# crowdbotp/socialways

Measured on AMD Instinct MI355X. Metric: GAN train steps/sec (256 scenes x 8 agents x 8+12 T per GPU step; fp32; social block on), higher is better.
Workload: dtype f32; 1 GPU; m1: 256 scenes x 8 agents x (8 obs + 12 pred) per GPU step = reference --batch-size 2048; use_social=True, n_unrolling_steps=1, info loss on; full=False, global_batch_scenes=256, parallelism=dp1, steps_per_graph_launch=32, settle_steps=992, rehearsal_regions=2, step_alg_bytes=5527040, inputs=z drawn on the host every step

## Files before the change

include/socialways_hip.h:

```cpp
#ifndef SOCIALWAYS_HIP_H
#define SOCIALWAYS_HIP_H
#include <stddef.h>
#include <stdint.h>

#ifdef __cplusplus
extern "C" {
#endif

#define SW_OK 0
#define SW_EARG -1
#define SW_ESHAPE -2
#define SW_EHIP -3

#define SW_H 64
#define SW_Z 32

enum { SW_GRP_ENC = 0, SW_GRP_EMB = 1, SW_GRP_ATT = 2, SW_GRP_DEC = 3, SW_GRP_DISC = 4 };

enum {
  SW_WS_GSAVE = 0,
  SW_WS_GDELTA = 1,
  SW_WS_DSAVE = 2,
  SW_WS_DDELTA = 3,
  SW_WS_WGRAD = 4,
  SW_WS_PAIRS = 5
};

int sw_version(void);
const char* sw_last_error(void);

int sw_param_count(int grp, int Tp);
int sw_param_offset(int grp, int idx, int Tp);
int sw_param_tensors(int grp);
size_t sw_workspace_floats(int ws_id, int B, int To, int Tp, int nb, long long P);

int sw_traj_4d(const float* obsv , const float* pred , int B, int To,
               int Tp, float* obsv4 , float* pred4 , void* stream);

int sw_enc_lstm_fwd(const float* x, int x_mode, const float* enc_w, const float* h0, const float* c0,
                    int B, int T, float* hT, float* cT, float* y , float* act,
                    float* x4s, int t0, void* stream);
int sw_enc_lstm_fwd_aux(const float* x, int x_mode, const float* enc_w, const float* h0, const float* c0, int B, int T,
                        float* hT, float* cT, float* y, float* act, float* x4s, int t0, const float* aux_src,
                        float* aux_dst, long long aux_n, void* stream);
int sw_enc_lstm_fwd_ragged(const float* x, int x_mode, const float* enc_w, const int* obs_len ,
                           int B, int T, float* hT , float* cT , void* stream);
int sw_enc_lstm_bwd(const float* enc_w, const float* act, const float* c0, const float* dhT,
                    const float* dcT, const float* dy, int B, int T, int t0, float* dgates,
                    float* dh0, float* dc0, void* stream);

int sw_social_pool_fwd(const float* obsv , int To, const float* h ,
                       const int* scene_off, int S, int B, int Amax ,
                       const float* emb_w, const float* att_w, float* S_out ,
                       float* attn ,
                       const int* big_blocks , int NB, float* wh_ws, float* ml , void* stream);
int sw_social_pool_fwd_aux(const float* obsv, int To, const float* h, const int* scene_off, int S, int B, int Amax,
                           const float* emb_w, const float* att_w, float* S_out, float* attn, const int* big_blocks,
                           int NB, float* wh_ws, float* ml, const float* aux_src, float* aux_dst, long long aux_n,
                           void* stream);
int sw_social_features(const float* x4_last , int B, float* feat , void* stream);
int sw_embed_features(const float* feat , long long R, const float* emb_w, float* out ,
                      void* stream);
int sw_attention_pool_dense(const float* f , const float* h , const int* scene_off,
                            int S, int B, const float* att_w, float* S_out , void* stream);
int sw_rows_gemm(const float* x, int ldx, const float* w, int w_rs, int w_cs, const float* bias, long long R, int K, int N,
                 float* y, int ldy, int accumulate, void* stream);
int sw_linear_wgrad(const float* delta, int ldd, const float* act, int lda, int R, int N, int K, float* dW, int ldw,
                    float* db, float* wgrad_ws, int accumulate, void* stream);
int sw_embed_features_bwd(const float* feat , long long R, const float* emb_w, const float* dout ,
                          float* rows, float* dfeat, void* stream);
int sw_attention_dense_fwd(const float* f, const float* h, const float* wh, const int* scene_off, int S, int B, float* attn,
                           float* S_out, void* stream);
int sw_attention_dense_bwd(const float* f, const float* h, const float* wh, const float* attn, const float* dS,
                           const int* scene_off, int S, int B, float* dsig, float* df, float* dwh, float* dh, void* stream);
int sw_enc_lstm_wgrad(const float* enc_w, const float* act, const float* x4s, const float* h0, const float* dgates, int B,
                      int T, float* d_enc_w, float* wgrad_ws, float* tmp, void* stream);
int sw_dec_fc_wgrad(const float* dec_w, const float* gsave, const float* gdelta, const float* h, const float* s,
                    const float* z, int B, int To, float* d_dec_w, float* wgrad_ws, float* tmp, void* stream);

int sw_dec_fc_dz(const float* dec_w, const float* gdelta, int B, int To, float* dz, void* stream);

typedef struct sw_wgrad_batch sw_wgrad_batch;
sw_wgrad_batch* sw_wgrad_batch_new(void);
void sw_wgrad_batch_free(sw_wgrad_batch* h);

int sw_social_pool_bwd(const float* obsv, int To, const float* h, const int* scene_off,
                       const long long* pair_off, int S, int B, int Amax, long long P,
                       const float* emb_w, const float* att_w, const float* attn, const float* dS,
                       float* dh, float* d_emb_w, float* d_att_w, float* pair_ws, float* wgrad_ws,
                       const int* big_blocks , int NB, const float* wh_ws, const float* ml,
                       const float* S_pool, float* big_part_ws,
                       sw_wgrad_batch* defer ,
                       void* stream);

int sw_dec_rollout_fwd(const float* obsv , int To, const float* z ,
                       const float* S_pool , const float* hT, const float* cT,
                       const float* enc_w, const float* dec_w, int B, int Tp,
                       float* pred4 , float* h_end, float* c_end ,
                       float* gsave ,
                       const float* gt , float inv_ss, float* ade_part ,
                       void* stream);
int sw_dec_rollout_fwd_aux(const float* obsv, int To, const float* z, const float* S_pool, const float* hT,
                           const float* cT, const float* enc_w, const float* dec_w, int B, int Tp, float* pred4,
                           float* h_end, float* c_end, float* gsave, const float* gt, float inv_ss, float* ade_part,
                           const float* d_w , float* dsave , void* stream);
int sw_dec_sample_fwd(const float* obsv , int To, const float* z ,
                      const float* S_pool , const float* hT, const float* cT ,
                      const float* enc_w, const float* dec_w, int B, int K, int Tp, float* pred4, const float* gt ,
                      float inv_ss, float* err, void* stream);
int sw_sample_reduce(const float* err , int B, int K, float* per_agent , int* best ,
                     void* stream);
int sw_sample_rank(const float* score , const float* err , const int* best ,
                   int B, int K, int M, int* order , float* per_agent , void* stream);
int sw_scene_clearance(const float* pos, int pstride, const float* start , int sstride, const int* scene_off,
                       int S, int B, int K, int Tp, float inv_ss, float* clear , void* stream);
int sw_scene_reduce(const float* err , const float* clear , const int* scene_off, int S, int B,
                    int K, float coll_dist, float* per_scene , int* best , void* stream);
int sw_sample_nms(const float* pos, int pstride, const float* score , const int* scene_off , int S,
                  int B, int K, int Tp, int M, int metric, float inv_ss, float radius, const float* err ,
                  const int* best , int* order , int* count , float* weight ,
                  int* assign , float* per_row , void* stream);
int sw_dec_rollout_bwd(const float* dpred4 , const float* enc_w, const float* dec_w,
                       const float* gsave, int B, int To, int Tp, float* gdelta,
                       float* dhT, float* dcT, float* dS_pool , void* stream);
int sw_dec_rollout_bwd_aux(const float* dpred4, const float* enc_w, const float* dec_w, const float* gsave, int B,
                           int To, int Tp, float* gdelta, float* dhT, float* dcT, float* dS_pool,
                           const float* aux_src, float* aux_dst, const float* aux_mask, long long aux_n, void* stream);
int sw_gen_wgrad(const float* enc_w, const float* dec_w, const float* gsave, const float* gdelta, const float* z,
                 const float* S_pool, int B, int To, int Tp, float* d_enc_w, float* d_dec_w, int part,
                 float* wgrad_ws, float* tmp ,
                 sw_wgrad_batch* pending ,
                 void* stream);
int sw_gen_wgrad_adam(const float* enc_w, const float* dec_w, const float* gsave, const float* gdelta,
                      const float* z, const float* S_pool, int B, int To, int Tp, float* d_enc_w, float* d_dec_w,
                      float* wgrad_ws, float* tmp , sw_wgrad_batch* pending , float* adam_w,
                      float* adam_m, float* adam_v, const float* adam_g, long long adam_n, const float* adam_step,
                      double lr, double beta1, double beta2, double eps, void* stream);

int sw_disc_fwd(const float* obsv, int To, int x_mode, const float* const* pred4 ,
                int nb, const float* d_w, int B, int Tp, float* const* label ,
                float* const* code , float* dsave ,
                int save_lstm ,
                float* w_snapshot ,
                void* stream);
int sw_disc_bwd(const float* d_w, const float* dsave, const float* const* dlabel,
                const float* const* dcode, int nb, int B, int To, int Tp, float* ddelta,
                float* d_d_w, float* const* dpred4, float* wgrad_ws, void* stream);

int sw_disc_bwd_gan(const float* d_w, const float* dsave, const float* const* label,
                    const float* const* code, const float* targets, int t0, int t1, const float* z ,
                    float g_label, float g_code, int nb, int B, int To, int Tp, float* ddelta,
                    float* d_d_w, float* const* dpred4, float* wgrad_ws,
                    float* loss_part ,
                    void* stream);
int sw_disc_bwd_gan_adam(const float* d_w, const float* dsave, const float* const* label, const float* const* code,
                         const float* targets, int t0, int t1, const float* z, float g_label, float g_code, int nb,
                         int B, int To, int Tp, float* ddelta, float* d_d_w, float* const* dpred4, float* wgrad_ws,
                         float* loss_part, float* adam_w, float* adam_m, float* adam_v, const float* adam_step,
                         double lr, double beta1, double beta2, double eps, void* stream);

int sw_disc_update_supported(const float* d_w, int B, int To, int Tp);
int sw_disc_update(const float* obsv , int To, const float* const* pred4 , const float* d_w, int B,
                   int Tp, float* const* label, float* const* code, float* dsave, int obs_pre, float* w_snapshot ,
                   const float* targets, int t0, int t1, const float* z, float g_label, float g_code, float* ddelta,
                   float* d_d_w, float* wgrad_ws, float* loss_part , float* adam_w , float* adam_m,
                   float* adam_v, const float* adam_step, double lr, double beta1, double beta2, double eps, void* stream);

int sw_disc_dpred_supported(int Tp);
int sw_disc_dpred(const float* obsv, int To, int x_mode, const float* pred4 , const float* d_w, int B, int Tp,
                  const float* targets, int t_idx, const float* z , float g_label, float g_code,
                  float* dpred4 , float* label , float* code ,
                  float* loss_part , void* stream);

int sw_disc_score(const float* obsv, int To, int x_mode, const float* pred4 , const float* d_w, int B, int K,
                  int Tp, float* score , float* code , void* stream);

int sw_disc_score_ragged(const float* obsv, int To, int x_mode, const int* obs_len ,
                         const float* pred4 , const float* d_w, int B, int K, int Tp, float* score ,
                         float* code , void* stream);

#define SW_RED_BLOCKS 64
int sw_gan_loss(const float* label_a, const float* targets , int ia,
                const float* code_a, const float* z , const float* label_b, int ib, int B,
                float g_label, float g_code, float* out_sums , float* dlabel_a, float* dcode_a,
                float* dlabel_b, float* dcode_b, float* scratch , void* stream);

int sw_l2_grad(const float* pred4_hat , const float* gt , int B, int Tp, int row0, int row1,
               float scale, float* dpred4 , void* stream);

int sw_variety_grad(const float* pred4_hat_K , const float* gt , int K, int B, int Tp,
                    float scale, float* dpred4_K , int* kmin, float* l2min, void* stream);

int sw_traj_dist(const float* a , const float* b , int Na, int Nb, int nPed, int T,
                 int t0, float* D , void* stream);

#define SW_STAGE_HEADER 8
int sw_stage_step(const float* slot, int B, int To, int Tp, float* obsv_dst , float* pred_dst ,
                  float* pred4_dst , float* targets_dst , float* z_dst ,
                  float* steps_dst , int n_d_updates, void* stream);

int sw_gen_image_floats(void);
int sw_gen_images(const float* enc_w, const float* dec_w, const float* emb_w , const float* att_w ,
                  float* img, void* stream);
int sw_stage_step_img(const float* slot, int B, int To, int Tp, float* obsv_dst, float* pred_dst, float* pred4_dst,
                      float* targets_dst, float* z_dst, float* steps_dst, int n_d_updates, const float* enc_w,
                      const float* dec_w, const float* emb_w , const float* att_w , float* img,
                      const float* d_w , float* d_img , const int* d_tab , void* stream);
int sw_stage_step_zdev(const float* slot, int B, int To, int Tp, float* obsv_dst, float* pred_dst, float* pred4_dst,
                       float* targets_dst, float* z_dst, float* steps_dst, int n_d_updates, const float* enc_w,
                       const float* dec_w, const float* emb_w, const float* att_w, float* img, const float* d_w, float* d_img,
                       const int* d_tab, int z_device, void* stream);

int sw_disc_image_floats(int Tp);
int sw_disc_image_table(int Tp, int* tab_host);
int sw_disc_images(const float* d_w, float* img, const int* tab, int Tp, void* stream);

int sw_lstm_point_fwd(const float* pre, const float* c_prev, int B, int H, float* gates, float* c, float* h, void* stream);
int sw_lstm_point_bwd(const float* gates, const float* c, const float* c_prev, const float* dh, const float* dc, int B,
                      int H, float* dpre, float* dc_prev, void* stream);
int sw_act_fwd(const float* x, long long n, int kind, float* y, void* stream);
int sw_act_bwd(const float* y, const float* dy, long long n, int kind, float* dx, void* stream);
int sw_sqdiff(const float* a, int lda, const float* b, int ldb, const float* target, int target_idx, long long R, int C,
              float gscale, float* out_sum, float* da, int ldda, void* stream);
int sw_pair_features(const float* x4_last, const int* scene_off, const long long* pair_off, int S, float* feat, void* stream);
int sw_attn_pairs_fwd(const float* f, const float* wh, const float* h, const int* scene_off, const long long* pair_off, int S,
                      int B, int F, int H, float* attn, float* S_out, void* stream);
int sw_attn_pairs_bwd(const float* f, const float* wh, const float* h, const float* attn, const float* dS, const int* scene_off,
                      const long long* pair_off, int S, int B, int F, int H, float* dsig, float* df, float* dwh, float* dh,
                      void* stream);

int sw_adam_packed(float* w, const float* g, float* m, float* v, long long n, const float* step, double lr, double beta1,
                   double beta2, double eps, int disc_Tp, void* stream);

int sw_enc_lstm_bwd_aux(const float* enc_w, const float* act, const float* c0, const float* dhT, const float* dcT,
                        const float* dy, int B, int T, int t0, float* dgates, float* dh0, float* dc0, const float* aux_src,
                        float* aux_dst, const float* aux_mask, long long aux_n, void* stream);
int sw_dec_rollout_bwd_dfuse(const float* obsv, const float* pred4, const float* d_w, const float* targets, int t_idx,
                             const float* z, float g_label, float g_code, float* loss_part, float* dpred4, const float* enc_w,
                             const float* dec_w, const float* gsave, int B, int To, int Tp, float* gdelta, float* dhT, float* dcT,
                             float* dS_pool, void* stream);

int sw_wide_gemm(const float* x, long long x_rs, int x_cs, const float* w, long long w_rs, int w_cs, const float* bias,
                 const float* cin, int cin_ld, const float* aux, int aux_ld, long long R, int K, int N, float* y, int y_ld, int epi,
                 void* stream);
int sw_wide_lstm_fwd(const float* x4, int x_ld, const float* h_prev, int hp_ld, const float* c_prev, const float* Wx,
                     const float* b1, const float* b2, const float* Whh, int B, int H, float* gates, float* c_out, float* h_out,
                     int h_ld, float* h_out2, int h2_ld, void* stream);
int sw_wide_lstm_bwd(const float* dh_ext, int dhe_ld, const float* dh_ext2, int dhe2_ld, const float* dg_next, const float* WhhT,
                     const float* gates, const float* c, const float* c_prev, const float* dc_in, int B, int H, float* dgates,
                     float* dc_out, void* stream);
int sw_wide_out_fwd(const float* a3, int D3, const float* W4, const float* b4, float* p, int B, float* pred4_i, int pred_ld,
                    float* x4_tm, void* stream);
int sw_wide_out_bwd(const float* dpred4_i, int pred_ld, const float* dg, const float* WxT, int H4, float* dp_run, int B, float* dv,
                    const float* W4, int D3, float* dz3, void* stream);
int sw_wide_sum_steps(const float* in, long long t_stride, int in_ld, int T, long long R, int C, float* out, int out_ld,
                      void* stream);
int sw_wide_transpose(const float* src, const int* tab, int ntab, int total_tiles, float* dst, void* stream);
int sw_wide_opimage(const float* src, const int* tab, int ntab, long long total_float4, float* dst, void* stream);
int sw_wide_lstm_seq_supported(int H);
int sw_wide_lstm_seq_fwd(const float* x4, const float* Wx, const float* b1, const float* b2, const float* whh_img, int B, int H, int T,
                         float* gates, float* cs, float* hs, float* h_last2, int h2_ld, void* stream);
int sw_wide_lstm_seq_bwd(const float* dh_ext, int dhe_ld, const float* dh_ext2, int dhe2_ld, const float* dg_init, const float* dc_init,
                         const float* whhT_img, const float* gates, const float* cs, int B, int H, int T, float* dgates, void* stream);
int sw_wide_dec_loop_supported(int H);
int sw_wide_dec_loop_fwd(const float* w1h_img, const float* w2_img, const float* w3_img, const float* whh_img, const float* u,
                         const float* b2, const float* b3, const float* W4, const float* b4, const float* Wx, const float* bx1,
                         const float* bx2, const float* p0, int p0_ld, float* a1, float* a2, float* a3, float* pred4, float* x4,
                         float* gates, float* cs, float* hs, float* cat, int B, int H, int To, int Tp, void* stream);
int sw_wide_dec_loop_bwd(const float* whhT_img, const float* w3T_img, const float* w2T_img, const float* w1hT_img,
                         const float* wxT_img, const float* W4, const float* dpred4, const float* a1, const float* a2,
                         const float* gates, const float* cs, float* dgates, float* dv, float* dz3, float* dz2, float* dz1,
                         float* dhcat_out, float* dc_out, int B, int H, int To, int Tp, void* stream);
int sw_wide_disc_heads_supported(int H, int K4, int nl);
int sw_wide_disc_heads_fwd(const long long* p, void* stream);
int sw_wide_disc_heads_bwd(const long long* p, void* stream);
int sw_wide_wgrad(const long long* desc, int n, float* wgrad_ws, void* stream);

long long sw_comm_bytes(int world, long long max_floats);
int sw_comm_alloc(long long bytes, void** ptr);
int sw_comm_free(void* ptr);
int sw_comm_ipc_export(void* ptr, void* handle64 );
int sw_comm_ipc_import(const void* handle64, void** ptr);
int sw_comm_ipc_close(void* ptr);
int sw_comm_status(const void* own_buf, int* status );
int sw_allreduce_direct(void* const* peer_bufs , int rank, int world, long long max_floats, float* grad,
                        long long n, void* stream);
int sw_allreduce_direct_adam(void* const* peer_bufs, int rank, int world, long long max_floats, float* grad, long long n,
                             float* w, float* m, float* v, const float* step, double lr, double beta1, double beta2,
                             double eps, int disc_Tp, void* stream);

int sw_ade_fde(const float* pred4 , const float* gt , int B, int Tp, float inv_ss,
               float* out , float* scratch , void* stream);

int sw_noise_uniform(unsigned long long seed, int domain, unsigned step0, int n_steps, unsigned draw0, int n_draws,
                     unsigned row0, int rows, int cols, int ld, float* out , void* stream);

int sw_kernel_timing(int on);
int sw_kernel_timing_read(char* buf, int cap);
int sw_debug_spin(double us, void* stream);

#ifdef __cplusplus
}
#endif
#endif
```

socialways_amd/_lib.py:

```python
import ctypes
import os

import torch

_HERE = os.path.dirname(os.path.abspath(__file__))
LIB_PATH = os.environ.get("SW_LIB_PATH") or os.path.join(_HERE, "libsocialways_hip.so")

GRP_ENC, GRP_EMB, GRP_ATT, GRP_DEC, GRP_DISC = 0, 1, 2, 3, 4
WS_GSAVE, WS_GDELTA, WS_DSAVE, WS_DDELTA, WS_WGRAD, WS_PAIRS = 0, 1, 2, 3, 4, 5
AMAX = 64
RED_BLOCKS = 64

_vp, _i, _f, _ll = ctypes.c_void_p, ctypes.c_int, ctypes.c_float, ctypes.c_longlong

PROTOTYPES = {
    "sw_version": (_i, []),
    "sw_last_error": (ctypes.c_char_p, []),
    "sw_param_count": (_i, [_i, _i]),
    "sw_param_offset": (_i, [_i, _i, _i]),
    "sw_param_tensors": (_i, [_i]),
    "sw_workspace_floats": (ctypes.c_size_t, [_i, _i, _i, _i, _i, _ll]),
    "sw_traj_4d": (_i, [_vp, _vp, _i, _i, _i, _vp, _vp, _vp]),
    "sw_enc_lstm_fwd": (_i, [_vp, _i, _vp, _vp, _vp, _i, _i, _vp, _vp, _vp, _vp, _vp, _i, _vp]),
    "sw_enc_lstm_fwd_aux": (_i, [_vp, _i, _vp, _vp, _vp, _i, _i, _vp, _vp, _vp, _vp, _vp, _i, _vp, _vp, _ll, _vp]),
    "sw_enc_lstm_fwd_ragged": (_i, [_vp, _i, _vp, _vp, _i, _i, _vp, _vp, _vp]),
    "sw_enc_lstm_bwd": (_i, [_vp, _vp, _vp, _vp, _vp, _vp, _i, _i, _i, _vp, _vp, _vp, _vp]),
    "sw_social_pool_fwd": (_i, [_vp, _i, _vp, _vp, _i, _i, _i, _vp, _vp, _vp, _vp, _vp, _i, _vp, _vp, _vp]),
    "sw_social_pool_fwd_aux": (_i, [_vp, _i, _vp, _vp, _i, _i, _i, _vp, _vp, _vp, _vp, _vp, _i, _vp, _vp, _vp, _vp, _ll, _vp]),
    "sw_social_features": (_i, [_vp, _i, _vp, _vp]),
    "sw_embed_features": (_i, [_vp, _ll, _vp, _vp, _vp]),
    "sw_attention_pool_dense": (_i, [_vp, _vp, _vp, _i, _i, _vp, _vp, _vp]),
    "sw_social_pool_bwd": (_i, [_vp, _i, _vp, _vp, _vp, _i, _i, _i, _ll, _vp, _vp, _vp, _vp, _vp, _vp, _vp,
                                _vp, _vp, _vp, _i, _vp, _vp, _vp, _vp, _vp, _vp]),
    "sw_dec_rollout_fwd": (_i, [_vp, _i, _vp, _vp, _vp, _vp, _vp, _vp, _i, _i, _vp, _vp, _vp, _vp, _vp, _f, _vp, _vp]),
    "sw_dec_rollout_fwd_aux": (_i, [_vp, _i, _vp, _vp, _vp, _vp, _vp, _vp, _i, _i, _vp, _vp, _vp, _vp, _vp, _f, _vp, _vp, _vp, _vp]),
    "sw_dec_sample_fwd": (_i, [_vp, _i, _vp, _vp, _vp, _vp, _vp, _vp, _i, _i, _i, _vp, _vp, _f, _vp, _vp]),
    "sw_sample_reduce": (_i, [_vp, _i, _i, _vp, _vp, _vp]),
    "sw_sample_rank": (_i, [_vp, _vp, _vp, _i, _i, _i, _vp, _vp, _vp]),
    "sw_scene_clearance": (_i, [_vp, _i, _vp, _i, _vp, _i, _i, _i, _i, _f, _vp, _vp]),
    "sw_scene_reduce": (_i, [_vp, _vp, _vp, _i, _i, _i, _f, _vp, _vp, _vp]),
    "sw_sample_nms": (_i, [_vp, _i, _vp, _vp, _i, _i, _i, _i, _i, _i, _f, _f, _vp, _vp, _vp, _vp, _vp, _vp, _vp, _vp]),
    "sw_dec_rollout_bwd": (_i, [_vp, _vp, _vp, _vp, _i, _i, _i, _vp, _vp, _vp, _vp, _vp]),
    "sw_dec_rollout_bwd_aux": (_i, [_vp, _vp, _vp, _vp, _i, _i, _i, _vp, _vp, _vp, _vp, _vp, _vp, _vp, _ll, _vp]),
    "sw_gen_wgrad": (_i, [_vp, _vp, _vp, _vp, _vp, _vp, _i, _i, _i, _vp, _vp, _i, _vp, _vp, _vp, _vp]),
    "sw_gen_wgrad_adam": (_i, [_vp, _vp, _vp, _vp, _vp, _vp, _i, _i, _i, _vp, _vp, _vp, _vp, _vp, _vp, _vp, _vp, _vp,
                               ctypes.c_longlong, _vp, ctypes.c_double, ctypes.c_double, ctypes.c_double, ctypes.c_double, _vp]),
    "sw_enc_lstm_bwd_aux": (_i, [_vp, _vp, _vp, _vp, _vp, _vp, _i, _i, _i, _vp, _vp, _vp, _vp, _vp, _vp, _ll, _vp]),
    "sw_dec_rollout_bwd_dfuse": (_i, [_vp, _vp, _vp, _vp, _i, _vp, _f, _f, _vp, _vp, _vp, _vp, _vp, _i, _i, _i, _vp, _vp, _vp, _vp,
                                      _vp]),
    "sw_rows_gemm": (_i, [_vp, _i, _vp, _i, _i, _vp, ctypes.c_longlong, _i, _i, _vp, _i, _i, _vp]),
    "sw_linear_wgrad": (_i, [_vp, _i, _vp, _i, _i, _i, _i, _vp, _i, _vp, _vp, _i, _vp]),
    "sw_embed_features_bwd": (_i, [_vp, ctypes.c_longlong, _vp, _vp, _vp, _vp, _vp]),
    "sw_attention_dense_fwd": (_i, [_vp, _vp, _vp, _vp, _i, _i, _vp, _vp, _vp]),
    "sw_attention_dense_bwd": (_i, [_vp, _vp, _vp, _vp, _vp, _vp, _i, _i, _vp, _vp, _vp, _vp, _vp]),
    "sw_enc_lstm_wgrad": (_i, [_vp, _vp, _vp, _vp, _vp, _i, _i, _vp, _vp, _vp, _vp]),
    "sw_dec_fc_dz": (_i, [_vp, _vp, _i, _i, _vp, _vp]),
    "sw_dec_fc_wgrad": (_i, [_vp, _vp, _vp, _vp, _vp, _vp, _i, _i, _vp, _vp, _vp, _vp]),
    "sw_wgrad_batch_new": (_vp, []),
    "sw_wgrad_batch_free": (None, [_vp]),
    "sw_disc_fwd": (_i, [_vp, _i, _i, _vp, _i, _vp, _i, _i, _vp, _vp, _vp, _i, _vp, _vp]),
    "sw_disc_bwd": (_i, [_vp, _vp, _vp, _vp, _i, _i, _i, _i, _vp, _vp, _vp, _vp, _vp]),
    "sw_disc_bwd_gan": (_i, [_vp, _vp, _vp, _vp, _vp, _i, _i, _vp, _f, _f, _i, _i, _i, _i, _vp, _vp, _vp, _vp, _vp, _vp]),
    "sw_disc_bwd_gan_adam": (_i, [_vp, _vp, _vp, _vp, _vp, _i, _i, _vp, _f, _f, _i, _i, _i, _i, _vp, _vp, _vp, _vp, _vp,
                                  _vp, _vp, _vp, _vp, ctypes.c_double, ctypes.c_double, ctypes.c_double, ctypes.c_double, _vp]),
    "sw_disc_update_supported": (_i, [_vp, _i, _i, _i]),
    "sw_disc_dpred_supported": (_i, [_i]),
    "sw_disc_update": (_i, [_vp, _i, _vp, _vp, _i, _i, _vp, _vp, _vp, _i, _vp, _vp, _i, _i, _vp, _f, _f, _vp, _vp, _vp, _vp,
                            _vp, _vp, _vp, _vp, ctypes.c_double, ctypes.c_double, ctypes.c_double, ctypes.c_double, _vp]),
    "sw_disc_dpred": (_i, [_vp, _i, _i, _vp, _vp, _i, _i, _vp, _i, _vp, _f, _f, _vp, _vp, _vp, _vp, _vp]),
    "sw_disc_score": (_i, [_vp, _i, _i, _vp, _vp, _i, _i, _i, _vp, _vp, _vp]),
    "sw_disc_score_ragged": (_i, [_vp, _i, _i, _vp, _vp, _vp, _i, _i, _i, _vp, _vp, _vp]),
    "sw_gan_loss": (_i, [_vp, _vp, _i, _vp, _vp, _vp, _i, _i, _f, _f, _vp, _vp, _vp, _vp, _vp, _vp, _vp]),
    "sw_l2_grad": (_i, [_vp, _vp, _i, _i, _i, _i, _f, _vp, _vp]),
    "sw_variety_grad": (_i, [_vp, _vp, _i, _i, _i, _f, _vp, _vp, _vp, _vp]),
    "sw_traj_dist": (_i, [_vp, _vp, _i, _i, _i, _i, _i, _vp, _vp]),
    "sw_stage_step": (_i, [_vp, _i, _i, _i, _vp, _vp, _vp, _vp, _vp, _vp, _i, _vp]),
    "sw_gen_image_floats": (_i, []),
    "sw_gen_images": (_i, [_vp, _vp, _vp, _vp, _vp, _vp]),
    "sw_stage_step_img": (_i, [_vp, _i, _i, _i, _vp, _vp, _vp, _vp, _vp, _vp, _i, _vp, _vp, _vp, _vp, _vp, _vp, _vp, _vp, _vp]),
    "sw_stage_step_zdev": (_i, [_vp, _i, _i, _i, _vp, _vp, _vp, _vp, _vp, _vp, _i, _vp, _vp, _vp, _vp, _vp, _vp, _vp, _vp, _i, _vp]),
    "sw_disc_image_floats": (_i, [_i]),
    "sw_disc_image_table": (_i, [_i, _vp]),
    "sw_disc_images": (_i, [_vp, _vp, _vp, _i, _vp]),
    "sw_ade_fde": (_i, [_vp, _vp, _i, _i, _f, _vp, _vp, _vp]),
    "sw_lstm_point_fwd": (_i, [_vp, _vp, _i, _i, _vp, _vp, _vp, _vp]),
    "sw_lstm_point_bwd": (_i, [_vp, _vp, _vp, _vp, _vp, _i, _i, _vp, _vp, _vp]),
    "sw_act_fwd": (_i, [_vp, _ll, _i, _vp, _vp]),
    "sw_act_bwd": (_i, [_vp, _vp, _ll, _i, _vp, _vp]),
    "sw_sqdiff": (_i, [_vp, _i, _vp, _i, _vp, _i, _ll, _i, _f, _vp, _vp, _i, _vp]),
    "sw_pair_features": (_i, [_vp, _vp, _vp, _i, _vp, _vp]),
    "sw_attn_pairs_fwd": (_i, [_vp, _vp, _vp, _vp, _vp, _i, _i, _i, _i, _vp, _vp, _vp]),
    "sw_attn_pairs_bwd": (_i, [_vp, _vp, _vp, _vp, _vp, _vp, _vp, _i, _i, _i, _i, _vp, _vp, _vp, _vp, _vp]),
    "sw_adam_packed": (_i, [_vp, _vp, _vp, _vp, _ll, _vp, ctypes.c_double, ctypes.c_double, ctypes.c_double,
                            ctypes.c_double, _i, _vp]),
    "sw_wide_gemm": (_i, [_vp, _ll, _i, _vp, _ll, _i, _vp, _vp, _i, _vp, _i, _ll, _i, _i, _vp, _i, _i, _vp]),
    "sw_wide_lstm_fwd": (_i, [_vp, _i, _vp, _i, _vp, _vp, _vp, _vp, _vp, _i, _i, _vp, _vp, _vp, _i, _vp, _i, _vp]),
    "sw_wide_lstm_bwd": (_i, [_vp, _i, _vp, _i, _vp, _vp, _vp, _vp, _vp, _vp, _i, _i, _vp, _vp, _vp]),
    "sw_wide_out_fwd": (_i, [_vp, _i, _vp, _vp, _vp, _i, _vp, _i, _vp, _vp]),
    "sw_wide_out_bwd": (_i, [_vp, _i, _vp, _vp, _i, _vp, _i, _vp, _vp, _i, _vp, _vp]),
    "sw_wide_sum_steps": (_i, [_vp, _ll, _i, _i, _ll, _i, _vp, _i, _vp]),
    "sw_wide_wgrad": (_i, [_vp, _i, _vp, _vp]),
    "sw_wide_transpose": (_i, [_vp, _vp, _i, _i, _vp, _vp]),
    "sw_wide_dec_loop_supported": (_i, [_i]),
    "sw_wide_dec_loop_fwd": (_i, [_vp] * 13 + [_i] + [_vp] * 9 + [_i, _i, _i, _i, _vp]),
    "sw_wide_dec_loop_bwd": (_i, [_vp] * 18 + [_i, _i, _i, _i, _vp]),
    "sw_wide_disc_heads_supported": (_i, [_i, _i, _i]),
    "sw_wide_disc_heads_fwd": (_i, [_vp, _vp]),
    "sw_wide_disc_heads_bwd": (_i, [_vp, _vp]),
    "sw_wide_opimage": (_i, [_vp, _vp, _i, _ll, _vp, _vp]),
    "sw_wide_lstm_seq_supported": (_i, [_i]),
    "sw_wide_lstm_seq_fwd": (_i, [_vp, _vp, _vp, _vp, _vp, _i, _i, _i, _vp, _vp, _vp, _vp, _i, _vp]),
    "sw_wide_lstm_seq_bwd": (_i, [_vp, _i, _vp, _i, _vp, _vp, _vp, _vp, _vp, _i, _i, _i, _vp, _vp]),
    "sw_comm_bytes": (_ll, [_i, _ll]),
    "sw_comm_alloc": (_i, [_ll, _vp]),
    "sw_comm_free": (_i, [_vp]),
    "sw_comm_ipc_export": (_i, [_vp, _vp]),
    "sw_comm_ipc_import": (_i, [_vp, _vp]),
    "sw_comm_ipc_close": (_i, [_vp]),
    "sw_comm_status": (_i, [_vp, _vp]),
    "sw_allreduce_direct": (_i, [_vp, _i, _i, _ll, _vp, _ll, _vp]),
    "sw_allreduce_direct_adam": (_i, [_vp, _i, _i, _ll, _vp, _ll, _vp, _vp, _vp, _vp, ctypes.c_double, ctypes.c_double,
                                      ctypes.c_double, ctypes.c_double, _i, _vp]),
    "sw_noise_uniform": (_i, [ctypes.c_ulonglong, _i, ctypes.c_uint, _i, ctypes.c_uint, _i, ctypes.c_uint, _i, _i, _i, _vp, _vp]),
}

DEBUG_PROTOTYPES = {
    "sw_kernel_timing": (_i, [_i]),
    "sw_kernel_timing_read": (_i, [ctypes.c_char_p, _i]),
    "sw_debug_spin": (_i, [ctypes.c_double, _vp]),
}
_lib = None


class SocialWaysHipError(RuntimeError):
    pass


def load():
    global _lib
    if _lib is not None:
        return _lib
    if not os.path.exists(LIB_PATH):
        raise SocialWaysHipError(
            "%s not found - build it with `python -c 'import __graft_entry__ as g; g.build()'` or "
            "`make -C socialways_amd/csrc`; socialways_amd has no CPU fallback" % LIB_PATH)
    lib = ctypes.CDLL(LIB_PATH)
    for name, (res, args) in list(PROTOTYPES.items()) + list(DEBUG_PROTOTYPES.items()):
        fn = getattr(lib, name)
        fn.restype = res
        fn.argtypes = args
    _lib = lib
    return lib


def ptr(t):
    if t is None:
        return None
    assert t.is_contiguous(), "socialways_amd kernels need contiguous tensors"
    return t.data_ptr()


def ptr_strided(t):
    return None if t is None else t.data_ptr()


def stream():
    return torch.cuda.current_stream().cuda_stream


TIMING = None


def call(name, *args):
    lib = load()
    t = TIMING
    if t is not None and name in t["names"]:
        e0, e1 = torch.cuda.Event(enable_timing=True), torch.cuda.Event(enable_timing=True)
        e0.record()
        rc = getattr(lib, name)(*args)
        e1.record()
        t["events"].append((name, e0, e1))
    else:
        rc = getattr(lib, name)(*args)
    if rc != 0:
        msg = {-1: "bad argument", -2: "unsupported shape", -3: "HIP error: " + lib.sw_last_error().decode()}.get(rc, "?")
        raise SocialWaysHipError("%s failed (%d): %s" % (name, rc, msg))


def ptr_array(tensors):
    arr = (ctypes.c_void_p * len(tensors))(*[ptr(t) for t in tensors])
    return ctypes.cast(arr, ctypes.c_void_p), arr


def workspace_floats(ws_id, B, To, Tp, nb=1, P=0):
    return int(load().sw_workspace_floats(ws_id, B, To, Tp, nb, P))


def require_gpu(t):
    if not t.is_cuda:
        raise SocialWaysHipError("socialways_amd runs on MI355X only: got a %s tensor (no CPU fallback)" % t.device)


def indexed_device(device):
    d = torch.device(device)
    if d.type == "cuda" and d.index is None and torch.cuda.is_available():
        d = torch.device("cuda", torch.cuda.current_device())
    return d
```

socialways_amd/csrc/sw_misc.hip:

```cpp
#include "../../include/socialways_hip.h"
#include "sw_common.h"
#include "sw_lstm_dev.h"
#include <stdlib.h>
#include "sw_wgrad.h"
#include <stdio.h>
#include <string.h>

static thread_local char g_err[256] = "";
void sw_set_error(const char* what, hipError_t e) {
  snprintf(g_err, sizeof(g_err), "%s: %s", what, hipGetErrorString(e));
}
extern "C" const char* sw_last_error(void) { return g_err; }

int sw_set_lds(const void* fn, int bytes, int& have) {
  if (have >= bytes) return SW_OK;
  hipError_t e = hipFuncSetAttribute(fn, hipFuncAttributeMaxDynamicSharedMemorySize, bytes);
  if (e != hipSuccess) {
    sw_set_error("hipFuncSetAttribute(MaxDynamicSharedMemorySize)", e);
    return SW_EHIP;
  }
  have = bytes;
  return SW_OK;
}

#include <string>
#include <vector>
#include <map>
bool g_sw_ktime_on = false;
#include <mutex>
namespace {
struct KtRec { const char* name; hipEvent_t e0, e1; bool ended; };
std::vector<KtRec> g_kt;
std::mutex g_kt_mu;
thread_local long t_kt_open = -1;
}
void sw_ktime_begin(const char* name, hipStream_t st) {
  t_kt_open = -1;
  hipStreamCaptureStatus cs = hipStreamCaptureStatusNone;
  if (hipStreamIsCapturing(st, &cs) != hipSuccess || cs != hipStreamCaptureStatusNone) { (void)hipGetLastError(); return; }
  KtRec r{name, nullptr, nullptr, false};
  if (hipEventCreate(&r.e0) != hipSuccess) { (void)hipGetLastError(); return; }
  if (hipEventCreate(&r.e1) != hipSuccess) { (void)hipGetLastError(); (void)hipEventDestroy(r.e0); return; }
  (void)hipEventRecord(r.e0, st);
  std::lock_guard<std::mutex> lk(g_kt_mu);
  g_kt.push_back(r);
  t_kt_open = (long)g_kt.size() - 1;
}
void sw_ktime_end(hipStream_t st) {
  const long i = t_kt_open;
  t_kt_open = -1;
  if (i < 0) return;
  std::lock_guard<std::mutex> lk(g_kt_mu);
  if (i >= (long)g_kt.size() || g_kt[i].ended) return;
  (void)hipEventRecord(g_kt[i].e1, st);
  g_kt[i].ended = true;
}
extern "C" int sw_kernel_timing(int on) {
  std::lock_guard<std::mutex> lk(g_kt_mu);
  for (auto& r : g_kt) { (void)hipEventDestroy(r.e0); (void)hipEventDestroy(r.e1); }
  g_kt.clear();
  g_sw_ktime_on = on != 0;
  return SW_OK;
}
extern "C" int sw_kernel_timing_read(char* buf, int cap) {
  if (hipDeviceSynchronize() != hipSuccess) return SW_EHIP;
  std::map<std::string, std::pair<long, double>> agg;
  std::lock_guard<std::mutex> lk(g_kt_mu);
  for (auto& r : g_kt) {
    if (!r.ended) continue;
    float ms = 0.f;
    if (hipEventElapsedTime(&ms, r.e0, r.e1) != hipSuccess) { (void)hipGetLastError(); continue; }
    std::string n(r.name);
    size_t a = n.find_first_not_of("( ");
    n = n.substr(a == std::string::npos ? 0 : a);
    n = n.substr(0, n.find_first_of("<)"));
    auto& e = agg[n];
    e.first += 1;
    e.second += 1e3 * ms;
  }
  std::string out;
  char line[256];
  for (auto& kv : agg) {
    snprintf(line, sizeof(line), "%s %ld %.3f\n", kv.first.c_str(), kv.second.first, kv.second.second);
    out += line;
  }
  if (buf && cap > 0) {
    const size_t k = out.size() < (size_t)cap - 1 ? out.size() : (size_t)cap - 1;
    memcpy(buf, out.data(), k);
    buf[k] = 0;
  }
  return (int)out.size() + 1;
}
__global__ void spin_kernel(long long cycles) {
  const long long t0 = wall_clock64();
  while (wall_clock64() - t0 < cycles) __builtin_amdgcn_s_sleep(32);
}
__global__ void nop_kernel() {}
extern "C" int sw_debug_spin(double us, void* stream) {
  if (us < 0 || us > 2e6) return SW_EARG;
  if (us == 0.0) {
    SW_LAUNCH(nop_kernel, dim3(1), dim3(64), 0, (hipStream_t)stream);
    SW_CHECK_LAUNCH("nop_kernel");
    return SW_OK;
  }
  SW_LAUNCH(spin_kernel, dim3(1), dim3(64), 0, (hipStream_t)stream, (long long)(us * 100.0));
  SW_CHECK_LAUNCH("spin_kernel");
  return SW_OK;
}

__global__ __launch_bounds__(256) void adam_packed_kernel(WgAdam ad, long long n) {
  __shared__ float bc[2];
  if (threadIdx.x == 0) wg_adam_bc_compute(ad.step, ad.beta1, ad.beta2, bc[0], bc[1]);
  __syncthreads();
  const float bc1 = bc[0], bc2s = bc[1];
  for (long long i = (long long)blockIdx.x * 256 + threadIdx.x; i < n; i += (long long)gridDim.x * 256) {
    const float g = ad.g0[i];
    wg_adam_fin(ad, wg_adam_pre(ad, ad.g0 + i), bc1, bc2s, g);
  }
}
extern "C" int sw_adam_packed(float* w, const float* g, float* m, float* v, long long n, const float* step, double lr,
                              double beta1, double beta2, double eps, int disc_Tp, void* stream) {
  if (!w || !g || !m || !v || !step || n < 1) return SW_EARG;
  WgAdam ad;
  ad.w = w; ad.m = m; ad.v = v; ad.g0 = g; ad.step = step; ad.n = (size_t)n;
  ad.lr = lr; ad.beta1 = beta1; ad.beta2 = beta2; ad.eps = eps;
  if (disc_Tp > 0) {
    const DiscImages di = sw_disc_images_for(w, disc_Tp);
    ad.img = const_cast<float*>(di.img);
    ad.tab = di.tab;
  }
  int blocks = (int)((n + 255) / 256);
  if (blocks > 512) blocks = 512;
  SW_LAUNCH(adam_packed_kernel, dim3(blocks), dim3(256), 0, (hipStream_t)stream, ad, n);
  SW_CHECK_LAUNCH("adam_packed_kernel");
  return SW_OK;
}
extern "C" int sw_version(void) { return 3; }

size_t sw_dsave_floats(int B, int To, int Tp, int nb);
size_t sw_ddelta_floats(int B, int To, int Tp, int nb);

static int group_offsets(int grp, int Tp, int* off, int* count) {
  using namespace swp;
  switch (grp) {
    case SW_GRP_ENC: {
      const int o[] = {ENC_EMB_W, ENC_EMB_B, ENC_WIH, ENC_WHH, ENC_BIH, ENC_BHH};
      memcpy(off, o, sizeof(o));
      *count = ENC_N;
      return 6;
    }
    case SW_GRP_EMB: {
      const int o[] = {EMB_W0, EMB_B0, EMB_W1, EMB_B1, EMB_W2, EMB_B2};
      memcpy(off, o, sizeof(o));
      *count = EMB_N;
      return 6;
    }
    case SW_GRP_ATT: {
      const int o[] = {ATT_W, ATT_B};
      memcpy(off, o, sizeof(o));
      *count = ATT_N;
      return 2;
    }
    case SW_GRP_DEC: {
      const int o[] = {DEC_W1, DEC_B1, DEC_W2, DEC_B2, DEC_W3, DEC_B3, DEC_W4, DEC_B4};
      memcpy(off, o, sizeof(o));
      *count = DEC_N;
      return 8;
    }
    case SW_GRP_DISC: {
      if (Tp < 1) return -1;
      Disc d = disc(Tp);
      const int o[] = {d.wih,  d.whh,  d.bih,  d.bhh,  d.of0w, d.of0b, d.of1w, d.of1b, d.pe0w, d.pe0b,
                       d.pe1w, d.pe1b, d.cl0w, d.cl0b, d.cl1w, d.cl1b, d.la0w, d.la0b, d.la1w, d.la1b};
      memcpy(off, o, sizeof(o));
      *count = d.n;
      return 20;
    }
  }
  return -1;
}
extern "C" int sw_param_tensors(int grp) {
  int off[32], n;
  return group_offsets(grp, 1, off, &n);
}
extern "C" int sw_param_count(int grp, int Tp) {
  int off[32], n = -1;
  if (group_offsets(grp, Tp, off, &n) < 0) return SW_EARG;
  return n;
}
extern "C" int sw_param_offset(int grp, int idx, int Tp) {
  int off[32], n;
  int k = group_offsets(grp, Tp, off, &n);
  if (k < 0 || idx < 0 || idx >= k) return SW_EARG;
  return off[idx];
}

extern "C" size_t sw_workspace_floats(int ws_id, int B, int To, int Tp, int nb, long long P) {
  if (B < 0 || To < 1 || Tp < 1) return 0;
  switch (ws_id) {
    case SW_WS_GSAVE: return gsave_layout(B, To, Tp).total;
    case SW_WS_GDELTA: return gdelta_layout(B, To, Tp).total;
    case SW_WS_DSAVE: return sw_dsave_floats(B, To, Tp, nb < 1 ? 1 : nb);
    case SW_WS_DDELTA: return sw_ddelta_floats(B, To, Tp, nb < 1 ? 1 : nb);
    case SW_WS_WGRAD: return SW_WG_WS_FLOATS;
    case SW_WS_PAIRS: return (size_t)B * 200 + (size_t)(P < 0 ? 0 : P) * 196;
  }
  return 0;
}

#define SW_DEC_COMPOSE_BLOCKS 13
__device__ __forceinline__ void compose_bwd_block(const int blk, const float* __restrict__ enc_w,
                                                  const float* __restrict__ dWx, const float* __restrict__ dbx,
                                                  float* __restrict__ d_enc_w, const float* __restrict__ dec_w,
                                                  const float* __restrict__ Ms, float* __restrict__ d_dec_w,
                                                  const WgAdam& ad, const float* __restrict__ snap) {
  using namespace swp;
  float bc1 = 1.f, bc2s = 1.f;
  if (ad.w) wg_adam_bc(ad, bc1, bc2s);
  auto put = [&](float* dst, float g) {
    *dst = g;
    if (ad.w) wg_adam1(ad, bc1, bc2s, dst, g);
  };
  if (blk >= 128) {
    const int o = (blk - 128) * 256 + threadIdx.x;
    const float* M = Ms;
    const float* sv = Ms + 160;
    const float* W3 = snap ? snap + swimg::RAW_W3 : dec_w + DEC_W3;
    const float* W4 = snap ? snap + swimg::RAW_W4 : dec_w + DEC_W4;
    const float* b3 = snap ? snap + swimg::RAW_B3 : dec_w + DEC_B3;
    if (o < 3200) {
      const int m = o / 80, k = o - m * 80;
      put(d_dec_w + DEC_W3 + o, fmaf(W4[m], M[k], W4[40 + m] * M[80 + k]));
    } else if (o < 3240) {
      const int m = o - 3200;
      put(d_dec_w + DEC_B3 + m, fmaf(W4[m], sv[0], W4[40 + m] * sv[1]));
    } else if (o < 3320) {
      const int c = (o - 3240) / 40, m = (o - 3240) - c * 40;
      float v = sv[c] * b3[m];
      for (int k = 0; k < 80; ++k) v = fmaf(M[c * 80 + k], W3[m * 80 + k], v);
      put(d_dec_w + DEC_W4 + c * 40 + m, v);
    } else if (o < 3322) {
      put(d_dec_w + DEC_B4 + (o - 3320), sv[o - 3320]);
    }
    return;
  }
  const float* We = snap ? snap + swimg::RAW_WE : enc_w + ENC_EMB_W;
  const float* be = snap ? snap + swimg::RAW_BE : enc_w + ENC_EMB_B;
  const float* Wih = snap ? snap + swimg::RAW_WIH : enc_w + ENC_WIH;
  const int t = threadIdx.x;
  if (blk < 64) {
    int i = blk * 256 + t;
    int row = i >> 6, e = i & 63;
    f32x4 g = ld4(dWx + row * 4), w = ld4(We + e * 4);
    float v = dbx[row] * be[e];
    v = fmaf(g[0], w[0], v); v = fmaf(g[1], w[1], v); v = fmaf(g[2], w[2], v); v = fmaf(g[3], w[3], v);
    put(d_enc_w + ENC_WIH + i, v);
    if (blk == 0) {
      put(d_enc_w + ENC_BIH + t, dbx[t]);
      put(d_enc_w + ENC_BHH + t, dbx[t]);
    }
    return;
  }
  __shared__ float red[5][256];
  const int e = blk - 64;
  float w = Wih[t * 64 + e];
  f32x4 g = ld4(dWx + t * 4);
  red[0][t] = w * g[0]; red[1][t] = w * g[1]; red[2][t] = w * g[2]; red[3][t] = w * g[3]; red[4][t] = w * dbx[t];
  __syncthreads();
  for (int o = 128; o > 0; o >>= 1) {
    if (t < o) {
#pragma unroll
      for (int c = 0; c < 5; ++c) red[c][t] += red[c][t + o];
    }
    __syncthreads();
  }
  if (t < 4) put(d_enc_w + ENC_EMB_W + e * 4 + t, red[t][0]);
  if (t == 4) put(d_enc_w + ENC_EMB_B + e, red[4][0]);
}

__global__ __launch_bounds__(256) void enc_compose_bwd_kernel(const float* __restrict__ enc_w,
                                                              const float* __restrict__ dWx,
                                                              const float* __restrict__ dbx,
                                                              float* __restrict__ d_enc_w,
                                                              const float* __restrict__ dec_w,
                                                              const float* __restrict__ Ms,
                                                              float* __restrict__ d_dec_w, WgAdam ad,
                                                              const float* __restrict__ snap) {
  compose_bwd_block((int)blockIdx.x, enc_w, dWx, dbx, d_enc_w, dec_w, Ms, d_dec_w, ad, snap);
}
__global__ __launch_bounds__(256) void compose_bwd_part_kernel(const float* __restrict__ enc_w, const float* __restrict__ dWx,
                                                               const float* __restrict__ dbx, float* __restrict__ d_enc_w,
                                                               const float* __restrict__ dec_w, const float* __restrict__ Ms,
                                                               float* __restrict__ d_dec_w, int block0) {
  compose_bwd_block((int)blockIdx.x + block0, enc_w, dWx, dbx, d_enc_w, dec_w, Ms, d_dec_w, WgAdam(), nullptr);
}

static int gen_wgrad_impl(const float* enc_w, const float* dec_w, const float* gsave, const float* gdelta, const float* z,
                          const float* S_pool, int B, int To, int Tp, float* d_enc_w, float* d_dec_w, int part,
                          float* wgrad_ws, float* tmp, sw_wgrad_batch* pending, void* stream, WgAdam ad,
                          const float* snap) {
  if (!enc_w || !dec_w || !gsave || !gdelta || !z || !S_pool || !d_enc_w || !d_dec_w || !wgrad_ws || !tmp || B < 1 || To < 2 ||
      Tp < 1 || part < 0 || part > 2)
    return SW_EARG;
  using namespace swp;
  const GSave gs = gsave_layout(B, To, Tp);
  const GDelta gd = gdelta_layout(B, To, Tp);
  const int Ta = To + Tp - 1;
  float* dWx = tmp;
  float* dbx = tmp + 1024;
  float* dM = tmp + 1280;
  hipStream_t st = (hipStream_t)stream;
  WgBatch wb;
  if (pending) {
    wb = *wg_pending(pending);
    *wg_pending(pending) = WgBatch();
  }
  int rc_add = 0;
  const int t_lo = part == 1 ? To : 0, t_hi = part == 2 ? To : Ta;
  const int acc = part == 2 ? 1 : 0;
  if (t_hi > t_lo)
    rc_add |= wg_add_tail(wb, gdelta + gd.dgates + (size_t)t_lo * B * 256, 256,
                          gsave + gs.act + ((ptrdiff_t)t_lo - 1) * B * 384 + 320, 384, (t_hi - t_lo) * B, 256, 64,
                          d_enc_w + ENC_WHH, 64, gsave + gs.x4s + (size_t)t_lo * B * 4, 4, 4, dWx, 4,
                          t_lo < 1 ? B : 0 , dbx, nullptr, acc);
  if (part != 2) {
    rc_add |= wg_add(wb, gdelta + gd.dz1, 160, gsave + gs.act + (size_t)(To - 1) * B * 384 + 320, 384, Tp * B, 160, 64,
                     d_dec_w + DEC_W1, 160, nullptr, nullptr, 0);
    rc_add |= wg_add(wb, gdelta + gd.du, 160, S_pool, 64, B, 160, 64, d_dec_w + DEC_W1 + 64, 160, nullptr, nullptr, 0);
    rc_add |= wg_add(wb, gdelta + gd.du, 160, z, 32, B, 160, 32, d_dec_w + DEC_W1 + 128, 160, d_dec_w + DEC_B1, nullptr, 0);
    rc_add |= wg_add(wb, gdelta + gd.dz2, 80, gsave + gs.a1, 160, Tp * B, 80, 160, d_dec_w + DEC_W2, 160, d_dec_w + DEC_B2,
                     nullptr, 0);
    rc_add |= wg_add(wb, gdelta + gd.dv, 4, gsave + gs.a2, 80, Tp * B, 2, 80, dM, 80, dM + 160, nullptr, 0);
  }
  if (rc_add) return SW_ESHAPE;
  if (int rc = ad.w ? wg_launch_adam(wb, wgrad_ws, ad, st) : wg_launch(wb, wgrad_ws, st)) return rc;
  if (part != 1) {
    SW_LAUNCH(enc_compose_bwd_kernel, dim3(128 + SW_DEC_COMPOSE_BLOCKS), dim3(256), 0, st, enc_w, dWx, dbx, d_enc_w,
                       dec_w, dM, d_dec_w, ad, snap);
    SW_CHECK_LAUNCH("enc_compose_bwd_kernel");
  }
  return SW_OK;
}
extern "C" int sw_gen_wgrad(const float* enc_w, const float* dec_w, const float* gsave, const float* gdelta, const float* z,
                            const float* S_pool, int B, int To, int Tp, float* d_enc_w, float* d_dec_w, int part,
                            float* wgrad_ws, float* tmp, sw_wgrad_batch* pending, void* stream) {
  return gen_wgrad_impl(enc_w, dec_w, gsave, gdelta, z, S_pool, B, To, Tp, d_enc_w, d_dec_w, part, wgrad_ws, tmp, pending,
                        stream, WgAdam(), nullptr);
}
extern "C" int sw_gen_wgrad_adam(const float* enc_w, const float* dec_w, const float* gsave, const float* gdelta,
                                 const float* z, const float* S_pool, int B, int To, int Tp, float* d_enc_w, float* d_dec_w,
                                 float* wgrad_ws, float* tmp, sw_wgrad_batch* pending, float* adam_w, float* adam_m,
                                 float* adam_v, const float* adam_g, long long adam_n, const float* adam_step, double lr,
                                 double beta1, double beta2, double eps, void* stream) {
  if (!adam_w || !adam_m || !adam_v || !adam_g || !adam_step || adam_n < 1 || !enc_w || !dec_w || !d_enc_w || !d_dec_w)
    return SW_EARG;
  if (enc_w - adam_w != d_enc_w - adam_g || dec_w - adam_w != d_dec_w - adam_g || enc_w < adam_w ||
      dec_w + swp::DEC_N > adam_w + adam_n || enc_w + swp::ENC_N > adam_w + adam_n || dec_w < adam_w)
    return SW_EARG;
  const float* img = sw_gen_images_for(enc_w, dec_w);
  if (!img) return SW_EARG;
  WgAdam ad;
  ad.w = adam_w; ad.m = adam_m; ad.v = adam_v; ad.g0 = adam_g; ad.step = adam_step; ad.n = (size_t)adam_n;
  ad.lr = lr; ad.beta1 = beta1; ad.beta2 = beta2; ad.eps = eps;
  return gen_wgrad_impl(enc_w, dec_w, gsave, gdelta, z, S_pool, B, To, Tp, d_enc_w, d_dec_w, 0, wgrad_ws, tmp, pending, stream,
                        ad, img);
}

extern "C" int sw_enc_lstm_wgrad(const float* enc_w, const float* act, const float* x4s, const float* h0, const float* dgates,
                                 int B, int T, float* d_enc_w, float* wgrad_ws, float* tmp, void* stream) {
  if (!enc_w || !act || !x4s || !dgates || !d_enc_w || !wgrad_ws || !tmp || B < 1 || T < 1) return SW_EARG;
  using namespace swp;
  hipStream_t st = (hipStream_t)stream;
  float* dWx = tmp;
  float* dbx = tmp + 1024;
  WgBatch wb;
  if (wg_add_tail(wb, dgates, 256, act - (ptrdiff_t)B * 384 + 320, 384, T * B, 256, 64, d_enc_w + ENC_WHH, 64, x4s, 4, 4, dWx, 4,
                  B, dbx, nullptr, 0))
    return SW_ESHAPE;
  if (int rc = wg_launch(wb, wgrad_ws, st)) return rc;
  if (h0) {
    WgBatch w0;
    if (wg_add(w0, dgates, 256, h0, 64, B, 256, 64, d_enc_w + ENC_WHH, 64, nullptr, nullptr, 1)) return SW_ESHAPE;
    if (int rc = wg_launch(w0, wgrad_ws, st)) return rc;
  }
  SW_LAUNCH(compose_bwd_part_kernel, dim3(128), dim3(256), 0, st, enc_w, dWx, dbx, d_enc_w, nullptr, nullptr, nullptr, 0);
  SW_CHECK_LAUNCH("compose_bwd_part_kernel");
  return SW_OK;
}
extern "C" int sw_dec_fc_wgrad(const float* dec_w, const float* gsave, const float* gdelta, const float* h, const float* s,
                               const float* z, int B, int To, float* d_dec_w, float* wgrad_ws, float* tmp, void* stream) {
  if (!dec_w || !gsave || !gdelta || !h || !z || !d_dec_w || !wgrad_ws || !tmp || B < 1 || To < 2) return SW_EARG;
  using namespace swp;
  hipStream_t st = (hipStream_t)stream;
  const GSave gs = gsave_layout(B, To, 1);
  const GDelta gd = gdelta_layout(B, To, 1);
  float* dM = tmp + 1280;
  WgBatch wb;
  int rc = 0;
  rc |= wg_add(wb, gdelta + gd.dz1, 160, h, 64, B, 160, 64, d_dec_w + DEC_W1, 160, nullptr, nullptr, 0);
  if (s) rc |= wg_add(wb, gdelta + gd.dz1, 160, s, 64, B, 160, 64, d_dec_w + DEC_W1 + 64, 160, nullptr, nullptr, 0);
  rc |= wg_add(wb, gdelta + gd.dz1, 160, z, 32, B, 160, 32, d_dec_w + DEC_W1 + 128, 160, d_dec_w + DEC_B1, nullptr, 0);
  rc |= wg_add(wb, gdelta + gd.dz2, 80, gsave + gs.a1, 160, B, 80, 160, d_dec_w + DEC_W2, 160, d_dec_w + DEC_B2, nullptr, 0);
  rc |= wg_add(wb, gdelta + gd.dv, 4, gsave + gs.a2, 80, B, 2, 80, dM, 80, dM + 160, nullptr, 0);
  if (rc) return SW_ESHAPE;
  if (int r2 = wg_launch(wb, wgrad_ws, st)) return r2;
  if (!s) {
    if (hipMemset2DAsync(d_dec_w + DEC_W1 + 64, 160 * sizeof(float), 0, 64 * sizeof(float), 160, st) != hipSuccess) return SW_EHIP;
  }
  SW_LAUNCH(compose_bwd_part_kernel, dim3(SW_DEC_COMPOSE_BLOCKS), dim3(256), 0, st, nullptr, nullptr, nullptr, nullptr,
                     dec_w, dM, d_dec_w, 128);
  SW_CHECK_LAUNCH("compose_bwd_part_kernel");
  return SW_OK;
}

__device__ __forceinline__ void block_sum3(float& a, float& b, float& c, float (*red)[16]) {
#pragma unroll
  for (int o = 32; o > 0; o >>= 1) {
    a += __shfl_xor(a, o);
    b += __shfl_xor(b, o);
    c += __shfl_xor(c, o);
  }
  int w = threadIdx.x >> 6, l = threadIdx.x & 63;
  if (l == 0) { red[0][w] = a; red[1][w] = b; red[2][w] = c; }
  __syncthreads();
  if (w == 0) {
    a = l < 16 ? red[0][l] : 0.f;
    b = l < 16 ? red[1][l] : 0.f;
    c = l < 16 ? red[2][l] : 0.f;
#pragma unroll
    for (int o = 8; o > 0; o >>= 1) {
      a += __shfl_xor(a, o);
      b += __shfl_xor(b, o);
      c += __shfl_xor(c, o);
    }
  }
}

__global__ __launch_bounds__(1024) void gan_loss_kernel(
    const float* __restrict__ label_a, const float* __restrict__ targets, int ia, const float* __restrict__ code_a,
    const float* __restrict__ z, const float* __restrict__ label_b, int ib, int B, float g_label, float g_code,
    float* __restrict__ out, float* __restrict__ dlabel_a, float* __restrict__ dcode_a, float* __restrict__ dlabel_b,
    float* __restrict__ dcode_b) {
  __shared__ float red[3][16];
  const float t_a = targets[ia], t_b = targets[ib];
  float s0 = 0.f, s1 = 0.f, s2 = 0.f;
  for (int b = blockIdx.x * blockDim.x + threadIdx.x; b < B; b += gridDim.x * blockDim.x) {
    float e = label_a[b] - t_a;
    s0 = fmaf(e, e, s0);
    if (dlabel_a) dlabel_a[b] = 2.0f * e * g_label;
    float c0 = code_a[(size_t)b * 2] - z[(size_t)b * SW_Z], c1 = code_a[(size_t)b * 2 + 1] - z[(size_t)b * SW_Z + 1];
    s1 += c0 * c0 + c1 * c1;
    if (dcode_a) {
      dcode_a[(size_t)b * 2] = 2.0f * c0 * g_code;
      dcode_a[(size_t)b * 2 + 1] = 2.0f * c1 * g_code;
    }
    if (label_b) {
      float f = label_b[b] - t_b;
      s2 = fmaf(f, f, s2);
      if (dlabel_b) dlabel_b[b] = 2.0f * f * g_label;
    }
    if (dcode_b) {
      dcode_b[(size_t)b * 2] = 0.f;
      dcode_b[(size_t)b * 2 + 1] = 0.f;
    }
  }
  block_sum3(s0, s1, s2, red);
  if (threadIdx.x == 0) { out[3 * blockIdx.x] = s0; out[3 * blockIdx.x + 1] = s1; out[3 * blockIdx.x + 2] = s2; }
}

__global__ __launch_bounds__(64) void sum3_kernel(const float* __restrict__ part, int G, float s_a, float* __restrict__ out) {
  float a = 0.f, b = 0.f, c = 0.f;
  for (int g = threadIdx.x; g < G; g += 64) { a += part[3 * g]; b += part[3 * g + 1]; c += part[3 * g + 2]; }
#pragma unroll
  for (int o = 32; o > 0; o >>= 1) {
    a += __shfl_xor(a, o);
    b += __shfl_xor(b, o);
    c += __shfl_xor(c, o);
  }
  if (threadIdx.x == 0) { out[0] = a * s_a; out[1] = b; out[2] = c; }
}
#define SW_RED_SINGLE 32768
static inline int red_blocks(long long n, const float* scratch) {
  if (!scratch || n <= SW_RED_SINGLE) return 1;
  long long g = (n + 8191) / 8192;
  return (int)(g > SW_RED_BLOCKS ? SW_RED_BLOCKS : g);
}

extern "C" int sw_gan_loss(const float* label_a, const float* targets, int ia, const float* code_a, const float* z,
                           const float* label_b, int ib, int B, float g_label, float g_code, float* out_sums,
                           float* dlabel_a, float* dcode_a, float* dlabel_b, float* dcode_b, float* scratch,
                           void* stream) {
  if (!label_a || !targets || !code_a || !z || !out_sums || B < 1 || ia < 0 || ib < 0) return SW_EARG;
  const int G = red_blocks((long long)B * 4, scratch);
  SW_LAUNCH(gan_loss_kernel, dim3(G), dim3(1024), 0, (hipStream_t)stream, label_a, targets, ia, code_a, z,
                     label_b, ib, B, g_label, g_code, G > 1 ? scratch : out_sums, dlabel_a, dcode_a, dlabel_b, dcode_b);
  SW_CHECK_LAUNCH("gan_loss_kernel");
  if (G > 1) {
    SW_LAUNCH(sum3_kernel, dim3(1), dim3(64), 0, (hipStream_t)stream, scratch, G, 1.0f, out_sums);
    SW_CHECK_LAUNCH("sum3_kernel");
  }
  return SW_OK;
}

__global__ __launch_bounds__(1024) void ade_fde_kernel(const float* __restrict__ pred4, const float* __restrict__ gt,
                                                       int B, int Tp, float inv_ss, float* __restrict__ out,
                                                       int single) {
  __shared__ float red[3][16];
  float sa = 0.f, sf = 0.f, sl = 0.f;
  const int n = B * Tp;
  for (int base = blockIdx.x * 1024 * 8; base < n; base += gridDim.x * 1024 * 8) {
    f32x4 p[8];
    float2 g[8];
#pragma unroll
    for (int u = 0; u < 8; ++u) {
      int i = base + threadIdx.x + 1024 * u;
      bool ok = i < n;
      p[u] = ok ? ld4(pred4 + (size_t)i * 4) : f32x4{0.f, 0.f, 0.f, 0.f};
      g[u] = ok ? *reinterpret_cast<const float2*>(gt + (size_t)i * 2) : float2{0.f, 0.f};
    }
#pragma unroll
    for (int u = 0; u < 8; ++u) {
      int i = base + threadIdx.x + 1024 * u;
      float dx = (p[u][0] - g[u].x) * inv_ss, dy = (p[u][1] - g[u].y) * inv_ss;
      float q = dx * dx + dy * dy;
      float e = sqrtf(q);
      sa += e;
      sl += q;
      if (i < n && i % Tp == Tp - 1) sf += e;
    }
  }
  block_sum3(sa, sf, sl, red);
  if (threadIdx.x == 0) {
    out[3 * blockIdx.x] = single ? sa / (float)Tp : sa;
    out[3 * blockIdx.x + 1] = sf;
    out[3 * blockIdx.x + 2] = sl;
  }
}

extern "C" int sw_ade_fde(const float* pred4, const float* gt, int B, int Tp, float inv_ss, float* out, float* scratch,
                          void* stream) {
  if (!pred4 || !gt || !out || B < 1 || Tp < 1) return SW_EARG;
  const int G = red_blocks((long long)B * Tp, scratch);
  SW_LAUNCH(ade_fde_kernel, dim3(G), dim3(1024), 0, (hipStream_t)stream, pred4, gt, B, Tp, inv_ss,
                     G > 1 ? scratch : out, G == 1 ? 1 : 0);
  SW_CHECK_LAUNCH("ade_fde_kernel");
  if (G > 1) {
    SW_LAUNCH(sum3_kernel, dim3(1), dim3(64), 0, (hipStream_t)stream, scratch, G, 1.0f / (float)Tp, out);
    SW_CHECK_LAUNCH("sum3_kernel");
  }
  return SW_OK;
}

__global__ __launch_bounds__(256) void l2_grad_kernel(const float* __restrict__ pred4, const float* __restrict__ gt,
                                                       int Tp, int row0, int row1, float scale,
                                                       float* __restrict__ dpred4) {
  const long long n = (long long)(row1 - row0) * Tp;
  for (long long i = (long long)blockIdx.x * 256 + threadIdx.x; i < n; i += (long long)gridDim.x * 256) {
    const size_t e = (size_t)row0 * Tp + i;
    f32x4 p = ld4(pred4 + e * 4), d = ld4(dpred4 + e * 4);
    float2 g = *reinterpret_cast<const float2*>(gt + e * 2);
    d[0] = fmaf(scale, p[0] - g.x, d[0]);
    d[1] = fmaf(scale, p[1] - g.y, d[1]);
    st4(dpred4 + e * 4, d);
  }
}
extern "C" int sw_l2_grad(const float* pred4, const float* gt, int B, int Tp, int row0, int row1, float scale,
                          float* dpred4, void* stream) {
  if (!pred4 || !gt || !dpred4 || B < 1 || Tp < 1 || row0 < 0 || row1 > B || row0 > row1) return SW_EARG;
  if (row0 == row1) return SW_OK;
  long long n = (long long)(row1 - row0) * Tp;
  int blocks = (int)((n + 255) / 256);
  if (blocks > 1024) blocks = 1024;
  SW_LAUNCH(l2_grad_kernel, dim3(blocks), dim3(256), 0, (hipStream_t)stream, pred4, gt, Tp, row0, row1, scale,
                     dpred4);
  SW_CHECK_LAUNCH("l2_grad_kernel");
  return SW_OK;
}

__global__ __launch_bounds__(256) void variety_grad_kernel(const float* __restrict__ predK, const float* __restrict__ gt,
                                                            int K, int B, int Tp, float scale, float* __restrict__ dpredK,
                                                            int* __restrict__ kmin_out, float* __restrict__ l2min_out) {
  const int lane = sw_lane(), b = blockIdx.x * 4 + sw_wave();
  if (b >= B) return;
  float l2 = 3.0e38f;
  if (lane < K) {
    float s = 0.f;
    const float* ph = predK + ((size_t)lane * B + b) * Tp * 4;
    for (int t = 0; t < Tp; ++t) {
      const f32x4 p = ld4(ph + t * 4);
      const float2 g = *reinterpret_cast<const float2*>(gt + ((size_t)b * Tp + t) * 2);
      const float dx = p[0] - g.x, dy = p[1] - g.y;
      s = fmaf(dx, dx, fmaf(dy, dy, s));
    }
    l2 = s / (float)(2 * Tp);
  }
  int km = lane;
#pragma unroll
  for (int o = 32; o > 0; o >>= 1) {
    const float ol = __shfl_xor(l2, o);
    const int ok = __shfl_xor(km, o);
    if (ol < l2 || (ol == l2 && ok < km)) {
      l2 = ol;
      km = ok;
    }
  }
  if (lane == 0) {
    if (kmin_out) kmin_out[b] = km;
    if (l2min_out) l2min_out[b] = l2;
  }
  for (int t = lane; t < Tp; t += 64) {
    const size_t e = ((size_t)km * B + b) * Tp + t;
    f32x4 p = ld4(predK + e * 4), d = ld4(dpredK + e * 4);
    const float2 g = *reinterpret_cast<const float2*>(gt + ((size_t)b * Tp + t) * 2);
    d[0] = fmaf(scale, p[0] - g.x, d[0]);
    d[1] = fmaf(scale, p[1] - g.y, d[1]);
    st4(dpredK + e * 4, d);
  }
}
extern "C" int sw_variety_grad(const float* predK, const float* gt, int K, int B, int Tp, float scale, float* dpredK,
                               int* kmin, float* l2min, void* stream) {
  if (!predK || !gt || !dpredK || B < 1 || Tp < 1 || K < 1) return SW_EARG;
  if (K > 64) return SW_ESHAPE;
  SW_LAUNCH(variety_grad_kernel, dim3((B + 3) / 4), dim3(256), 0, (hipStream_t)stream, predK, gt, K, B, Tp, scale,
                     dpredK, kmin, l2min);
  SW_CHECK_LAUNCH("variety_grad_kernel");
  return SW_OK;
}

__global__ __launch_bounds__(256) void sample_reduce_kernel(const float* __restrict__ err, int B, int K,
                                                             float* __restrict__ per_agent, int* __restrict__ best) {
  const int a = blockIdx.x * 256 + threadIdx.x;
  if (a >= B) return;
  const float2* e = reinterpret_cast<const float2*>(err) + a;
  float2 v = e[0];
  float sa = v.x, sf = v.y, ma = v.x, mf = v.y;
  int kb = 0;
#pragma unroll 8
  for (int k = 1; k < K; ++k) {
    v = e[(size_t)k * B];
    sa += v.x;
    sf += v.y;
    if (v.x < ma) {
      ma = v.x;
      kb = k;
    }
    mf = v.y < mf ? v.y : mf;
  }
  st4(per_agent + (size_t)a * 4, f32x4{sa / (float)K, sf / (float)K, ma, mf});
  if (best) best[a] = kb;
}
extern "C" int sw_sample_reduce(const float* err, int B, int K, float* per_agent, int* best, void* stream) {
  if (!err || !per_agent || B < 0 || K < 1) return SW_EARG;
  if (B == 0) return SW_OK;
  SW_LAUNCH(sample_reduce_kernel, dim3((B + 255) / 256), dim3(256), 0, (hipStream_t)stream, err, B, K, per_agent, best);
  SW_CHECK_LAUNCH("sample_reduce_kernel");
  return SW_OK;
}

#define SW_RANK_MAXK 4096
__global__ __launch_bounds__(256) void sample_rank_kernel(const float* __restrict__ score, const float* __restrict__ err,
                                                           const int* __restrict__ best, int B, int K, int M,
                                                           int* __restrict__ order, float* __restrict__ per_agent) {
  extern __shared__ __attribute__((aligned(16))) float rank_s[];
  const int wave = threadIdx.x >> 6, lane = threadIdx.x & 63;
  const int a = min((int)blockIdx.x * 4 + wave, B - 1);
  const bool live = (int)blockIdx.x * 4 + wave < B;
  float* s = rank_s + wave * K;
  for (int k = lane; k < K; k += 64) s[k] = score[(size_t)k * B + a];
  __syncthreads();
  const float2* e = reinterpret_cast<const float2*>(err);
  const float inf = __builtin_inff();
  float ma = inf, mf = inf;
  int k0 = -1, rb = 0;
  const int kb = best ? best[a] : -1;
  for (int k = lane; k < K; k += 64) {
    const float v = s[k];
    int r = 0;
    for (int j = 0; j < K; ++j) {
      const float u = s[j];
      r += (u > v || (u == v && j < k)) ? 1 : 0;
    }
    if (r < M) {
      if (live) order[(size_t)a * M + r] = k;
      if (per_agent) {
        const float2 ek = e[(size_t)k * B + a];
        ma = fminf(ma, ek.x);
        mf = fminf(mf, ek.y);
      }
    }
    if (r == 0) k0 = k;
    if (k == kb) rb = r;
  }
  if (!per_agent) return;
#pragma unroll
  for (int o = 32; o > 0; o >>= 1) {
    ma = fminf(ma, __shfl_xor(ma, o));
    mf = fminf(mf, __shfl_xor(mf, o));
    k0 = max(k0, __shfl_xor(k0, o));
    rb = max(rb, __shfl_xor(rb, o));
  }
  if (lane == 0 && live) {
    const float2 e0 = e[(size_t)max(k0, 0) * B + a];
    float* p = per_agent + (size_t)a * 5;
    p[0] = e0.x; p[1] = e0.y; p[2] = ma; p[3] = mf; p[4] = (float)rb;
  }
}
extern "C" int sw_sample_rank(const float* score, const float* err, const int* best, int B, int K, int M, int* order,
                              float* per_agent, void* stream) {
  if (!score || !order || B < 0 || K < 1 || M < 1 || M > K || (per_agent && !err)) return SW_EARG;
  if (K > SW_RANK_MAXK) return SW_ESHAPE;
  if (B == 0) return SW_OK;
  SW_LAUNCH(sample_rank_kernel, dim3((B + 3) / 4), dim3(256), 4 * K * sizeof(float), (hipStream_t)stream, score, err, best, B, K,
            M, order, per_agent);
  SW_CHECK_LAUNCH("sample_rank_kernel");
  return SW_OK;
}

__global__ __launch_bounds__(256) void traj_dist_kernel(const float* __restrict__ a, const float* __restrict__ b, int Na,
                                                         int Nb, int nPed, int T, int t0, float* __restrict__ D) {
  const long long n = (long long)nPed * Na * Nb;
  for (long long e = (long long)blockIdx.x * 256 + threadIdx.x; e < n; e += (long long)gridDim.x * 256) {
    const int j = (int)(e % Nb), i = (int)((e / Nb) % Na), k = (int)(e / ((long long)Nb * Na));
    const float2* pa = reinterpret_cast<const float2*>(a) + ((size_t)i * nPed + k) * T;
    const float2* pb = reinterpret_cast<const float2*>(b) + ((size_t)j * nPed + k) * T;
    float s = 0.f;
    for (int t = t0; t < T; ++t) {
      float2 x = pa[t], y = pb[t];
      float dx = x.x - y.x, dy = x.y - y.y;
      s += sqrtf(dx * dx + dy * dy);
    }
    D[e] = s / (float)(T - t0);
  }
}
extern "C" int sw_traj_dist(const float* a, const float* b, int Na, int Nb, int nPed, int T, int t0, float* D,
                            void* stream) {
  if (!a || !b || !D || Na < 1 || Nb < 1 || nPed < 1 || T < 1 || t0 < 0 || t0 >= T) return SW_EARG;
  long long n = (long long)nPed * Na * Nb;
  int blocks = (int)((n + 255) / 256);
  if (blocks > 2048) blocks = 2048;
  SW_LAUNCH(traj_dist_kernel, dim3(blocks), dim3(256), 0, (hipStream_t)stream, a, b, Na, Nb, nPed, T, t0, D);
  SW_CHECK_LAUNCH("traj_dist_kernel");
  return SW_OK;
}

#define SW_IMG_BLOCKS 64
__device__ __forceinline__ void gen_images_block(const float* __restrict__ enc_w, const float* __restrict__ dec_w,
                                                 const float* __restrict__ emb_w, const float* __restrict__ att_w,
                                                 float* __restrict__ img, int blk) {
  using namespace swp;
  if (blk == 0) {
    lstm_prep_rows(enc_w + ENC_EMB_W, enc_w + ENC_EMB_B, enc_w + ENC_WIH, enc_w + ENC_BIH, enc_w + ENC_BHH, true,
                   img + swimg::WX, img + swimg::BX);
    return;
  }
  if (blk == 1) {
    const int t = threadIdx.x;
    if (t < 160) {
      const int c = t / 80, k = t - c * 80;
      const float* w4 = dec_w + DEC_W4 + c * 40;
      float v0 = 0.f, v1 = 0.f, v2 = 0.f, v3 = 0.f;
#pragma unroll
      for (int m = 0; m < 40; m += 4) {
        v0 = fmaf(w4[m], dec_w[DEC_W3 + m * 80 + k], v0);
        v1 = fmaf(w4[m + 1], dec_w[DEC_W3 + (m + 1) * 80 + k], v1);
        v2 = fmaf(w4[m + 2], dec_w[DEC_W3 + (m + 2) * 80 + k], v2);
        v3 = fmaf(w4[m + 3], dec_w[DEC_W3 + (m + 3) * 80 + k], v3);
      }
      img[swimg::W43 + c * 80 + k] = (v0 + v1) + (v2 + v3);
    } else if (t < 162) {
      const int c = t - 160;
      float v = dec_w[DEC_B4 + c];
#pragma unroll
      for (int m = 0; m < 40; m += 4) {
        const f32x4 w = ld4(dec_w + DEC_W4 + c * 40 + m), bb = ld4(dec_w + DEC_B3 + m);
        v = fmaf(w[0], bb[0], fmaf(w[1], bb[1], fmaf(w[2], bb[2], fmaf(w[3], bb[3], v))));
      }
      img[swimg::W43 + 160 + c] = v;
    }
    return;
  }
  const int nth = (SW_IMG_BLOCKS - 2) * 256, tid = (blk - 2) * 256 + threadIdx.x;
  for (int i = tid; i < (swimg::RAW_END - swimg::RAW_WIH) / 4; i += nth) {
    const int o = swimg::RAW_WIH + 4 * i;
    const float* src = o < swimg::RAW_WE   ? enc_w + ENC_WIH + (o - swimg::RAW_WIH)
                       : o < swimg::RAW_BE ? enc_w + ENC_EMB_W + (o - swimg::RAW_WE)
                       : o < swimg::RAW_W3 ? enc_w + ENC_EMB_B + (o - swimg::RAW_BE)
                       : o < swimg::RAW_B3 ? dec_w + DEC_W3 + (o - swimg::RAW_W3)
                       : o < swimg::RAW_W4 ? dec_w + DEC_B3 + (o - swimg::RAW_B3)
                                           : dec_w + DEC_W4 + (o - swimg::RAW_W4);
    st4(img + o, ld4(src));
  }
  auto op_image = [&](int dst0, const float* W, int ldw, int c0, int KJ, int ntile) {
    for (int f = tid; f < ntile * KJ * 64; f += nth) {
      const int t = f / (KJ * 64), rem = f - t * (KJ * 64), j = rem >> 6, l = rem & 63;
      st4(img + dst0 + 4 * (size_t)f, ld4(W + (size_t)(16 * t + (l & 15)) * ldw + c0 + 16 * j + 4 * (l >> 4)));
    }
  };
  auto op_image_T = [&](int dst0, const float* W, int ldw, int KJ, int ntile) {
    for (int f = tid; f < ntile * KJ * 64; f += nth) {
      const int t = f / (KJ * 64), rem = f - t * (KJ * 64), j = rem >> 6, l = rem & 63;
      const float* col = W + (size_t)(16 * j + 4 * (l >> 4)) * ldw + 16 * t + (l & 15);
      st4(img + dst0 + 4 * (size_t)f, f32x4{col[0], col[ldw], col[2 * ldw], col[3 * ldw]});
    }
  };
  op_image(swimg::OP_WHH, enc_w + ENC_WHH, 64, 0, 4, 16);
  op_image(swimg::OP_W1H, dec_w + DEC_W1, 160, 0, 4, 10);
  op_image(swimg::OP_W1SZ, dec_w + DEC_W1, 160, 64, 6, 10);
  op_image(swimg::OP_W2, dec_w + DEC_W2, 160, 0, 10, 5);
  op_image_T(swimg::OP_WHHT, enc_w + ENC_WHH, 64, 16, 4);
  op_image_T(swimg::OP_W2T, dec_w + DEC_W2, 160, 5, 10);
  op_image_T(swimg::OP_W1HT, dec_w + DEC_W1, 160, 10, 4);
  for (int f = tid; f < 8 * 2 * 4 * 64; f += nth) {
    const int l = f & 63, j = (f >> 6) & 3, tile = (f >> 8) & 1, w = f >> 9, m = l & 15;
    const int row = (2 * tile + ((m & 3) >> 1)) * 64 + 8 * w + 2 * (m >> 2) + (m & 1);
    st4(img + swimg::OP_WHH8 + 4 * (size_t)f, ld4(enc_w + ENC_WHH + (size_t)row * 64 + 16 * j + 4 * (l >> 4)));
  }
  if (emb_w) {
    op_image(swimg::OP_E1, emb_w + EMB_W1, 32, 0, 2, 4);
    op_image(swimg::OP_E2, emb_w + EMB_W2, 64, 0, 4, 4);
    op_image_T(swimg::OP_E1T, emb_w + EMB_W1, 32, 4, 2);
    op_image_T(swimg::OP_E2T, emb_w + EMB_W2, 64, 4, 4);
    op_image_T(swimg::OP_ATT_T, att_w + ATT_W, 64, 4, 4);
  }
}
__global__ __launch_bounds__(256) void gen_images_kernel(const float* __restrict__ enc_w, const float* __restrict__ dec_w,
                                                          const float* __restrict__ emb_w, const float* __restrict__ att_w,
                                                          float* __restrict__ img) {
  gen_images_block(enc_w, dec_w, emb_w, att_w, img, blockIdx.x);
}
static thread_local const float *g_img_enc = nullptr, *g_img_dec = nullptr, *g_img_emb = nullptr, *g_img_att = nullptr,
                                *g_img = nullptr;
const float* sw_soc_images_for(const float* emb_w, const float* att_w) {
  return (g_img && emb_w && emb_w == g_img_emb && att_w == g_img_att) ? g_img : nullptr;
}
const float* sw_gen_images_for(const float* enc_w, const float* dec_w) {
  return (g_img && enc_w == g_img_enc && (!dec_w || dec_w == g_img_dec)) ? g_img : nullptr;
}
extern "C" int sw_gen_image_floats(void) { return swimg::N; }
static void gen_images_register(const float* enc_w, const float* dec_w, const float* emb_w, const float* att_w,
                                const float* img) {
  g_img_enc = enc_w; g_img_dec = dec_w; g_img_emb = emb_w; g_img_att = att_w; g_img = img;
}
extern "C" int sw_gen_images(const float* enc_w, const float* dec_w, const float* emb_w, const float* att_w, float* img,
                             void* stream) {
  if (!img) {
    gen_images_register(nullptr, nullptr, nullptr, nullptr, nullptr);
    return SW_OK;
  }
  if (!enc_w || !dec_w || ((emb_w != nullptr) != (att_w != nullptr))) return SW_EARG;
  SW_LAUNCH(gen_images_kernel, dim3(SW_IMG_BLOCKS), dim3(256), 0, (hipStream_t)stream, enc_w, dec_w, emb_w, att_w, img);
  SW_CHECK_LAUNCH("gen_images_kernel");
  gen_images_register(enc_w, dec_w, emb_w, att_w, img);
  return SW_OK;
}

__global__ __launch_bounds__(256) void stage_step_kernel(const float* __restrict__ slot, int B, int To, int Tp,
                                                          float* __restrict__ obsv_dst, float* __restrict__ pred_dst,
                                                          float* __restrict__ pred4_dst, float* __restrict__ targets_dst,
                                                          float* __restrict__ z_dst, float* __restrict__ steps_dst,
                                                          int n_d_updates, const float* __restrict__ enc_w,
                                                          const float* __restrict__ dec_w, const float* __restrict__ emb_w,
                                                          const float* __restrict__ att_w, float* __restrict__ img,
                                                          int img_blocks, const float* __restrict__ d_w,
                                                          float* __restrict__ d_img, const int* __restrict__ d_tab, int d_n,
                                                          int dimg_blocks, int z_device) {
  if ((int)blockIdx.x >= (int)gridDim.x - img_blocks) {
    gen_images_block(enc_w, dec_w, emb_w, att_w, img, (int)blockIdx.x - ((int)gridDim.x - img_blocks));
    return;
  }
  if ((int)blockIdx.x >= (int)gridDim.x - img_blocks - dimg_blocks) {
    disc_images_scatter(d_w, d_img, d_tab, d_n, (int)blockIdx.x - ((int)gridDim.x - img_blocks - dimg_blocks), dimg_blocks);
    return;
  }
  const unsigned long long* ptrs = reinterpret_cast<const unsigned long long*>(slot);
  const float* obsv = reinterpret_cast<const float*>(ptrs[0]);
  const float* pred = reinterpret_cast<const float*>(ptrs[1]);
  const int gid = blockIdx.x * 256 + threadIdx.x, gsz = ((int)gridDim.x - img_blocks - dimg_blocks) * 256;
  if (z_dst) {
    const float* zs = z_device ? reinterpret_cast<const float*>(ptrs[4]) : slot + 8;
    for (int i = gid; i < B * SW_Z / 4; i += gsz) st4(z_dst + 4 * (size_t)i, ld4(zs + 4 * (size_t)i));
  }
  if (gid < 2) targets_dst[gid] = slot[4 + gid];
  if (steps_dst && gid <= n_d_updates) steps_dst[gid] = gid < n_d_updates ? slot[6] + 1.0f + (float)gid : slot[7] + 1.0f;
  for (int i = gid; i < B * To; i += gsz)
    *reinterpret_cast<float2*>(obsv_dst + 2 * (size_t)i) = *reinterpret_cast<const float2*>(obsv + 2 * (size_t)i);
  for (int k = gid; k < B * Tp; k += gsz) {
    const int b = k / Tp, t = k - b * Tp;
    const float2 p = *reinterpret_cast<const float2*>(pred + 2 * (size_t)k);
    const float2 q = *reinterpret_cast<const float2*>(t == 0 ? obsv + ((size_t)b * To + To - 1) * 2 : pred + 2 * (size_t)k - 2);
    *reinterpret_cast<float2*>(pred_dst + 2 * (size_t)k) = p;
    st4(pred4_dst + 4 * (size_t)k, f32x4{p.x, p.y, p.x - q.x, p.y - q.y});
  }
}
#define SW_DIMG_BLOCKS 16
extern "C" int sw_stage_step_zdev(const float* slot, int B, int To, int Tp, float* obsv_dst, float* pred_dst,
                                  float* pred4_dst, float* targets_dst, float* z_dst, float* steps_dst, int n_d_updates,
                                  const float* enc_w, const float* dec_w, const float* emb_w, const float* att_w, float* img,
                                  const float* d_w, float* d_img, const int* d_tab, int z_device, void* stream) {
  if (z_device && !z_dst) return SW_EARG;
  if (!slot || !obsv_dst || !pred_dst || !pred4_dst || !targets_dst || B < 1 || To < 2 || Tp < 1 ||
      n_d_updates < 0 || n_d_updates > 254)
    return SW_EARG;
  if (img && (!enc_w || !dec_w || ((emb_w != nullptr) != (att_w != nullptr)))) return SW_EARG;
  if (d_img && (!d_w || !d_tab || Tp > 64)) return SW_EARG;
  int n = z_dst ? B * SW_Z / 4 : B * (To > Tp ? To : Tp);
  int blocks = (n + 255) / 256;
  if (blocks > 1024) blocks = 1024;
  const int ib = img ? SW_IMG_BLOCKS : 0, db = d_img ? SW_DIMG_BLOCKS : 0;
  SW_LAUNCH(stage_step_kernel, dim3(blocks + ib + db), dim3(256), 0, (hipStream_t)stream, slot, B, To, Tp, obsv_dst,
                     pred_dst, pred4_dst, targets_dst, z_dst, steps_dst, n_d_updates, enc_w, dec_w, emb_w, att_w, img, ib,
                     d_w, d_img, d_tab, d_img ? swp::disc(Tp).n : 0, db, z_device ? 1 : 0);
  SW_CHECK_LAUNCH("stage_step_kernel");
  if (img) gen_images_register(enc_w, dec_w, emb_w, att_w, img);
  if (d_img) sw_disc_images_register(d_w, d_img, d_tab, Tp);
  return SW_OK;
}
extern "C" int sw_stage_step_img(const float* slot, int B, int To, int Tp, float* obsv_dst, float* pred_dst,
                                 float* pred4_dst, float* targets_dst, float* z_dst, float* steps_dst, int n_d_updates,
                                 const float* enc_w, const float* dec_w, const float* emb_w, const float* att_w, float* img,
                                 const float* d_w, float* d_img, const int* d_tab, void* stream) {
  return sw_stage_step_zdev(slot, B, To, Tp, obsv_dst, pred_dst, pred4_dst, targets_dst, z_dst, steps_dst, n_d_updates, enc_w,
                            dec_w, emb_w, att_w, img, d_w, d_img, d_tab, 0, stream);
}
extern "C" int sw_stage_step(const float* slot, int B, int To, int Tp, float* obsv_dst, float* pred_dst,
                             float* pred4_dst, float* targets_dst, float* z_dst, float* steps_dst, int n_d_updates,
                             void* stream) {
  return sw_stage_step_img(slot, B, To, Tp, obsv_dst, pred_dst, pred4_dst, targets_dst, z_dst, steps_dst, n_d_updates, nullptr,
                           nullptr, nullptr, nullptr, nullptr, nullptr, nullptr, nullptr, stream);
}
```

socialways_amd/csrc/sw_wgrad.h:

```cpp
#pragma once
#include <hip/hip_runtime.h>
#include <stddef.h>

#define SW_WG_MAXP 24
#define SW_WG_MAXSPLIT 256
#define SW_WG_WS_FLOATS ((size_t)SW_WG_MAXSPLIT * 65536)

struct WgProblem {
  const float* delta;
  const float* act;
  float* dW;
  float* db;
  float* db2;
  size_t ws_off;
  int ldd, lda, ldw, R, N, K, ones, accumulate;
  int nbn, nbk, nsplit, job0, out0;
  int pre;
  const float* act2;
  float* dW2;
  int lda2, ldw2, K2, row0;
};
struct WgBatch {
  int job0s[SW_WG_MAXP], out0s[SW_WG_MAXP];
  WgProblem p[SW_WG_MAXP];
  int np = 0, total_jobs = 0, total_out = 0;
  size_t top_reserved = 0;
};

struct WgAdam {
  float* w = nullptr;
  float* m = nullptr;
  float* v = nullptr;
  const float* g0 = nullptr;
  const float* step = nullptr;
  double lr = 0, beta1 = 0, beta2 = 0, eps = 0;
  size_t n = ~(size_t)0;
  const float* bc = nullptr;
  float* img = nullptr;
  const int* tab = nullptr;
};
__device__ __forceinline__ void wg_adam_bc_compute(const float* step, double beta1, double beta2, float& bc1, float& bc2s) {
  const float st = *step;
  bc1 = (float)(1 - pow(beta1, (double)st));
  bc2s = (float)sqrt(1 - pow(beta2, (double)st));
}
__device__ __forceinline__ void wg_adam_bc(const WgAdam& A, float& bc1, float& bc2s) {
  if (A.bc) {
    bc1 = A.bc[0];
    bc2s = A.bc[1];
    return;
  }
  wg_adam_bc_compute(A.step, A.beta1, A.beta2, bc1, bc2s);
}
struct WgAdamPre {
  size_t i;
  float m, v, w;
  int2 t;
};
__device__ __forceinline__ WgAdamPre wg_adam_pre(const WgAdam& A, const float* gptr) {
  WgAdamPre s;
  s.i = (size_t)(gptr - A.g0);
  s.t = int2{-1, -1};
  if (s.i >= A.n) {
    s.i = ~(size_t)0;
    s.m = s.v = s.w = 0.f;
    return s;
  }
  s.m = A.m[s.i];
  s.v = A.v[s.i];
  s.w = A.w[s.i];
  if (A.img) s.t = reinterpret_cast<const int2*>(A.tab)[s.i];
  return s;
}
__device__ __forceinline__ void wg_adam_fin(const WgAdam& A, const WgAdamPre& s, float bc1, float bc2s, float grad) {
  if (s.i == ~(size_t)0) return;
  const float m = (float)((double)s.m + (1 - A.beta1) * ((double)grad - (double)s.m));
  const float v = (float)(A.beta2 * s.v + (1 - A.beta2) * grad * grad);
  const float step_size = (float)(A.lr / bc1);
  const float denom = (float)((sqrtf(v) / bc2s) + A.eps);
  A.m[s.i] = m;
  A.v[s.i] = v;
  const float wn = s.w - step_size * m / denom;
  A.w[s.i] = wn;
  if (A.img) {
    if (s.t.x >= 0) A.img[s.t.x] = wn;
    if (s.t.y >= 0) A.img[s.t.y] = wn;
  }
}
__device__ __forceinline__ void wg_adam1(const WgAdam& A, float bc1, float bc2s, const float* gptr, float grad) {
  wg_adam_fin(A, wg_adam_pre(A, gptr), bc1, bc2s, grad);
}
int wg_reduce_launch_adam(WgBatch& b, float* ws, const WgAdam& ad, hipStream_t stream);
int wg_reduce_launch(WgBatch& b, float* ws, hipStream_t stream);
int wg_launch_adam(WgBatch& b, float* ws, WgAdam& ad, hipStream_t stream);

bool wg_shape_ok(int N, int K);
int wg_add(WgBatch& b, const float* delta, int ldd, const float* act, int lda, int R, int N, int K, float* dW,
           int ldw, float* db, float* db2, int accumulate);
int wg_add_tail(WgBatch& b, const float* delta, int ldd, const float* act, int lda, int R, int N, int K, float* dW,
                int ldw, const float* act2, int lda2, int K2, float* dW2, int ldw2, int row0, float* db, float* db2,
                int accumulate);
double wg_total_work(const WgBatch& b);
size_t wg_finalize(WgBatch& b);
int wg_launch(WgBatch& b, float* ws, hipStream_t stream);
int wg_add_pre(WgBatch& b, int N, int K, float* dW, int ldw, float* db, int nslices);
int wg_launch_finalized(WgBatch& b, float* ws, hipStream_t stream);
struct sw_wgrad_batch;
WgBatch* wg_pending(sw_wgrad_batch* h);
```

socialways_amd/csrc/sw_wgrad.hip:

```cpp
#include "../../include/socialways_hip.h"
#include "sw_common.h"
#include "sw_wgrad.h"
#include "sw_wgrad_dev.h"
#include <stdlib.h>

__host__ __device__ inline int wg_grid_jobs(int total_jobs) { return (total_jobs + 31) & ~31; }
#ifdef SW_WG_STAMP
__device__ unsigned long long g_wg_stamps[4 * 4096];
extern "C" int sw_debug_wg_stamps(unsigned long long* host, int n) {
  return hipMemcpyFromSymbol(host, HIP_SYMBOL(g_wg_stamps), sizeof(unsigned long long) * (size_t)n) == hipSuccess ? 0 : -1;
}
#endif
__global__ __launch_bounds__(SW_THREADS, 2) void wgrad_partial_kernel(WgBatch batch, float* __restrict__ ws,
                                                                      const float* __restrict__ adam_step, double beta1,
                                                                      double beta2, float* __restrict__ bc_out) {
  __shared__ __attribute__((aligned(16))) float red[SW_WG_RED_FLOATS];
  if ((int)blockIdx.x >= wg_grid_jobs(batch.total_jobs)) {
    if (threadIdx.x == 0) {
      float bc1, bc2s;
      wg_adam_bc_compute(adam_step, beta1, beta2, bc1, bc2s);
      bc_out[0] = bc1;
      bc_out[1] = bc2s;
    }
    return;
  }
  const int v = blockIdx.x, l = v >> 3;
  const int job = ((((l >> 2) << 3) + (v & 7)) << 2) + (l & 3);
  if (job >= batch.total_jobs) return;
#ifdef SW_WG_STAMP
  const unsigned long long t0 = wall_clock64();
#endif
  wg_job(batch, ws, job, red);
#ifdef SW_WG_STAMP
  if (threadIdx.x == 0 && blockIdx.x < 2048) {
    int p = 0;
    while (p + 1 < batch.np && job >= batch.job0s[p + 1]) ++p;
    unsigned long long* o = g_wg_stamps + (batch.total_jobs < 400 ? 4 * 2048 : 0) + 4 * blockIdx.x;
    o[0] = t0;
    o[1] = wall_clock64();
    o[2] = p;
    o[3] = batch.total_jobs;
  }
#endif
}
__device__ float g_wg_bc[2 * 64];
static float* wg_bc_slot() {
  static float* base[32] = {};
  static unsigned next = 0;
  int dev = -1;
  if (hipGetDevice(&dev) != hipSuccess || dev < 0 || dev >= 32) return nullptr;
  if (!base[dev]) {
    void* p = nullptr;
    if (hipGetSymbolAddress(&p, HIP_SYMBOL(g_wg_bc)) != hipSuccess) {
      (void)hipGetLastError();
      return nullptr;
    }
    base[dev] = (float*)p;
  }
  return base[dev] + 2 * (next++ % 64);
}

#ifndef SW_WG_RSUB
#define SW_WG_RSUB 4
#endif
#define SW_WG_REL (64 / SW_WG_RSUB)
__global__ __launch_bounds__(256) void wgrad_reduce_kernel(WgBatch batch, const float* __restrict__ ws, WgAdam ad) {
  const int gid = blockIdx.x * 256 + threadIdx.x;
  const int lane = gid & 63, el = lane % SW_WG_REL, sub = lane / SW_WG_REL;
  const int i = (gid >> 6) * SW_WG_REL + el;
  bool live = i < batch.total_out;
  int ii = live ? i : batch.total_out - 1;
  int p = 0;
#pragma unroll 1
  while (p + 1 < batch.np && ii >= batch.out0s[p + 1]) ++p;
  const WgProblem& P = batch.p[p];
  const int e = ii - P.out0;
  const int Kc = P.K + P.K2 + P.ones;
  const size_t stride = (size_t)P.N * Kc;
  const float* src = ws + P.ws_off + e;
  const int n = e / Kc, k = e - n * Kc;
  float* dst = k < P.K ? P.dW + (size_t)n * P.ldw + k : k < P.K + P.K2 ? P.dW2 + (size_t)n * P.ldw2 + (k - P.K) : P.db + n;
  float* dst2 = (k >= P.K + P.K2 && P.db2) ? P.db2 + n : nullptr;
  WgAdamPre a1 = {}, a2 = {};
  float old1 = 0.f, old2 = 0.f;
  if (ad.w) {
    a1 = wg_adam_pre(ad, dst);
    if (dst2) a2 = wg_adam_pre(ad, dst2);
  }
  if (P.accumulate) {
    old1 = *dst;
    if (dst2) old2 = *dst2;
  }
  float s = 0.f;
  float s1 = 0.f, s2 = 0.f, s3 = 0.f;
  int q = sub;
  for (; q + 3 * SW_WG_RSUB < P.nsplit; q += 4 * SW_WG_RSUB) {
    s += src[(size_t)q * stride];
    s1 += src[(size_t)(q + SW_WG_RSUB) * stride];
    s2 += src[(size_t)(q + 2 * SW_WG_RSUB) * stride];
    s3 += src[(size_t)(q + 3 * SW_WG_RSUB) * stride];
  }
  for (; q < P.nsplit; q += SW_WG_RSUB) s += src[(size_t)q * stride];
  s = (s + s1) + (s2 + s3);
#pragma unroll
  for (int o = SW_WG_REL; o < 64; o <<= 1) s += __shfl_xor(s, o);
  float bc1 = 1.f, bc2s = 1.f;
  if (ad.w) wg_adam_bc(ad, bc1, bc2s);
  if (!live || sub != 0) return;
  const float g = P.accumulate ? old1 + s : s;
  *dst = g;
  if (ad.w) wg_adam_fin(ad, a1, bc1, bc2s, g);
  if (dst2) {
    const float g2 = P.accumulate ? old2 + s : s;
    *dst2 = g2;
    if (ad.w) wg_adam_fin(ad, a2, bc1, bc2s, g2);
  }
}

bool wg_shape_ok(int N, int K) {
  for (int n0 = 0; n0 < N; n0 += 64)
    if (!wg_tiles(N - n0 < 64 ? N - n0 : 64, false)) return false;
  return K == 0 || wg_tiles(K, true) != 0;
}

static bool wg_span_ok(int R, int ld, int row0) {
  const long long rows = (long long)R / 4 + 4 + 8 * 4 * SW_WG_DEPTH + row0;
  return rows * ld * 4 < (1LL << 31);
}

int wg_add(WgBatch& b, const float* delta, int ldd, const float* act, int lda, int R, int N, int K, float* dW,
           int ldw, float* db, float* db2, int accumulate) {
  if (N > 256 || (ldd & 3) || (lda & 3)) return SW_ESHAPE;
  if (!wg_span_ok(R, ldd, 0) || !wg_span_ok(R, lda, 0)) return SW_ESHAPE;
  if (K < 1) return SW_ESHAPE;
  const int Nfull = N > 64 && (N & 63) && (N & 63) <= 32 && b.np + 2 * ((K + 63) / 64) <= SW_WG_MAXP ? (N & ~63) : N;
  for (int n0 = 0; n0 < N; n0 = (n0 == 0 ? Nfull : N)) {
    const int Nseg = n0 == 0 ? Nfull : N - Nfull;
    for (int c0 = 0; c0 < K; c0 += 64) {
      if (b.np >= SW_WG_MAXP) return SW_ESHAPE;
      const int c1 = c0 + 64 < K ? c0 + 64 : K;
      const bool has_ones = db && c1 == K;
      WgProblem& P = b.p[b.np++];
      P.delta = delta + n0; P.ldd = ldd; P.act = act + c0; P.lda = lda;
      P.R = R; P.N = Nseg; P.K = c1 - c0; P.ones = has_ones ? 1 : 0;
      P.dW = dW + (size_t)n0 * ldw + c0; P.ldw = ldw; P.db = has_ones ? db + n0 : nullptr;
      P.db2 = has_ones && db2 ? db2 + n0 : nullptr;
      P.accumulate = accumulate;
      P.pre = 0;
      P.act2 = nullptr; P.dW2 = nullptr; P.lda2 = P.ldw2 = P.K2 = P.row0 = 0;
      if (!wg_shape_ok(Nseg, P.K)) return SW_ESHAPE;
      P.nbn = (Nseg + 15) / 16;
      P.nbk = P.K > 0 ? wg_tiles(P.K, true) : 1;
    }
  }
  return SW_OK;
}

int wg_add_tail(WgBatch& b, const float* delta, int ldd, const float* act, int lda, int R, int N, int K, float* dW,
                int ldw, const float* act2, int lda2, int K2, float* dW2, int ldw2, int row0, float* db, float* db2,
                int accumulate) {
  if (N > 256 || (ldd & 3) || (lda & 3) || (lda2 & 3) || K != 64 || K2 != 4 || b.np >= SW_WG_MAXP)
    return SW_ESHAPE;
  if (row0 < 0 || !wg_span_ok(R, ldd, 0) || !wg_span_ok(R, lda, row0) || !wg_span_ok(R, lda2, 0)) return SW_ESHAPE;
  WgProblem& P = b.p[b.np++];
  P.delta = delta; P.ldd = ldd; P.act = act; P.lda = lda; P.R = R; P.N = N; P.K = K; P.ones = db ? 1 : 0;
  P.dW = dW; P.ldw = ldw; P.db = db; P.db2 = db ? db2 : nullptr; P.accumulate = accumulate; P.pre = 0;
  P.act2 = act2; P.lda2 = lda2; P.K2 = K2; P.dW2 = dW2; P.ldw2 = ldw2; P.row0 = row0;
  if (!wg_shape_ok(N, K)) return SW_ESHAPE;
  P.nbn = (N + 15) / 16;
  P.nbk = 4;
  return SW_OK;
}

int wg_add_pre(WgBatch& b, int N, int K, float* dW, int ldw, float* db, int nslices) {
  if (b.np >= SW_WG_MAXP || N < 1 || K < 1 || !db || nslices < 1) return SW_ESHAPE;
  WgProblem& P = b.p[b.np++];
  P.delta = nullptr; P.act = nullptr; P.ldd = P.lda = 0; P.R = 0;
  P.N = N; P.K = K; P.ones = 1; P.dW = dW; P.ldw = ldw; P.db = db; P.db2 = nullptr; P.accumulate = 0;
  P.nbn = (N + 15) / 16; P.nbk = (K + 1 + 15) / 16;
  P.act2 = nullptr; P.dW2 = nullptr; P.lda2 = P.ldw2 = P.K2 = P.row0 = 0;
  P.pre = nslices;
  b.top_reserved += (size_t)nslices * N * (K + 1);
  if (b.top_reserved > SW_WG_WS_FLOATS) return SW_ESHAPE;
  P.ws_off = SW_WG_WS_FLOATS - b.top_reserved;
  return SW_OK;
}

#ifndef SW_WG_GROUP_C0
#define SW_WG_GROUP_C0 256.0
#endif
#ifndef SW_WG_ROUND_UP
#define SW_WG_ROUND_UP 0.75
#endif
static double wg_cost(const WgProblem& P) {
  double c = 0;
  for (int n0 = 0; n0 < P.N; n0 += 64) {
    int ni = (P.N - n0 + 15) / 16;
    if (ni > 4) ni = 4;
    double per_group = ni * P.nbk * 32.0 + ni * (P.K2 + P.ones) * 4.0 + SW_WG_GROUP_C0;
    if (per_group < 192.0) per_group = 192.0;
    c += per_group;
  }
  return c * (P.R / 4.0 + 8.0);
}
double wg_total_work(const WgBatch& b) {
  double w = 0;
  for (int i = 0; i < b.np; ++i)
    if (!b.p[i].pre) w += wg_cost(b.p[i]);
  return w;
}

size_t wg_finalize(WgBatch& b) {
  {
    auto key = [](const WgProblem& P) { return P.pre ? 0 : (P.N + 63) / 64; };
    for (int i = 1; i < b.np; ++i) {
      const WgProblem t = b.p[i];
      int j = i;
      for (; j > 0 && key(b.p[j - 1]) < key(t); --j) b.p[j] = b.p[j - 1];
      b.p[j] = t;
    }
  }
  const double total = wg_total_work(b) + 1.0;
  static const double grain = 8192.0 * (1.0 + SW_WG_GROUP_C0 / 512.0);
  double target = total / grain / 4.0;
  if (target < 64.0) target = 64.0;
  const double maxwg = target >= 4096.0 ? 1024.0 : 512.0;
  if (target > maxwg) target = maxwg;
  const double small_env = 256.0;
  const bool one_per_cu = target > 256.0 && target < 448.0;
  if (one_per_cu) target = small_env;
  auto assign = [&](double tgt) {
    size_t ws = 0;
    int job = 0, out = 0;
    for (int i = 0; i < b.np; ++i) {
      WgProblem& P = b.p[i];
      const int NB = (P.N + 63) / 64;
      int ns;
      if (P.pre) {
        ns = P.pre;
      } else {
        const double share = tgt * wg_cost(P) / total / NB;
        ns = (int)(share + (share < 4.0 && maxwg <= 512.0 ? SW_WG_ROUND_UP : 0.5));
        int cap = (P.R + 127) / 128;
        if (ns > cap) ns = cap;
        if (ns > SW_WG_MAXSPLIT) ns = SW_WG_MAXSPLIT;
        if (ns < 1) ns = 1;
      }
      P.nsplit = ns;
      P.job0 = job;
      b.job0s[i] = job;
      b.out0s[i] = out;
      if (!P.pre) job += ns * NB;
      P.out0 = out;
      const int Kc = P.K + P.K2 + P.ones;
      out += P.N * Kc;
      if (!P.pre) {
        P.ws_off = ws;
        ws += (size_t)ns * P.N * Kc;
      }
    }
    b.total_jobs = job;
    b.total_out = out;
    return ws;
  };
  size_t ws = assign(target);
  const int limit = one_per_cu ? (int)small_env : (target >= maxwg ? (int)maxwg : 1 << 30);
  for (double tgt = target - 4.0; b.total_jobs > limit && tgt > 64.0; tgt -= 4.0) ws = assign(tgt);
  return ws + b.top_reserved;
}

struct sw_wgrad_batch {
  WgBatch b;
};
extern "C" sw_wgrad_batch* sw_wgrad_batch_new(void) { return new sw_wgrad_batch(); }
extern "C" void sw_wgrad_batch_free(sw_wgrad_batch* h) { delete h; }
WgBatch* wg_pending(sw_wgrad_batch* h) { return h ? &h->b : nullptr; }

int wg_launch(WgBatch& b, float* ws, hipStream_t stream) {
  if (b.np == 0) return SW_OK;
  size_t need = wg_finalize(b);
  if (need > SW_WG_WS_FLOATS) return SW_ESHAPE;
  return wg_launch_finalized(b, ws, stream);
}

int wg_reduce_launch_adam(WgBatch& b, float* ws, const WgAdam& ad, hipStream_t stream) {
  if (b.total_out == 0) return SW_OK;
  SW_LAUNCH(wgrad_reduce_kernel, dim3((b.total_out * SW_WG_RSUB + 255) / 256), dim3(256), 0, stream, b, ws, ad);
  SW_CHECK_LAUNCH("wgrad_reduce_kernel");
  return SW_OK;
}
int wg_reduce_launch(WgBatch& b, float* ws, hipStream_t stream) { return wg_reduce_launch_adam(b, ws, WgAdam(), stream); }
int wg_launch_adam(WgBatch& b, float* ws, WgAdam& ad, hipStream_t stream) {
  if (b.np == 0) return SW_OK;
  size_t need = wg_finalize(b);
  if (need > SW_WG_WS_FLOATS) return SW_ESHAPE;
  if (b.total_out == 0) return SW_OK;
  ad.bc = nullptr;
  if (b.total_jobs > 0) {
    float* bc = ad.w ? wg_bc_slot() : nullptr;
    SW_LAUNCH(wgrad_partial_kernel, dim3(wg_grid_jobs(b.total_jobs) + (bc ? 1 : 0)), dim3(SW_THREADS), 0, stream, b, ws, ad.step,
                       ad.beta1, ad.beta2, bc);
    SW_CHECK_LAUNCH("wgrad_partial_kernel");
    ad.bc = bc;
  }
  return wg_reduce_launch_adam(b, ws, ad, stream);
}

int wg_launch_finalized(WgBatch& b, float* ws, hipStream_t stream) {
  if (b.total_out == 0) return SW_OK;
  if (b.total_jobs > 0) {
    SW_LAUNCH(wgrad_partial_kernel, dim3(wg_grid_jobs(b.total_jobs)), dim3(SW_THREADS), 0, stream, b, ws, (const float*)nullptr,
                       0.0, 0.0, (float*)nullptr);
    SW_CHECK_LAUNCH("wgrad_partial_kernel");
  }
  return wg_reduce_launch(b, ws, stream);
}
```

socialways_amd/csrc/sw_wgrad_dev.h:

```cpp
#pragma once
#include <type_traits>
#include "sw_common.h"
#include "sw_wgrad.h"
#ifndef SW_WG_DEPTH
#define SW_WG_DEPTH 4
#endif
#ifndef SW_WG_DEPTH5
#define SW_WG_DEPTH5 2
#endif
#ifndef SW_WG_DEPTH_TAIL
#define SW_WG_DEPTH_TAIL SW_WG_DEPTH
#endif

#define SW_WG_RLD 69

typedef __amdgpu_buffer_rsrc_t wg_rsrc;
__device__ __forceinline__ wg_rsrc wg_make_rsrc(const float* base, unsigned bytes) {
  return __builtin_amdgcn_make_buffer_rsrc(const_cast<float*>(base), 0, (int)bytes, 0x00020000);
}
template <int NV>
__device__ __forceinline__ void wg_ldv(float (&v)[NV], wg_rsrc rs, unsigned off) {
  unsigned u[NV];
  if constexpr (NV == 4) {
    const auto q = __builtin_amdgcn_raw_buffer_load_b128(rs, (int)off, 0, 0);
    u[0] = q[0]; u[1] = q[1]; u[2] = q[2]; u[3] = q[3];
  } else if constexpr (NV == 3) {
    const auto q = __builtin_amdgcn_raw_buffer_load_b96(rs, (int)off, 0, 0);
    u[0] = q[0]; u[1] = q[1]; u[2] = q[2];
  } else if constexpr (NV == 2) {
    const auto q = __builtin_amdgcn_raw_buffer_load_b64(rs, (int)off, 0, 0);
    u[0] = q[0]; u[1] = q[1];
  } else {
    u[0] = __builtin_amdgcn_raw_buffer_load_b32(rs, (int)off, 0, 0);
  }
#pragma unroll
  for (int i = 0; i < NV; ++i) v[i] = __uint_as_float(u[i]);
}

__host__ __device__ inline int wg_tiles(int n, bool allow3) {
  if (n <= 16) return 1;
  for (int t = (n + 15) >> 4; t <= 4; ++t)
    if ((t != 3 || allow3) && n % t == 0) return t;
  return 0;
}

template <int NA, int KR, int K2, int ONES, int DSCALE = 1>
__device__ __forceinline__ void wg_run(const float* __restrict__ dbase, const float* __restrict__ abase, int ldd, int lda,
                                       int rbeg, int rend, int acol, int bcol, int lg, int ln,
                                       float* __restrict__ mine,
                                       const float* __restrict__ abase2, int lda2, int row0, int xoff) {
  constexpr int KT = KR, XC = K2 + ONES;
  f32x4 acc[NA][KT];
#pragma unroll
  for (int i = 0; i < NA; ++i) {
#pragma unroll
    for (int kt = 0; kt < KT; ++kt) acc[i][kt] = f32x4{0.f, 0.f, 0.f, 0.f};
  }
  float xacc[NA][XC > 0 ? XC : 1];
#pragma unroll
  for (int i = 0; i < NA; ++i) {
#pragma unroll
    for (int c = 0; c < (XC > 0 ? XC : 1); ++c) xacc[i][c] = 0.f;
  }
  constexpr int DEPTH = (K2 > 0 ? SW_WG_DEPTH_TAIL : SW_WG_DEPTH) * DSCALE;
  float a[DEPTH][NA], b[DEPTH][KT];
  f32x4 xq[DEPTH];
  const int abeg = K2 > 0 ? max(rbeg, row0) : rbeg, aend = max(abeg, rend);
  const wg_rsrc drs = wg_make_rsrc(dbase + (size_t)rbeg * ldd, (unsigned)(rend - rbeg) * (unsigned)ldd * 4u);
  const wg_rsrc ars = wg_make_rsrc(abase + (size_t)abeg * lda, (unsigned)(aend - abeg) * (unsigned)lda * 4u);
  const wg_rsrc xrs = wg_make_rsrc(abase2 + (size_t)rbeg * lda2, (unsigned)(rend - rbeg) * (unsigned)lda2 * 4u);
  unsigned doff = (unsigned)(lg * ldd + acol) * 4u, aoff = (unsigned)((rbeg - abeg + lg) * lda + bcol) * 4u;
  unsigned xoff2 = (unsigned)(lg * lda2) * 4u;
  const unsigned dstep = 16u * (unsigned)ldd, astep = 16u * (unsigned)lda, xstep = 16u * (unsigned)lda2;
  auto load = [&](float (&av)[NA], float (&bv)[KT], f32x4& xv) {
    wg_ldv<NA>(av, drs, doff);
    doff += dstep;
    wg_ldv<KR>(bv, ars, aoff);
    aoff += astep;
    if constexpr (K2 > 0) {
      float x4[4];
      wg_ldv<4>(x4, xrs, xoff2);
      xv = f32x4{x4[0], x4[1], x4[2], x4[3]};
      xoff2 += xstep;
    }
  };
#pragma unroll
  for (int q = 0; q < DEPTH - 1; ++q) load(a[q], b[q], xq[q]);
  for (int r = rbeg; r < rend; r += 4 * DEPTH) {
#pragma unroll
    for (int q = 0; q < DEPTH; ++q) {
      load(a[(q + DEPTH - 1) % DEPTH], b[(q + DEPTH - 1) % DEPTH], xq[(q + DEPTH - 1) % DEPTH]);
      asm volatile("" ::: "memory");
#pragma unroll
      for (int i = 0; i < NA; ++i) asm volatile("" : "+v"(a[q][i]));
#pragma unroll
      for (int kt = 0; kt < KT; ++kt) asm volatile("" : "+v"(b[q][kt]));
      if constexpr (K2 > 0) asm volatile("" : "+v"(xq[q]));
#pragma unroll
      for (int i = 0; i < NA; ++i) {
#pragma unroll
        for (int kt = 0; kt < KT; ++kt) {
          acc[i][kt] = SW_MFMA(a[q][i], b[q][kt], acc[i][kt]);
        }
      }
#pragma unroll
      for (int i = 0; i < NA; ++i) {
        if constexpr (K2 > 0) {
#pragma unroll
          for (int c = 0; c < K2; ++c) xacc[i][c] = fmaf(a[q][i], xq[q][c], xacc[i][c]);
        }
        if constexpr (ONES) xacc[i][K2] += a[q][i];
      }
    }
  }
#pragma unroll
  for (int i = 0; i < NA; ++i) {
#pragma unroll
    for (int kt = 0; kt < KT; ++kt) {
#pragma unroll
      for (int r = 0; r < 4; ++r) {
        const int orow = NA * (4 * lg + r) + i;
        if (KR * ln + kt < xoff) mine[orow * SW_WG_RLD + KR * ln + kt] = acc[i][kt][r];
      }
    }
  }
  if constexpr (XC > 0) {
#pragma unroll
    for (int i = 0; i < NA; ++i) {
#pragma unroll
      for (int c = 0; c < XC; ++c) {
        float v = xacc[i][c];
        v += __shfl_xor(v, 16);
        v += __shfl_xor(v, 32);
        if (lg == 0) mine[(NA * ln + i) * SW_WG_RLD + xoff + c] = v;
      }
    }
  }
}

#define SW_WG_RED_FLOATS (4 * 64 * SW_WG_RLD)
template <int DSCALE = 1>
__device__ __forceinline__ void wg_job(const WgBatch& batch, float* __restrict__ ws, int job, float* red) {
  const int lane = sw_lane(), wave = sw_wave(), ln = lane & 15, lg = lane >> 4;
  int p = 0;
#pragma unroll 1
  while (p + 1 < batch.np && job >= batch.job0s[p + 1]) ++p;
  const WgProblem& P = batch.p[p];
  const int j = job - P.job0;
  const int NB = (P.N + 63) >> 6;
  const int sg = j / NB, nb = j - sg * NB;
  const int s = sg * 4 + wave;
  const int N = P.N, K = P.K, Kc = P.K + P.K2 + P.ones;
  const int n0 = nb * 64;
  const int Nb = min(64, N - n0);
  const int NA = wg_tiles(Nb, false);
  const int KR = K > 0 ? wg_tiles(K, true) : 1;
  const int nsub = P.nsplit * 4;
  const int rows_per = (((P.R + nsub - 1) / nsub) + 3) & ~3;
  const int rbeg = __builtin_amdgcn_readfirstlane(min(P.R, s * rows_per));
  const int rend = __builtin_amdgcn_readfirstlane(min(P.R, rbeg + rows_per));
  const int acol = n0 + max(0, min(NA * ln, Nb - NA));
  const int bcol = max(0, min(KR * ln, K - KR));
  float* mine = red + wave * 64 * SW_WG_RLD;
#define WG_CASE(na, kr, k2, on)                                                                                     \
  case ((na * 8 + kr) * 2 + (k2 ? 1 : 0)) * 2 + on:                                                                 \
    wg_run<na, kr, k2, on, DSCALE>(P.delta, P.act, P.ldd, P.lda, rbeg, rend, acol, bcol, lg, ln,                      \
                                   mine, P.act2 ? P.act2 : P.delta, P.act2 ? P.lda2 : P.ldd, P.row0, K);            \
    break;
#define WG_CASES(na)                                                                                                \
  WG_CASE(na, 1, 0, 0) WG_CASE(na, 2, 0, 0) WG_CASE(na, 3, 0, 0) WG_CASE(na, 4, 0, 0)                               \
  WG_CASE(na, 1, 0, 1) WG_CASE(na, 2, 0, 1) WG_CASE(na, 3, 0, 1) WG_CASE(na, 4, 0, 1)                               \
  WG_CASE(na, 4, 4, 0) WG_CASE(na, 4, 4, 1)
  switch (((NA * 8 + KR) * 2 + (P.K2 ? 1 : 0)) * 2 + (P.ones ? 1 : 0)) {
    WG_CASES(1) WG_CASES(2) WG_CASES(4)
  }
#undef WG_CASES
#undef WG_CASE
  sw_barrier();
  float* out = ws + P.ws_off + (size_t)sg * N * Kc;
  const int rows = min(64, N - n0), cols = min(SW_WG_RLD, Kc);
  const int dq = SW_THREADS / cols, dr = SW_THREADS - dq * cols;
  int rr = threadIdx.x / cols, cc = threadIdx.x - rr * cols;
  const float* r0 = red, *r1 = red + 64 * SW_WG_RLD, *r2 = red + 2 * 64 * SW_WG_RLD, *r3 = red + 3 * 64 * SW_WG_RLD;
  for (int e = threadIdx.x; e < rows * cols; e += SW_THREADS) {
    const int o = rr * SW_WG_RLD + cc;
    const float v = (r0[o] + r1[o]) + (r2[o] + r3[o]);
    out[(size_t)(n0 + rr) * Kc + cc] = v;
    cc += dr;
    rr += dq;
    if (cc >= cols) {
      cc -= cols;
      ++rr;
    }
  }
}
```

socialways_amd/ops.py:

```python
import os

import numpy as np
import torch

from . import _lib as L
from .data import check_obs_len


class SceneIndex:

    def __init__(self, sub_batches, B, device):
        sb = np.asarray(sub_batches, dtype=np.int64).reshape(-1, 2)
        if len(sb) == 0:
            sb = np.array([[0, B]], dtype=np.int64)
        if sb[0, 0] != 0 or sb[-1, 1] != B or (sb[1:, 0] != sb[:-1, 1]).any():
            raise ValueError("sub_batches must tile [0, B) contiguously")
        n = sb[:, 1] - sb[:, 0]
        if (n <= 0).any():
            raise ValueError("empty scene in sub_batches")
        self.S = len(sb)
        self.B = int(B)
        small = n <= L.AMAX
        self.amax = int(n[small].max()) if small.any() else 0
        pairs = np.where((n > 1) & small, n * n, 0)
        recs, row = [], 0
        for sc in np.nonzero(~small)[0]:
            ns = int(n[sc])
            nblk = (ns + 15) // 16
            for k in range(nblk):
                recs.append((sc, 16 * k, row + k * ns, row, nblk, k, 0, 0))
            row += nblk * ns
        self.NB, self.big_rows = len(recs), row
        self.big_blocks = torch.tensor(recs, dtype=torch.int32).reshape(-1, 8).to(device) if recs else None
        poff = np.concatenate([[0], np.cumsum(pairs)]).astype(np.int64)
        self.P = int(poff[-1])
        off = np.concatenate([sb[:, 0], [B]]).astype(np.int32)
        self.scene_off = torch.from_numpy(off).to(device)
        self.pair_off = torch.from_numpy(poff).to(device)
        self.sizes = n

    _cache = {}

    @classmethod
    def get(cls, sub_batches, B, device):
        sb = np.ascontiguousarray(np.asarray(sub_batches, dtype=np.int64))
        key = (sb.tobytes(), int(B), str(device))
        hit = cls._cache.get(key)
        if hit is None:
            if len(cls._cache) > 4096:
                cls._cache.clear()
            hit = cls._cache[key] = cls(sb, B, device)
            hit.key = key
        return hit


class Workspaces:

    def __init__(self, device):
        self.device = device
        self.buf = {}
        self._wgb = None
        self.retired = []
        self.version = 0

    @property
    def wgrad_batch(self):
        if self._wgb is None:
            lib = L.load()
            self._wgb, self._free = lib.sw_wgrad_batch_new(), lib.sw_wgrad_batch_free
        return self._wgb

    def __del__(self):
        if getattr(self, "_wgb", None):
            self._free(self._wgb)
            self._wgb = None

    def get(self, name, nfloats):
        t = self.buf.get(name)
        if t is None or t.numel() < nfloats:
            if t is not None:
                self.retired.append(t)
                self.version += 1
            n = max(int(nfloats), 1) if t is None else max(int(nfloats), int(1.25 * t.numel()))
            t = torch.empty(n, dtype=torch.float32, device=self.device)
            self.buf[name] = t
        return t

    def release_retired(self):
        self.retired.clear()


_default_ws = {}


def default_ws(device):
    key = str(device)
    if key not in _default_ws:
        _default_ws[key] = Workspaces(device)
    return _default_ws[key]


class GenCtx:
    __slots__ = ("obsv", "noise", "scenes", "hT", "cT", "S", "attn", "gsave", "B", "To", "Tp", "use_social", "wh", "ml")


def gen_forward(enc_w, emb_w, att_w, dec_w, obsv, noise, scenes, n_next, use_social, save, ws=None, tag="g", ade=None,
                noise_src=None, d_obs=None):
    L.require_gpu(obsv)
    obsv = obsv.contiguous()
    noise = noise.contiguous()
    B, To = obsv.shape[0], obsv.shape[1]
    if noise.shape != (B, 32):
        raise ValueError("noise must be (B, 32)")
    dev = obsv.device
    st = L.stream()
    hT = torch.empty(B, 64, device=dev)
    cT = torch.empty(B, 64, device=dev)
    pred4 = torch.empty(B, n_next, 4, device=dev)
    gsave = None
    if save:
        nfl = L.workspace_floats(L.WS_GSAVE, B, To, n_next)
        gsave = ws.get(tag + ".gsave", nfl) if ws is not None else torch.empty(nfl, device=dev)
    x4s_off = (To + n_next - 1) * B * 384
    z_in_enc, z_in_soc, n_enc = noise_src, None, noise.numel() if noise_src else 0
    L.call("sw_enc_lstm_fwd_aux", L.ptr(obsv), 0, L.ptr(enc_w), None, None, B, To, L.ptr(hT), L.ptr(cT), None,
           L.ptr(gsave), (gsave.data_ptr() + 4 * x4s_off) if save else None, 0,
           z_in_enc, L.ptr(noise) if z_in_enc else None, n_enc, st)
    attn = wh = ml = None
    if use_social:
        S = torch.empty(B, 64, device=dev)
        attn = torch.empty(B, L.AMAX, device=dev) if save else None
        if scenes.NB:
            wh = torch.empty(B * 132, device=dev)
            ml = torch.empty(B, 2, device=dev) if save else None
        L.call("sw_social_pool_fwd_aux", L.ptr(obsv), To, L.ptr(hT), L.ptr(scenes.scene_off), scenes.S, B, scenes.amax,
               L.ptr(emb_w), L.ptr(att_w), L.ptr(S), L.ptr(attn), L.ptr(scenes.big_blocks), scenes.NB, L.ptr(wh), L.ptr(ml),
               z_in_soc, (noise.data_ptr() + 4 * n_enc) if z_in_soc else None, (noise.numel() - n_enc) if z_in_soc else 0, st)
    else:
        S = torch.zeros(B, 64, device=dev)
    L.call("sw_dec_rollout_fwd_aux", L.ptr(obsv), To, L.ptr(noise), L.ptr(S), L.ptr(hT), L.ptr(cT), L.ptr(enc_w),
           L.ptr(dec_w), B, n_next, L.ptr(pred4), None, None, L.ptr(gsave),
           L.ptr(ade[0]) if ade else None, float(ade[1]) if ade else 0.0, L.ptr(ade[2]) if ade else None,
           L.ptr(d_obs[0]) if d_obs else None, L.ptr(d_obs[1]) if d_obs else None, st)
    if not save:
        return pred4, None
    ctx = GenCtx()
    ctx.obsv, ctx.noise, ctx.scenes, ctx.hT, ctx.cT, ctx.S, ctx.attn = obsv, noise, scenes, hT, cT, S, attn
    ctx.gsave, ctx.B, ctx.To, ctx.Tp, ctx.use_social = gsave, B, To, n_next, use_social
    ctx.wh, ctx.ml = wh, ml
    return pred4, ctx


DFUSE = True


def gen_backward(enc_w, emb_w, att_w, dec_w, ctx, dpred4, d_enc, d_emb, d_att, d_dec, ws=None, tag="g", aux=None, adam=None,
                 dfuse=None):
    dev = ctx.obsv.device
    ws = ws or default_ws(dev)
    B, To, Tp = ctx.B, ctx.To, ctx.Tp
    gdelta = ws.get(tag + ".gdelta", L.workspace_floats(L.WS_GDELTA, B, To, Tp))
    wgrad = ws.get("wgrad", L.workspace_floats(L.WS_WGRAD, B, To, Tp))
    tmp = ws.get(tag + ".dwx", 2048)
    dhT = torch.empty(B, 64, device=dev)
    dcT = torch.empty(B, 64, device=dev)
    dS = torch.empty(B, 64, device=dev)
    aux_late = None
    if dfuse is not None:
        d_w, pred_hat, targets, t_idx, z, g_label, g_code, loss_part = dfuse
        dscr = ws.get(tag + ".dpred", B * Tp * 4)
        L.call("sw_dec_rollout_bwd_dfuse", L.ptr(ctx.obsv), L.ptr(pred_hat), L.ptr(d_w), L.ptr(targets), int(t_idx), L.ptr(z),
               g_label, g_code, L.ptr(loss_part), L.ptr(dscr), L.ptr(enc_w), L.ptr(dec_w), L.ptr(ctx.gsave), B, To, Tp,
               L.ptr(gdelta), L.ptr(dhT), L.ptr(dcT), L.ptr(dS), L.stream())
        aux_late = aux
    else:
        dpred4 = dpred4.contiguous()
        L.call("sw_dec_rollout_bwd_aux", L.ptr(dpred4), L.ptr(enc_w), L.ptr(dec_w), L.ptr(ctx.gsave), B, To, Tp,
               L.ptr(gdelta), L.ptr(dhT), L.ptr(dcT), L.ptr(dS), L.ptr(aux[0]) if aux else None, L.ptr(aux[1]) if aux else None,
               L.ptr(aux[2]) if aux else None, aux[1].numel() if aux else 0, L.stream())
    pending = None
    if ctx.use_social and (ctx.scenes.P > 0 or ctx.scenes.NB > 0):
        sc = ctx.scenes
        pending = ws.wgrad_batch
        pws = ws.get("pairs", L.workspace_floats(L.WS_PAIRS, B, To, Tp, 1, sc.P))
        bigp = ws.get("bigpart", sc.big_rows * 132) if sc.NB else None
        L.call("sw_social_pool_bwd", L.ptr(ctx.obsv), To, L.ptr(ctx.hT), L.ptr(sc.scene_off), L.ptr(sc.pair_off), sc.S,
               B, sc.amax, sc.P, L.ptr(emb_w), L.ptr(att_w), L.ptr(ctx.attn), L.ptr(dS), L.ptr(dhT), L.ptr(d_emb),
               L.ptr(d_att), L.ptr(pws), L.ptr(wgrad), L.ptr(sc.big_blocks), sc.NB, L.ptr(ctx.wh), L.ptr(ctx.ml),
               L.ptr(ctx.S), L.ptr(bigp), pending, L.stream())
    else:
        d_emb.zero_()
        d_att.zero_()
    L.call("sw_enc_lstm_bwd_aux", L.ptr(enc_w), L.ptr(ctx.gsave), None, L.ptr(dhT), L.ptr(dcT), None, B, To, 0,
           L.ptr(gdelta), None, None, L.ptr(aux_late[0]) if aux_late else None, L.ptr(aux_late[1]) if aux_late else None,
           L.ptr(aux_late[2]) if aux_late else None, aux_late[1].numel() if aux_late else 0, L.stream())
    if adam is not None:
        w_all, g_all, m, v, step, lr, b1, b2, eps = adam
        L.call("sw_gen_wgrad_adam", L.ptr(enc_w), L.ptr(dec_w), L.ptr(ctx.gsave), L.ptr(gdelta), L.ptr(ctx.noise), L.ptr(ctx.S),
               B, To, Tp, L.ptr(d_enc), L.ptr(d_dec), L.ptr(wgrad), L.ptr(tmp), pending, L.ptr(w_all), L.ptr(m), L.ptr(v),
               L.ptr(g_all), w_all.numel(), L.ptr(step), lr, b1, b2, eps, L.stream())
        return
    L.call("sw_gen_wgrad", L.ptr(enc_w), L.ptr(dec_w), L.ptr(ctx.gsave), L.ptr(gdelta), L.ptr(ctx.noise), L.ptr(ctx.S), B, To, Tp,
           L.ptr(d_enc), L.ptr(d_dec), 0, L.ptr(wgrad), L.ptr(tmp), pending, L.stream())


class GenCtxK:
    __slots__ = ("one", "K", "obsv_k", "noise_k", "S_k", "gsave_k")


def gen_forward_k(enc_w, emb_w, att_w, dec_w, obsv, noise_k, scenes, n_next, use_social, K, ws, tag="gv"):
    L.require_gpu(obsv)
    obsv = obsv.contiguous()
    noise_k = noise_k.contiguous()
    B, To = obsv.shape[0], obsv.shape[1]
    KB = K * B
    if noise_k.shape != (KB, 32):
        raise ValueError("noise must be (K * B, 32)")
    dev = obsv.device
    st = L.stream()
    hT, cT = torch.empty(B, 64, device=dev), torch.empty(B, 64, device=dev)
    gsave_1 = ws.get(tag + ".gsave1", L.workspace_floats(L.WS_GSAVE, B, To, n_next))
    gsave_k = ws.get(tag + ".gsave", L.workspace_floats(L.WS_GSAVE, KB, To, n_next))
    Ta = To + n_next - 1
    L.call("sw_enc_lstm_fwd_aux", L.ptr(obsv), 0, L.ptr(enc_w), None, None, B, To, L.ptr(hT), L.ptr(cT), None,
           L.ptr(gsave_1), gsave_1.data_ptr() + 4 * Ta * B * 384, 0, None, None, 0, st)
    attn = wh = ml = None
    if use_social:
        S = torch.empty(B, 64, device=dev)
        attn = torch.empty(B, L.AMAX, device=dev)
        if scenes.NB:
            wh, ml = torch.empty(B * 132, device=dev), torch.empty(B, 2, device=dev)
        L.call("sw_social_pool_fwd_aux", L.ptr(obsv), To, L.ptr(hT), L.ptr(scenes.scene_off), scenes.S, B, scenes.amax,
               L.ptr(emb_w), L.ptr(att_w), L.ptr(S), L.ptr(attn), L.ptr(scenes.big_blocks), scenes.NB, L.ptr(wh), L.ptr(ml),
               None, None, 0, st)
    else:
        S = torch.zeros(B, 64, device=dev)
    obsv_k, hT_k, cT_k, S_k = obsv.repeat(K, 1, 1), hT.repeat(K, 1), cT.repeat(K, 1), S.repeat(K, 1)
    row = gsave_1[(To - 1) * B * 384: To * B * 384].view(1, B, 384)
    gsave_k[(To - 1) * KB * 384: To * KB * 384].view(K, B, 384).copy_(row.expand(K, B, 384))
    pred4 = torch.empty(KB, n_next, 4, device=dev)
    L.call("sw_dec_rollout_fwd_aux", L.ptr(obsv_k), To, L.ptr(noise_k), L.ptr(S_k), L.ptr(hT_k), L.ptr(cT_k), L.ptr(enc_w),
           L.ptr(dec_w), KB, n_next, L.ptr(pred4), None, None, L.ptr(gsave_k), None, 0.0, None, None, None, st)
    one = GenCtx()
    one.obsv, one.noise, one.scenes, one.hT, one.cT, one.S, one.attn = obsv, noise_k[:B], scenes, hT, cT, S, attn
    one.gsave, one.B, one.To, one.Tp, one.use_social, one.wh, one.ml = gsave_1, B, To, n_next, use_social, wh, ml
    ctx = GenCtxK()
    ctx.one, ctx.K, ctx.obsv_k, ctx.noise_k, ctx.S_k, ctx.gsave_k = one, K, obsv_k, noise_k, S_k, gsave_k
    return pred4, ctx


def gen_backward_k(enc_w, emb_w, att_w, dec_w, ctx, dpred4_k, d_enc, d_emb, d_att, d_dec, ws, tag="gv", aux=None):
    one, K = ctx.one, ctx.K
    dev = dpred4_k.device
    B, To, Tp = one.B, one.To, one.Tp
    KB = K * B
    dpred4_k = dpred4_k.contiguous()
    gdelta_k = ws.get(tag + ".gdelta", L.workspace_floats(L.WS_GDELTA, KB, To, Tp))
    gdelta_1 = ws.get(tag + ".gdelta1", L.workspace_floats(L.WS_GDELTA, B, To, Tp))
    wgrad = ws.get("wgrad", L.workspace_floats(L.WS_WGRAD, B, To, Tp))
    tmp = ws.get(tag + ".dwx", 2048)
    dh_k, dc_k, dS_k = (torch.empty(KB, 64, device=dev) for _ in range(3))
    L.call("sw_dec_rollout_bwd_aux", L.ptr(dpred4_k), L.ptr(enc_w), L.ptr(dec_w), L.ptr(ctx.gsave_k), KB, To, Tp,
           L.ptr(gdelta_k), L.ptr(dh_k), L.ptr(dc_k), L.ptr(dS_k), L.ptr(aux[0]) if aux else None,
           L.ptr(aux[1]) if aux else None, L.ptr(aux[2]) if aux else None, aux[1].numel() if aux else 0, L.stream())
    dhT, dcT, dS = (t.view(K, B, 64).sum(0) for t in (dh_k, dc_k, dS_k))
    L.call("sw_gen_wgrad", L.ptr(enc_w), L.ptr(dec_w), L.ptr(ctx.gsave_k), L.ptr(gdelta_k), L.ptr(ctx.noise_k), L.ptr(ctx.S_k),
           KB, To, Tp, L.ptr(d_enc), L.ptr(d_dec), 1, L.ptr(wgrad), L.ptr(tmp), None, L.stream())
    pending = None
    if one.use_social and (one.scenes.P > 0 or one.scenes.NB > 0):
        sc = one.scenes
        pending = ws.wgrad_batch
        pws = ws.get("pairs", L.workspace_floats(L.WS_PAIRS, B, To, Tp, 1, sc.P))
        bigp = ws.get("bigpart", sc.big_rows * 132) if sc.NB else None
        L.call("sw_social_pool_bwd", L.ptr(one.obsv), To, L.ptr(one.hT), L.ptr(sc.scene_off), L.ptr(sc.pair_off), sc.S,
               B, sc.amax, sc.P, L.ptr(emb_w), L.ptr(att_w), L.ptr(one.attn), L.ptr(dS), L.ptr(dhT), L.ptr(d_emb),
               L.ptr(d_att), L.ptr(pws), L.ptr(wgrad), L.ptr(sc.big_blocks), sc.NB, L.ptr(one.wh), L.ptr(one.ml),
               L.ptr(one.S), L.ptr(bigp), pending, L.stream())
    else:
        d_emb.zero_()
        d_att.zero_()
    L.call("sw_enc_lstm_bwd", L.ptr(enc_w), L.ptr(one.gsave), None, L.ptr(dhT), L.ptr(dcT), None, B, To, 0,
           L.ptr(gdelta_1), None, None, L.stream())
    L.call("sw_gen_wgrad", L.ptr(enc_w), L.ptr(dec_w), L.ptr(one.gsave), L.ptr(gdelta_1), L.ptr(one.noise), L.ptr(one.S), B, To, Tp,
           L.ptr(d_enc), L.ptr(d_dec), 2, L.ptr(wgrad), L.ptr(tmp), pending, L.stream())


def obs_len_arg(obs_len, B, To, lo, device):
    if obs_len is None:
        return None
    if isinstance(obs_len, torch.Tensor) and obs_len.device.type != "cpu":
        if obs_len.dtype not in (torch.int32, torch.int64, torch.int16, torch.int8, torch.uint8):
            raise ValueError("obs_len must hold integers, got dtype %s" % obs_len.dtype)
        if tuple(obs_len.shape) != (B,):
            raise ValueError("obs_len must be (B,) = (%d,), got %s" % (B, tuple(obs_len.shape)))
        return obs_len.to(device=device, dtype=torch.int32).contiguous()
    host = obs_len.numpy() if isinstance(obs_len, torch.Tensor) else obs_len
    return torch.from_numpy(check_obs_len(host, B, To, lo)).to(device)


def _check_obs_len_tensor(obs_len, B, device):
    if not isinstance(obs_len, torch.Tensor) or obs_len.dtype != torch.int32 or tuple(obs_len.shape) != (B,) \
            or obs_len.device != device:
        raise ValueError("obs_len must be an int32 tensor (B,) = (%d,) on %s" % (B, device))
    return obs_len.contiguous()


_sample_img = {}


def gen_sample(enc_w, emb_w, att_w, dec_w, obsv, noise_k, scenes, n_next, use_social, K, gt=None, inv_ss=1.0,
               want_pred=True, keep_pred=False, obs_len=None):
    L.require_gpu(obsv)
    obsv = obsv.contiguous()
    noise_k = noise_k.contiguous()
    B, To = obsv.shape[0], obsv.shape[1]
    if K < 1:
        raise ValueError("K must be at least 1")
    if noise_k.shape != (K * B, 32):
        raise ValueError("noise must be (K * B, 32)")
    want_pred = want_pred or keep_pred
    if gt is None and not want_pred:
        raise ValueError("nothing asked for: neither trajectories nor errors")
    if gt is not None:
        gt = gt.contiguous()
        if gt.shape != (B, n_next, 2):
            raise ValueError("gt must be (B, n_next, 2)")
    dev = obsv.device
    if obs_len is not None:
        obs_len = _check_obs_len_tensor(obs_len, B, dev)
    st = L.stream()
    pred4 = torch.empty(K * B, n_next, 4, device=dev) if want_pred else None
    if B == 0:
        return pred4, None
    img = _sample_img.get(str(dev))
    if img is None:
        img = _sample_img[str(dev)] = torch.empty(L.load().sw_gen_image_floats(), device=dev)
    hT, cT = torch.empty(B, 64, device=dev), torch.empty(B, 64, device=dev)
    err = torch.empty(K, B, 2, device=dev) if gt is not None else None
    L.call("sw_gen_images", L.ptr(enc_w), L.ptr(dec_w), L.ptr(emb_w), L.ptr(att_w), L.ptr(img), st)
    try:
        if obs_len is None:
            L.call("sw_enc_lstm_fwd_aux", L.ptr(obsv), 0, L.ptr(enc_w), None, None, B, To, L.ptr(hT), L.ptr(cT), None,
                   None, None, 0, None, None, 0, st)
        else:
            L.call("sw_enc_lstm_fwd_ragged", L.ptr(obsv), 0, L.ptr(enc_w), L.ptr(obs_len), B, To, L.ptr(hT), L.ptr(cT), st)
        S = None
        if use_social:
            S = torch.empty(B, 64, device=dev)
            wh = torch.empty(B * 132, device=dev) if scenes.NB else None
            L.call("sw_social_pool_fwd_aux", L.ptr(obsv), To, L.ptr(hT), L.ptr(scenes.scene_off), scenes.S, B, scenes.amax,
                   L.ptr(emb_w), L.ptr(att_w), L.ptr(S), None, L.ptr(scenes.big_blocks), scenes.NB, L.ptr(wh), None,
                   None, None, 0, st)
        L.call("sw_dec_sample_fwd", L.ptr(obsv), To, L.ptr(noise_k), L.ptr(S), L.ptr(hT), L.ptr(cT), L.ptr(enc_w),
               L.ptr(dec_w), B, K, n_next, L.ptr(pred4), L.ptr(gt), float(inv_ss), L.ptr(err), st)
    finally:
        L.call("sw_gen_images", None, None, None, None, None, None)
    if err is None:
        return pred4, None
    per_agent = torch.empty(B, 4, device=dev)
    best = torch.empty(B, dtype=torch.int32, device=dev)
    L.call("sw_sample_reduce", L.ptr(err), B, K, L.ptr(per_agent), L.ptr(best), st)
    return pred4, (per_agent, best, err)


def scene_clearance(pos, start, scenes, K, inv_ss=1.0):
    L.require_gpu(pos)
    pos = pos.contiguous()
    Tp, pstride, B = pos.shape[-2], pos.shape[-1], scenes.B
    if pstride not in (2, 4) or pos.numel() != K * B * Tp * pstride:
        raise ValueError("pos must be (K * B, Tp, 2 or 4) with K = %d, B = %d, got %s" % (K, B, tuple(pos.shape)))
    sstride = 0
    if start is not None:
        if start.dim() != 2 or start.shape[0] != B or start.shape[1] < 2 or start.device != pos.device:
            raise ValueError("start must be (B, >= 2) on the device of pos, got %s" % (tuple(start.shape),))
        if start.dtype != torch.float32 or start.stride(1) != 1 or start.stride(0) < 2:
            start = start[:, :2].float().contiguous()
        sstride = start.stride(0)
    clear = torch.empty(K, B, device=pos.device)
    L.call("sw_scene_clearance", L.ptr(pos), pstride, L.ptr_strided(start), sstride, L.ptr(scenes.scene_off), scenes.S, B, K,
           Tp, float(inv_ss), L.ptr(clear), L.stream())
    return clear


def scene_reduce(err, clear, scenes, K, coll_dist):
    L.require_gpu(err)
    err = err.contiguous()
    B = scenes.B
    if err.numel() != K * B * 2 or (clear is not None and tuple(clear.shape) != (K, B)):
        raise ValueError("err must be (K, B, 2) and clear (K, B)")
    per_scene = torch.empty(scenes.S, 6, device=err.device)
    kbest = torch.empty(scenes.S, dtype=torch.int32, device=err.device)
    L.call("sw_scene_reduce", L.ptr(err), L.ptr(clear), L.ptr(scenes.scene_off), scenes.S, B, K, float(coll_dist),
           L.ptr(per_scene), L.ptr(kbest), L.stream())
    return per_scene, kbest


def scene_metrics(err, pred4, obsv, scenes, K, n_next, inv_ss, coll_dist):
    if pred4.shape[-2] != n_next:
        raise ValueError("pred4 must hold n_next = %d steps" % n_next)
    clear = scene_clearance(pred4, obsv[:, -1], scenes, K, inv_ss)
    per_scene, kbest = scene_reduce(err, clear, scenes, K, coll_dist)
    return per_scene, kbest, clear


class DiscCtx:
    __slots__ = ("dsave", "B", "To", "Tp", "nb")


D_OBS_MAX_TILES = 128


def d_obs_buffer(ws, B, To, Tp, nb=2, tag="d"):
    if (B + 15) // 16 > D_OBS_MAX_TILES:
        return None
    return ws.get(tag + ".dsave", L.workspace_floats(L.WS_DSAVE, B, To, Tp, nb))


def disc_forward(d_w, obsv, preds, save, ws=None, tag="d", save_lstm=True, w_snapshot=None):
    L.require_gpu(obsv)
    obsv = obsv.contiguous()
    preds = [p.contiguous() for p in preds]
    B, To = obsv.shape[0], obsv.shape[1]
    x_mode = {2: 0, 4: 1}[obsv.shape[2]]
    Tp = preds[0].shape[1]
    nb = len(preds)
    dev = obsv.device
    labels = [torch.empty(B, 1, device=dev) for _ in preds]
    codes = [torch.empty(B, 2, device=dev) for _ in preds]
    dsave = None
    if save:
        nfl = L.workspace_floats(L.WS_DSAVE, B, To, Tp, nb)
        dsave = ws.get(tag + ".dsave", nfl) if ws is not None else torch.empty(nfl, device=dev)
    pp, _k1 = L.ptr_array(preds)
    lp, _k2 = L.ptr_array(labels)
    cp, _k3 = L.ptr_array(codes)
    L.call("sw_disc_fwd", L.ptr(obsv), To, x_mode, pp, nb, L.ptr(d_w), B, Tp, lp, cp, L.ptr(dsave), int(save_lstm),
           L.ptr(w_snapshot), L.stream())
    if not save:
        return labels, codes, None
    ctx = DiscCtx()
    ctx.dsave, ctx.B, ctx.To, ctx.Tp, ctx.nb = dsave, B, To, Tp, nb
    return labels, codes, ctx


def disc_score(d_w, obsv, pred4, K, want_code=True, obs_len=None):
    if K < 1:
        raise ValueError("K must be at least 1")
    if obsv.dim() != 3 or obsv.shape[2] not in (2, 4) or (obsv.shape[2] == 2 and obsv.shape[1] < 2) or obsv.shape[1] < 1:
        raise ValueError("obsv must be (B, To >= 2, 2) or (B, To >= 1, 4), got %s" % (tuple(obsv.shape),))
    B, To = obsv.shape[0], obsv.shape[1]
    if pred4.dim() not in (3, 4) or pred4.shape[-1] != 4 or pred4.shape[-2] < 1 or pred4.numel() != K * B * pred4.shape[-2] * 4 \
            or (pred4.dim() == 4 and tuple(pred4.shape[:2]) != (K, B)):
        raise ValueError("pred4 must be (K * B, Tp, 4) or (K, B, Tp, 4) with K = %d, B = %d, got %s" % (K, B, tuple(pred4.shape)))
    if pred4.device != obsv.device:
        raise ValueError("pred4 must be on the device of obsv")
    L.require_gpu(obsv)
    if obs_len is not None:
        obs_len = _check_obs_len_tensor(obs_len, B, obsv.device)
    obsv, pred4 = obsv.float().contiguous(), pred4.float().contiguous()
    Tp = pred4.shape[-2]
    score = torch.empty(K, B, device=obsv.device)
    code = torch.empty(K, B, 2, device=obsv.device) if want_code else None
    if B == 0:
        return score, code
    x_mode = {2: 0, 4: 1}[obsv.shape[2]]
    if obs_len is None:
        L.call("sw_disc_score", L.ptr(obsv), To, x_mode, L.ptr(pred4), L.ptr(d_w), B, K, Tp, L.ptr(score), L.ptr(code), L.stream())
    else:
        L.call("sw_disc_score_ragged", L.ptr(obsv), To, x_mode, L.ptr(obs_len), L.ptr(pred4), L.ptr(d_w), B, K, Tp, L.ptr(score),
               L.ptr(code), L.stream())
    return score, code


RANK_MAX_K = 4096


def _check_picks(score, K, M, err, best):
    if score.dim() != 2 or score.shape[0] != K or K < 1:
        raise ValueError("score must be (K, B) with K = %d >= 1, got %s" % (K, tuple(score.shape)))
    B = score.shape[1]
    if not 1 <= M <= K:
        raise ValueError("M must lie in 1 .. K = %d, got %d" % (K, M))
    if K > RANK_MAX_K:
        raise ValueError("K must be at most %d, got %d" % (RANK_MAX_K, K))
    if err is not None and (tuple(err.shape) != (K, B, 2) or err.device != score.device):
        raise ValueError("err must be (K, B, 2) = (%d, %d, 2) on the device of score, got %s" % (K, B, tuple(err.shape)))
    if best is not None:
        if err is None:
            raise ValueError("best is only used with err")
        if tuple(best.shape) != (B,) or best.dtype != torch.int32 or best.device != score.device:
            raise ValueError("best must be (B,) = (%d,) int32 on the device of score, got %s %s" % (B, tuple(best.shape), best.dtype))
        best = best.contiguous()
    return B, best


def sample_rank(score, K, M, err=None, best=None):
    B, best = _check_picks(score, K, M, err, best)
    L.require_gpu(score)
    score = score.float().contiguous()
    order = torch.empty(B, M, dtype=torch.int32, device=score.device)
    per_agent = None
    if err is not None:
        err = err.float().contiguous()
        per_agent = torch.empty(B, 5, device=score.device)
    if B == 0:
        return order, per_agent
    L.call("sw_sample_rank", L.ptr(score), L.ptr(err), L.ptr(best), B, K, M, L.ptr(order), L.ptr(per_agent), L.stream())
    return order, per_agent


NMS_METRICS = {"fde": 0, "ade": 1}


def sample_nms(pos, score, K, M, radius, metric="fde", scenes=None, inv_ss=1.0, err=None, best=None):
    B, best = _check_picks(score, K, M, err, best)
    if metric not in NMS_METRICS:
        raise ValueError("metric must be one of %s, got %r" % (sorted(NMS_METRICS), metric))
    if not float(radius) >= 0.0:
        raise ValueError("radius must be >= 0, got %r" % (radius,))
    if not float(inv_ss) > 0.0:
        raise ValueError("inv_ss must be > 0, got %r" % (inv_ss,))
    if pos.dim() not in (3, 4) or pos.shape[-1] not in (2, 4) or pos.shape[-2] < 1 \
            or pos.numel() != K * B * pos.shape[-2] * pos.shape[-1] or (pos.dim() == 4 and tuple(pos.shape[:2]) != (K, B)):
        raise ValueError("pos must be (K * B, Tp, 2 or 4) or (K, B, Tp, 2 or 4) with K = %d, B = %d, got %s" % (K, B, tuple(pos.shape)))
    if pos.device != score.device:
        raise ValueError("pos must be on the device of score")
    if scenes is not None and scenes.B != B:
        raise ValueError("scenes index %d rows, score has B = %d" % (scenes.B, B))
    L.require_gpu(score)
    score, pos = score.float().contiguous(), pos.float().contiguous()
    dev = score.device
    G = scenes.S if scenes is not None else B
    order = torch.empty(G, M, dtype=torch.int32, device=dev)
    count = torch.empty(G, dtype=torch.int32, device=dev)
    weight = torch.empty(G, M, device=dev)
    assign = torch.empty(G, K, dtype=torch.int32, device=dev)
    per_row = None
    if err is not None:
        err = err.float().contiguous()
        per_row = torch.empty(B, 6, device=dev)
    if B == 0:
        return order, count, weight, assign, per_row
    L.call("sw_sample_nms", L.ptr(pos), pos.shape[-1], L.ptr(score), L.ptr(scenes.scene_off) if scenes is not None else None,
           G if scenes is not None else 0, B, K, pos.shape[-2], M, NMS_METRICS[metric], float(inv_ss), float(radius), L.ptr(err),
           L.ptr(best), L.ptr(order), L.ptr(count), L.ptr(weight), L.ptr(assign), L.ptr(per_row), L.stream())
    return order, count, weight, assign, per_row


def disc_backward(d_w, ctx, dlabels, dcodes, d_d_w=None, want_dpred=(), ws=None, tag="d"):
    dev = dlabels[0].device
    ws = ws or default_ws(dev)
    B, To, Tp, nb = ctx.B, ctx.To, ctx.Tp, ctx.nb
    dlabels = [t.contiguous() for t in dlabels]
    dcodes = [t.contiguous() for t in dcodes]
    want = list(want_dpred) + [False] * (nb - len(want_dpred))
    dpreds = [torch.empty(B, Tp, 4, device=dev) if w else None for w in want]
    ddelta = wgrad = None
    if d_d_w is not None:
        ddelta = ws.get(tag + ".ddelta", L.workspace_floats(L.WS_DDELTA, B, To, Tp, nb))
        wgrad = ws.get("wgrad", L.workspace_floats(L.WS_WGRAD, B, To, Tp))
    lp, _k1 = L.ptr_array(dlabels)
    cp, _k2 = L.ptr_array(dcodes)
    dp, _k3 = L.ptr_array(dpreds)
    L.call("sw_disc_bwd", L.ptr(d_w), L.ptr(ctx.dsave), lp, cp, nb, B, To, Tp, L.ptr(ddelta), L.ptr(d_d_w), dp,
           L.ptr(wgrad), L.stream())
    return dpreds


def disc_dpred(d_w, obsv, pred_hat, targets, t_idx, z, g_label, g_code, loss_part=None):
    L.require_gpu(obsv)
    obsv, pred_hat = obsv.contiguous(), pred_hat.contiguous()
    B, To, Tp = obsv.shape[0], obsv.shape[1], pred_hat.shape[1]
    x_mode = {2: 0, 4: 1}[obsv.shape[2]]
    dpred = torch.empty(B, Tp, 4, device=obsv.device)
    L.call("sw_disc_dpred", L.ptr(obsv), To, x_mode, L.ptr(pred_hat), L.ptr(d_w), B, Tp, L.ptr(targets), int(t_idx), L.ptr(z),
           g_label, g_code, L.ptr(dpred), None, None, L.ptr(loss_part), L.stream())
    return dpred


def disc_dpred_supported(Tp):
    return bool(L.load().sw_disc_dpred_supported(int(Tp)))


def disc_backward_gan(d_w, ctx, labels, codes, targets, t_idx, z, g_label, g_code, d_d_w=None, want_dpred=(), ws=None,
                      tag="d", loss_part=None, adam=None):
    dev = labels[0].device
    ws = ws or default_ws(dev)
    B, To, Tp, nb = ctx.B, ctx.To, ctx.Tp, ctx.nb
    want = list(want_dpred) + [False] * (nb - len(want_dpred))
    dpreds = [torch.empty(B, Tp, 4, device=dev) if w else None for w in want]
    ddelta = wgrad = None
    if d_d_w is not None:
        ddelta = ws.get(tag + ".ddelta", L.workspace_floats(L.WS_DDELTA, B, To, Tp, nb))
        wgrad = ws.get("wgrad", L.workspace_floats(L.WS_WGRAD, B, To, Tp))
    lp, _k1 = L.ptr_array(labels)
    cp, _k2 = L.ptr_array(codes)
    dp, _k3 = L.ptr_array(dpreds)
    t0, t1 = (list(t_idx) + [0])[:2]
    if adam is not None:
        m, v, step, lr, b1, b2, eps = adam
        L.call("sw_disc_bwd_gan_adam", L.ptr(d_w), L.ptr(ctx.dsave), lp, cp, L.ptr(targets), t0, t1, L.ptr(z), g_label, g_code,
               nb, B, To, Tp, L.ptr(ddelta), L.ptr(d_d_w), dp, L.ptr(wgrad), L.ptr(loss_part), L.ptr(d_w), L.ptr(m), L.ptr(v),
               L.ptr(step), float(lr), float(b1), float(b2), float(eps), L.stream())
        return dpreds
    L.call("sw_disc_bwd_gan", L.ptr(d_w), L.ptr(ctx.dsave), lp, cp, L.ptr(targets), t0, t1, L.ptr(z), g_label, g_code, nb,
           B, To, Tp, L.ptr(ddelta), L.ptr(d_d_w), dp, L.ptr(wgrad), L.ptr(loss_part), L.stream())
    return dpreds


def disc_update_supported(d_w, B, To, Tp):
    return bool(L.load().sw_disc_update_supported(L.ptr(d_w), int(B), int(To), int(Tp)))


def disc_update(d_w, obsv, preds, targets, t_idx, z, g_label, g_code, d_d_w, ws, tag="d", obs_pre=False, w_snapshot=None,
                loss_part=None, adam=None):
    L.require_gpu(obsv)
    obsv = obsv.contiguous()
    preds = [p.contiguous() for p in preds]
    B, To, Tp = obsv.shape[0], obsv.shape[1], preds[0].shape[1]
    dev = obsv.device
    labels = [torch.empty(B, 1, device=dev) for _ in preds]
    codes = [torch.empty(B, 2, device=dev) for _ in preds]
    dsave = ws.get(tag + ".dsave", L.workspace_floats(L.WS_DSAVE, B, To, Tp, 2))
    ddelta = ws.get(tag + ".ddelta", L.workspace_floats(L.WS_DDELTA, B, To, Tp, 2))
    wgrad = ws.get("wgrad", L.workspace_floats(L.WS_WGRAD, B, To, Tp))
    pp, _k1 = L.ptr_array(preds)
    lp, _k2 = L.ptr_array(labels)
    cp, _k3 = L.ptr_array(codes)
    m = v = step = None
    lr = b1 = b2 = eps = 0.0
    if adam is not None:
        m, v, step, lr, b1, b2, eps = adam
    L.call("sw_disc_update", L.ptr(obsv), To, pp, L.ptr(d_w), B, Tp, lp, cp, L.ptr(dsave), int(bool(obs_pre)), L.ptr(w_snapshot),
           L.ptr(targets), int(t_idx[0]), int(t_idx[1]), L.ptr(z), g_label, g_code, L.ptr(ddelta), L.ptr(d_d_w), L.ptr(wgrad),
           L.ptr(loss_part), L.ptr(d_w) if adam is not None else None, L.ptr(m), L.ptr(v), L.ptr(step), float(lr), float(b1),
           float(b2), float(eps), L.stream())
    return labels, codes
```

Baseline: 2817 steps/s.

## Fold generator wgrad split-K reduction into the weight compose and Adam kernel

Adds a combined kernel that reduces the split-K partial sums for the LSTM input and decoder-head weight gradients and composes them into the final encoder and decoder parameter gradients. Optional Adam updates happen in the same launch. Previously this took a separate reduce launch followed by a compose launch. The generic reduction is reworked with sub-lane slice sums and shuffle reductions, and the fold is on by default through a WFOLD flag, with an unfolded entry point kept as a fallback. This saves a kernel launch and a global round trip of intermediate gradients. In exchange it adds complex pattern-matching on problem descriptors and extra workgroups that do redundant reads.

After: 2712 steps/s. 0.963x the previous value.

```diff
diff --git a/include/socialways_hip.h b/include/socialways_hip.h
--- a/include/socialways_hip.h
+++ b/include/socialways_hip.h
@@ -136,6 +136,11 @@
                       float* wgrad_ws, float* tmp , sw_wgrad_batch* pending , float* adam_w,
                       float* adam_m, float* adam_v, const float* adam_g, long long adam_n, const float* adam_step,
                       double lr, double beta1, double beta2, double eps, void* stream);
+int sw_gen_wgrad_unfolded(const float* enc_w, const float* dec_w, const float* gsave, const float* gdelta,
+                          const float* z, const float* S_pool, int B, int To, int Tp, float* d_enc_w, float* d_dec_w,
+                          int part, float* wgrad_ws, float* tmp , sw_wgrad_batch* pending ,
+                          float* adam_w , float* adam_m, float* adam_v, const float* adam_g, long long adam_n,
+                          const float* adam_step, double lr, double beta1, double beta2, double eps, void* stream);
 
 int sw_disc_fwd(const float* obsv, int To, int x_mode, const float* const* pred4 ,
                 int nb, const float* d_w, int B, int Tp, float* const* label ,
diff --git a/socialways_amd/_lib.py b/socialways_amd/_lib.py
--- a/socialways_amd/_lib.py
+++ b/socialways_amd/_lib.py
@@ -45,6 +45,9 @@
     "sw_gen_wgrad": (_i, [_vp, _vp, _vp, _vp, _vp, _vp, _i, _i, _i, _vp, _vp, _i, _vp, _vp, _vp, _vp]),
     "sw_gen_wgrad_adam": (_i, [_vp, _vp, _vp, _vp, _vp, _vp, _i, _i, _i, _vp, _vp, _vp, _vp, _vp, _vp, _vp, _vp, _vp,
                                ctypes.c_longlong, _vp, ctypes.c_double, ctypes.c_double, ctypes.c_double, ctypes.c_double, _vp]),
+    "sw_gen_wgrad_unfolded": (_i, [_vp, _vp, _vp, _vp, _vp, _vp, _i, _i, _i, _vp, _vp, _i, _vp, _vp, _vp, _vp, _vp, _vp, _vp,
+                                   ctypes.c_longlong, _vp, ctypes.c_double, ctypes.c_double, ctypes.c_double, ctypes.c_double,
+                                   _vp]),
     "sw_enc_lstm_bwd_aux": (_i, [_vp, _vp, _vp, _vp, _vp, _vp, _i, _i, _i, _vp, _vp, _vp, _vp, _vp, _vp, _ll, _vp]),
     "sw_dec_rollout_bwd_dfuse": (_i, [_vp, _vp, _vp, _vp, _i, _vp, _f, _f, _vp, _vp, _vp, _vp, _vp, _i, _i, _i, _vp, _vp, _vp, _vp,
                                       _vp]),
diff --git a/socialways_amd/csrc/sw_misc.hip b/socialways_amd/csrc/sw_misc.hip
--- a/socialways_amd/csrc/sw_misc.hip
+++ b/socialways_amd/csrc/sw_misc.hip
@@ -3,6 +3,7 @@
 #include "sw_lstm_dev.h"
 #include <stdlib.h>
 #include "sw_wgrad.h"
+#include "sw_wgrad_dev.h"
 #include <stdio.h>
 #include <string.h>
 
@@ -209,6 +210,35 @@
 }
 
 #define SW_DEC_COMPOSE_BLOCKS 13
+template <class Put>
+__device__ __forceinline__ void compose_dec_elem(const int o, const float* __restrict__ M, const float* __restrict__ sv,
+                                                 const float* __restrict__ W3, const float* __restrict__ W4,
+                                                 const float* __restrict__ b3, float* __restrict__ d_dec_w, Put put) {
+  using namespace swp;
+  if (o < 3200) {
+    const int m = o / 80, k = o - m * 80;
+    put(d_dec_w + DEC_W3 + o, fmaf(W4[m], M[k], W4[40 + m] * M[80 + k]));
+  } else if (o < 3240) {
+    const int m = o - 3200;
+    put(d_dec_w + DEC_B3 + m, fmaf(W4[m], sv[0], W4[40 + m] * sv[1]));
+  } else if (o < 3320) {
+    const int c = (o - 3240) / 40, m = (o - 3240) - c * 40;
+    float v = sv[c] * b3[m];
+    for (int k = 0; k < 80; ++k) v = fmaf(M[c * 80 + k], W3[m * 80 + k], v);
+    put(d_dec_w + DEC_W4 + c * 40 + m, v);
+  } else if (o < 3322) {
+    put(d_dec_w + DEC_B4 + (o - 3320), sv[o - 3320]);
+  }
+}
+template <class Put>
+__device__ __forceinline__ void compose_wih_elem(const int i, const f32x4 g, const float dbx_row, const float* __restrict__ We,
+                                                 const float* __restrict__ be, float* __restrict__ d_enc_w, Put put) {
+  const int e = i & 63;
+  const f32x4 w = ld4(We + e * 4);
+  float v = dbx_row * be[e];
+  v = fmaf(g[0], w[0], v); v = fmaf(g[1], w[1], v); v = fmaf(g[2], w[2], v); v = fmaf(g[3], w[3], v);
+  put(d_enc_w + swp::ENC_WIH + i, v);
+}
 __device__ __forceinline__ void compose_bwd_block(const int blk, const float* __restrict__ enc_w,
                                                   const float* __restrict__ dWx, const float* __restrict__ dbx,
                                                   float* __restrict__ d_enc_w, const float* __restrict__ dec_w,
@@ -222,26 +252,10 @@
     if (ad.w) wg_adam1(ad, bc1, bc2s, dst, g);
   };
   if (blk >= 128) {
-    const int o = (blk - 128) * 256 + threadIdx.x;
-    const float* M = Ms;
-    const float* sv = Ms + 160;
     const float* W3 = snap ? snap + swimg::RAW_W3 : dec_w + DEC_W3;
     const float* W4 = snap ? snap + swimg::RAW_W4 : dec_w + DEC_W4;
     const float* b3 = snap ? snap + swimg::RAW_B3 : dec_w + DEC_B3;
-    if (o < 3200) {
-      const int m = o / 80, k = o - m * 80;
-      put(d_dec_w + DEC_W3 + o, fmaf(W4[m], M[k], W4[40 + m] * M[80 + k]));
-    } else if (o < 3240) {
-      const int m = o - 3200;
-      put(d_dec_w + DEC_B3 + m, fmaf(W4[m], sv[0], W4[40 + m] * sv[1]));
-    } else if (o < 3320) {
-      const int c = (o - 3240) / 40, m = (o - 3240) - c * 40;
-      float v = sv[c] * b3[m];
-      for (int k = 0; k < 80; ++k) v = fmaf(M[c * 80 + k], W3[m * 80 + k], v);
-      put(d_dec_w + DEC_W4 + c * 40 + m, v);
-    } else if (o < 3322) {
-      put(d_dec_w + DEC_B4 + (o - 3320), sv[o - 3320]);
-    }
+    compose_dec_elem((blk - 128) * 256 + threadIdx.x, Ms , Ms + 160 , W3, W4, b3, d_dec_w, put);
     return;
   }
   const float* We = snap ? snap + swimg::RAW_WE : enc_w + ENC_EMB_W;
@@ -250,11 +264,8 @@
   const int t = threadIdx.x;
   if (blk < 64) {
     int i = blk * 256 + t;
-    int row = i >> 6, e = i & 63;
-    f32x4 g = ld4(dWx + row * 4), w = ld4(We + e * 4);
-    float v = dbx[row] * be[e];
-    v = fmaf(g[0], w[0], v); v = fmaf(g[1], w[1], v); v = fmaf(g[2], w[2], v); v = fmaf(g[3], w[3], v);
-    put(d_enc_w + ENC_WIH + i, v);
+    int row = i >> 6;
+    compose_wih_elem(i, ld4(dWx + row * 4), dbx[row], We, be, d_enc_w, put);
     if (blk == 0) {
       put(d_enc_w + ENC_BIH + t, dbx[t]);
       put(d_enc_w + ENC_BHH + t, dbx[t]);
@@ -295,10 +306,133 @@
   compose_bwd_block((int)blockIdx.x + block0, enc_w, dWx, dbx, d_enc_w, dec_w, Ms, d_dec_w, WgAdam(), nullptr);
 }
 
+#define SW_FOLD_THREADS 1024
+#define SW_FOLD_ENC_WGS 8
+#define SW_FOLD_DEC_WGS 4
+struct GenFold {
+  WgFold f;
+  const float* enc_w;
+  const float* dec_w;
+  const float* snap;
+  const float* old;
+  float* d_enc_w;
+  float* d_dec_w;
+  float* tmp;
+};
+__device__ __forceinline__ float mul_unfused(float a, float b) {
+#pragma clang fp contract(off)
+  float r = a * b;
+  asm volatile("" : "+v"(r));
+  return r;
+}
+__global__ __launch_bounds__(SW_FOLD_THREADS, 8) void wgrad_reduce_compose_kernel(WgBatch batch, const float* __restrict__ ws,
+                                                                               WgAdam ad, GenFold gf) {
+  using namespace swp;
+  constexpr int NF = SW_FOLD_ENC_WGS + SW_FOLD_DEC_WGS;
+  const int blk = blockIdx.x, t = threadIdx.x;
+  if (blk >= NF) {
+    wg_reduce_thread<true>(batch, ws, ad, (blk - NF) * SW_FOLD_THREADS + t, gf.f);
+    return;
+  }
+  __shared__ float sg[1280];
+  const int lane = t & 63, wave = t >> 6, el = lane % SW_WG_REL, sub = lane / SW_WG_REL;
+  float bc1 = 1.f, bc2s = 1.f;
+  auto put = [&](float* dst, float g) {
+    *dst = g;
+    if (ad.w) wg_adam1(ad, bc1, bc2s, dst, g);
+  };
+  if (blk < SW_FOLD_ENC_WGS) {
+    const WgProblem& P = batch.p[gf.f.p_lstm];
+    const int Kc = P.K + 5;
+    constexpr int NE = 1280 * SW_WG_RSUB / SW_FOLD_THREADS;
+    const unsigned stride = (unsigned)(P.N * Kc) * 4u;
+    const wg_rsrc rs = wg_make_rsrc(ws + P.ws_off, (unsigned)P.nsplit * stride);
+    unsigned off[NE];
+#pragma unroll
+    for (int j = 0; j < NE; ++j) {
+      const int idx = (j * (SW_FOLD_THREADS / 64) + wave) * SW_WG_REL + el, row = idx / 5;
+      off[j] = (unsigned)(row * Kc + P.K + (idx - row * 5)) * 4u + (unsigned)sub * stride;
+    }
+    float sum[NE];
+    wg_slice_sums<NE>([&](int j, int k) {
+      return __uint_as_float(__builtin_amdgcn_raw_buffer_load_b32(rs, (int)off[j], (int)((unsigned)k * stride), 0)); },
+      P.nsplit, sub, sum);
+    if (sub == 0) {
+#pragma unroll
+      for (int j = 0; j < NE; ++j) {
+        const int idx = (j * (SW_FOLD_THREADS / 64) + wave) * SW_WG_REL + el, row = idx / 5, c = idx - row * 5;
+        const float g = P.accumulate ? gf.old[c < 4 ? row * 4 + c : 1024 + row] + sum[j] : sum[j];
+        sg[idx] = g;
+        if (row / (256 / SW_FOLD_ENC_WGS) == blk) *(c < 4 ? P.dW2 + (size_t)row * P.ldw2 + c : P.db + row) = g;
+      }
+    }
+    __syncthreads();
+    if (ad.w) wg_adam_bc(ad, bc1, bc2s);
+    const float* We = gf.snap ? gf.snap + swimg::RAW_WE : gf.enc_w + ENC_EMB_W;
+    const float* be = gf.snap ? gf.snap + swimg::RAW_BE : gf.enc_w + ENC_EMB_B;
+    const float* Wih = gf.snap ? gf.snap + swimg::RAW_WIH : gf.enc_w + ENC_WIH;
+    constexpr int ROWS = 256 / SW_FOLD_ENC_WGS;
+#pragma unroll
+    for (int u = 0; u < ROWS * 64 / SW_FOLD_THREADS; ++u) {
+      const int i = blk * ROWS * 64 + u * SW_FOLD_THREADS + t, row = i >> 6;
+      compose_wih_elem(i, f32x4{sg[row * 5], sg[row * 5 + 1], sg[row * 5 + 2], sg[row * 5 + 3]}, sg[row * 5 + 4], We, be,
+                       gf.d_enc_w, put);
+    }
+    if (wave < 64 / SW_FOLD_ENC_WGS) {
+      const int e = blk * (64 / SW_FOLD_ENC_WGS) + wave;
+      float w[4];
+#pragma unroll
+      for (int j = 0; j < 4; ++j) w[j] = Wih[(lane + 64 * j) * 64 + e];
+      float mine = 0.f;
+#pragma unroll
+      for (int c = 0; c < 5; ++c) {
+        float x[4];
+#pragma unroll
+        for (int j = 0; j < 4; ++j) x[j] = mul_unfused(w[j], sg[(lane + 64 * j) * 5 + c]);
+        float v = (x[0] + x[2]) + (x[1] + x[3]);
+#pragma unroll
+        for (int o = 32; o > 0; o >>= 1) v += __shfl_xor(v, o);
+        if (lane == c) mine = v;
+      }
+      if (lane < 4) put(gf.d_enc_w + ENC_EMB_W + e * 4 + lane, mine);
+      if (lane == 4) put(gf.d_enc_w + ENC_EMB_B + e, mine);
+    } else if (t - 64 * (64 / SW_FOLD_ENC_WGS) < ROWS) {
+      const int row = blk * ROWS + t - 64 * (64 / SW_FOLD_ENC_WGS);
+      put(gf.d_enc_w + ENC_BIH + row, sg[row * 5 + 4]);
+      put(gf.d_enc_w + ENC_BHH + row, sg[row * 5 + 4]);
+    }
+    return;
+  }
+  float* sm = sg;
+  float* dM = gf.tmp + 1280;
+  const int d = blk - SW_FOLD_ENC_WGS;
+  if (gf.f.p_m0 >= 0) {
+    const bool second = wave >= 8;
+    const WgProblem& P = batch.p[second ? gf.f.p_m1 : gf.f.p_m0];
+    const int Kc = P.K + P.ones, nel = P.N * Kc;
+    const int e0 = (wave - (second ? 8 : 0)) * SW_WG_REL + el, e = min(e0, nel - 1);
+    const float sum[1] = {wg_slice_sum1(ws + P.ws_off + e, (size_t)nel, P.nsplit, sub)};
+    if (sub == 0 && e0 < nel && wave < 11) {
+      const int n = e / Kc, k = e - n * Kc;
+      float* dst = k < P.K ? P.dW + (size_t)n * P.ldw + k : P.db + n;
+      sm[dst - dM] = sum[0];
+      if (d == 0) *dst = sum[0];
+    }
+  } else if (t < 162) {
+    sm[t] = dM[t];
+  }
+  __syncthreads();
+  if (ad.w) wg_adam_bc(ad, bc1, bc2s);
+  const float* W3 = gf.snap ? gf.snap + swimg::RAW_W3 : gf.dec_w + DEC_W3;
+  const float* W4 = gf.snap ? gf.snap + swimg::RAW_W4 : gf.dec_w + DEC_W4;
+  const float* b3 = gf.snap ? gf.snap + swimg::RAW_B3 : gf.dec_w + DEC_B3;
+  compose_dec_elem(d * SW_FOLD_THREADS + t, sm, sm + 160, W3, W4, b3, gf.d_dec_w, put);
+}
+
 static int gen_wgrad_impl(const float* enc_w, const float* dec_w, const float* gsave, const float* gdelta, const float* z,
                           const float* S_pool, int B, int To, int Tp, float* d_enc_w, float* d_dec_w, int part,
                           float* wgrad_ws, float* tmp, sw_wgrad_batch* pending, void* stream, WgAdam ad,
-                          const float* snap) {
+                          const float* snap, bool fold) {
   if (!enc_w || !dec_w || !gsave || !gdelta || !z || !S_pool || !d_enc_w || !d_dec_w || !wgrad_ws || !tmp || B < 1 || To < 2 ||
       Tp < 1 || part < 0 || part > 2)
     return SW_EARG;
@@ -317,7 +451,7 @@
   }
   int rc_add = 0;
   const int t_lo = part == 1 ? To : 0, t_hi = part == 2 ? To : Ta;
-  const int acc = part == 2 ? 1 : 0;
+  const int acc = part == 2 && Ta > To ? 1 : 0;
   if (t_hi > t_lo)
     rc_add |= wg_add_tail(wb, gdelta + gd.dgates + (size_t)t_lo * B * 256, 256,
                           gsave + gs.act + ((ptrdiff_t)t_lo - 1) * B * 384 + 320, 384, (t_hi - t_lo) * B, 256, 64,
@@ -333,6 +467,29 @@
     rc_add |= wg_add(wb, gdelta + gd.dv, 4, gsave + gs.a2, 80, Tp * B, 2, 80, dM, 80, dM + 160, nullptr, 0);
   }
   if (rc_add) return SW_ESHAPE;
+  if (fold && part != 1) {
+    const size_t need = wg_finalize(wb);
+    if (need > SW_WG_WS_FLOATS) return SW_ESHAPE;
+    GenFold gf;
+    for (int i = 0; i < wb.np; ++i) {
+      const WgProblem& P = wb.p[i];
+      if (P.pre) continue;
+      if (P.dW2 == dWx && P.db == dbx && !P.db2 && P.N == 256 && P.K2 == 4 && P.ones && P.ldw2 == 4) gf.f.p_lstm = i;
+      if (P.dW == dM && P.N == 2 && P.K == 64 && !P.ones && P.ldw == 80 && !P.accumulate) gf.f.p_m0 = i;
+      if (P.dW == dM + 64 && P.N == 2 && P.K == 16 && P.db == dM + 160 && !P.db2 && P.ldw == 80 && !P.accumulate) gf.f.p_m1 = i;
+    }
+    float* old = wgrad_ws + (need - wb.top_reserved);
+    const bool room = !acc || need + 1280 <= SW_WG_WS_FLOATS;
+    if (gf.f.p_lstm >= 0 && (gf.f.p_m0 >= 0) == (part == 0) && (gf.f.p_m1 >= 0) == (part == 0) && wb.total_jobs > 0 && room) {
+      if (int rc = wg_partial_launch(wb, wgrad_ws, ad, acc ? tmp : nullptr, acc ? old : nullptr, acc ? 1280 : 0, st)) return rc;
+      gf.enc_w = enc_w; gf.dec_w = dec_w; gf.snap = snap; gf.old = old; gf.d_enc_w = d_enc_w; gf.d_dec_w = d_dec_w; gf.tmp = tmp;
+      const int regular = (wb.total_out * SW_WG_RSUB + SW_FOLD_THREADS - 1) / SW_FOLD_THREADS;
+      SW_LAUNCH(wgrad_reduce_compose_kernel, dim3(SW_FOLD_ENC_WGS + SW_FOLD_DEC_WGS + regular), dim3(SW_FOLD_THREADS), 0, st, wb,
+                         wgrad_ws, ad, gf);
+      SW_CHECK_LAUNCH("wgrad_reduce_compose_kernel");
+      return SW_OK;
+    }
+  }
   if (int rc = ad.w ? wg_launch_adam(wb, wgrad_ws, ad, st) : wg_launch(wb, wgrad_ws, st)) return rc;
   if (part != 1) {
     SW_LAUNCH(enc_compose_bwd_kernel, dim3(128 + SW_DEC_COMPOSE_BLOCKS), dim3(256), 0, st, enc_w, dWx, dbx, d_enc_w,
@@ -345,13 +502,13 @@
                             const float* S_pool, int B, int To, int Tp, float* d_enc_w, float* d_dec_w, int part,
                             float* wgrad_ws, float* tmp, sw_wgrad_batch* pending, void* stream) {
   return gen_wgrad_impl(enc_w, dec_w, gsave, gdelta, z, S_pool, B, To, Tp, d_enc_w, d_dec_w, part, wgrad_ws, tmp, pending,
-                        stream, WgAdam(), nullptr);
-}
-extern "C" int sw_gen_wgrad_adam(const float* enc_w, const float* dec_w, const float* gsave, const float* gdelta,
-                                 const float* z, const float* S_pool, int B, int To, int Tp, float* d_enc_w, float* d_dec_w,
-                                 float* wgrad_ws, float* tmp, sw_wgrad_batch* pending, float* adam_w, float* adam_m,
-                                 float* adam_v, const float* adam_g, long long adam_n, const float* adam_step, double lr,
-                                 double beta1, double beta2, double eps, void* stream) {
+                        stream, WgAdam(), nullptr, true);
+}
+static int gen_wgrad_adam_impl(const float* enc_w, const float* dec_w, const float* gsave, const float* gdelta, const float* z,
+                               const float* S_pool, int B, int To, int Tp, float* d_enc_w, float* d_dec_w, float* wgrad_ws,
+                               float* tmp, sw_wgrad_batch* pending, float* adam_w, float* adam_m, float* adam_v,
+                               const float* adam_g, long long adam_n, const float* adam_step, double lr, double beta1,
+                               double beta2, double eps, void* stream, bool fold) {
   if (!adam_w || !adam_m || !adam_v || !adam_g || !adam_step || adam_n < 1 || !enc_w || !dec_w || !d_enc_w || !d_dec_w)
     return SW_EARG;
   if (enc_w - adam_w != d_enc_w - adam_g || dec_w - adam_w != d_dec_w - adam_g || enc_w < adam_w ||
@@ -363,7 +520,27 @@
   ad.w = adam_w; ad.m = adam_m; ad.v = adam_v; ad.g0 = adam_g; ad.step = adam_step; ad.n = (size_t)adam_n;
   ad.lr = lr; ad.beta1 = beta1; ad.beta2 = beta2; ad.eps = eps;
   return gen_wgrad_impl(enc_w, dec_w, gsave, gdelta, z, S_pool, B, To, Tp, d_enc_w, d_dec_w, 0, wgrad_ws, tmp, pending, stream,
-                        ad, img);
+                        ad, img, fold);
+}
+extern "C" int sw_gen_wgrad_adam(const float* enc_w, const float* dec_w, const float* gsave, const float* gdelta,
+                                 const float* z, const float* S_pool, int B, int To, int Tp, float* d_enc_w, float* d_dec_w,
+                                 float* wgrad_ws, float* tmp, sw_wgrad_batch* pending, float* adam_w, float* adam_m,
+                                 float* adam_v, const float* adam_g, long long adam_n, const float* adam_step, double lr,
+                                 double beta1, double beta2, double eps, void* stream) {
+  return gen_wgrad_adam_impl(enc_w, dec_w, gsave, gdelta, z, S_pool, B, To, Tp, d_enc_w, d_dec_w, wgrad_ws, tmp, pending, adam_w,
+                             adam_m, adam_v, adam_g, adam_n, adam_step, lr, beta1, beta2, eps, stream, true);
+}
+extern "C" int sw_gen_wgrad_unfolded(const float* enc_w, const float* dec_w, const float* gsave, const float* gdelta,
+                                     const float* z, const float* S_pool, int B, int To, int Tp, float* d_enc_w, float* d_dec_w,
+                                     int part, float* wgrad_ws, float* tmp, sw_wgrad_batch* pending, float* adam_w,
+                                     float* adam_m, float* adam_v, const float* adam_g, long long adam_n,
+                                     const float* adam_step, double lr, double beta1, double beta2, double eps, void* stream) {
+  if (!adam_w)
+    return gen_wgrad_impl(enc_w, dec_w, gsave, gdelta, z, S_pool, B, To, Tp, d_enc_w, d_dec_w, part, wgrad_ws, tmp, pending,
+                          stream, WgAdam(), nullptr, false);
+  if (part != 0) return SW_EARG;
+  return gen_wgrad_adam_impl(enc_w, dec_w, gsave, gdelta, z, S_pool, B, To, Tp, d_enc_w, d_dec_w, wgrad_ws, tmp, pending, adam_w,
+                             adam_m, adam_v, adam_g, adam_n, adam_step, lr, beta1, beta2, eps, stream, false);
 }
 
 extern "C" int sw_enc_lstm_wgrad(const float* enc_w, const float* act, const float* x4s, const float* h0, const float* dgates,
diff --git a/socialways_amd/csrc/sw_wgrad.h b/socialways_amd/csrc/sw_wgrad.h
--- a/socialways_amd/csrc/sw_wgrad.h
+++ b/socialways_amd/csrc/sw_wgrad.h
@@ -93,6 +93,7 @@
 int wg_reduce_launch_adam(WgBatch& b, float* ws, const WgAdam& ad, hipStream_t stream);
 int wg_reduce_launch(WgBatch& b, float* ws, hipStream_t stream);
 int wg_launch_adam(WgBatch& b, float* ws, WgAdam& ad, hipStream_t stream);
+int wg_partial_launch(WgBatch& b, float* ws, WgAdam& ad, const float* cp_src, float* cp_dst, int cp_n, hipStream_t stream);
 
 bool wg_shape_ok(int N, int K);
 int wg_add(WgBatch& b, const float* delta, int ldd, const float* act, int lda, int R, int N, int K, float* dW,
diff --git a/socialways_amd/csrc/sw_wgrad.hip b/socialways_amd/csrc/sw_wgrad.hip
--- a/socialways_amd/csrc/sw_wgrad.hip
+++ b/socialways_amd/csrc/sw_wgrad.hip
@@ -6,17 +6,23 @@
 
 __host__ __device__ inline int wg_grid_jobs(int total_jobs) { return (total_jobs + 31) & ~31; }
 #ifdef SW_WG_STAMP
-__device__ unsigned long long g_wg_stamps[4 * 4096];
+__device__ unsigned long long g_wg_stamps[3 * 1024 * SW_WG_STAMP_N];
 extern "C" int sw_debug_wg_stamps(unsigned long long* host, int n) {
   return hipMemcpyFromSymbol(host, HIP_SYMBOL(g_wg_stamps), sizeof(unsigned long long) * (size_t)n) == hipSuccess ? 0 : -1;
 }
+#define WG_STAMP_PARAM , int stamp_slot
+#else
+#define WG_STAMP_PARAM
 #endif
 __global__ __launch_bounds__(SW_THREADS, 2) void wgrad_partial_kernel(WgBatch batch, float* __restrict__ ws,
                                                                       const float* __restrict__ adam_step, double beta1,
-                                                                      double beta2, float* __restrict__ bc_out) {
+                                                                      double beta2, float* __restrict__ bc_out,
+                                                                      const float* __restrict__ cp_src,
+                                                                      float* __restrict__ cp_dst, int cp_n WG_STAMP_PARAM) {
   __shared__ __attribute__((aligned(16))) float red[SW_WG_RED_FLOATS];
   if ((int)blockIdx.x >= wg_grid_jobs(batch.total_jobs)) {
-    if (threadIdx.x == 0) {
+    for (int i = threadIdx.x; i < cp_n; i += SW_THREADS) cp_dst[i] = cp_src[i];
+    if (threadIdx.x == 0 && bc_out) {
       float bc1, bc2s;
       wg_adam_bc_compute(adam_step, beta1, beta2, bc1, bc2s);
       bc_out[0] = bc1;
@@ -28,19 +34,15 @@
   const int job = ((((l >> 2) << 3) + (v & 7)) << 2) + (l & 3);
   if (job >= batch.total_jobs) return;
 #ifdef SW_WG_STAMP
-  const unsigned long long t0 = wall_clock64();
-#endif
+  unsigned long long* st = nullptr;
+  if (threadIdx.x == 0 && blockIdx.x < 1024) {
+    st = g_wg_stamps + ((size_t)stamp_slot * 1024 + blockIdx.x) * SW_WG_STAMP_N;
+    st[0] = wall_clock64();
+  }
+  wg_job(batch, ws, job, red, st);
+  if (st) st[6] = wall_clock64();
+#else
   wg_job(batch, ws, job, red);
-#ifdef SW_WG_STAMP
-  if (threadIdx.x == 0 && blockIdx.x < 2048) {
-    int p = 0;
-    while (p + 1 < batch.np && job >= batch.job0s[p + 1]) ++p;
-    unsigned long long* o = g_wg_stamps + (batch.total_jobs < 400 ? 4 * 2048 : 0) + 4 * blockIdx.x;
-    o[0] = t0;
-    o[1] = wall_clock64();
-    o[2] = p;
-    o[3] = batch.total_jobs;
-  }
 #endif
 }
 __device__ float g_wg_bc[2 * 64];
@@ -60,61 +62,8 @@
   return base[dev] + 2 * (next++ % 64);
 }
 
-#ifndef SW_WG_RSUB
-#define SW_WG_RSUB 4
-#endif
-#define SW_WG_REL (64 / SW_WG_RSUB)
 __global__ __launch_bounds__(256) void wgrad_reduce_kernel(WgBatch batch, const float* __restrict__ ws, WgAdam ad) {
-  const int gid = blockIdx.x * 256 + threadIdx.x;
-  const int lane = gid & 63, el = lane % SW_WG_REL, sub = lane / SW_WG_REL;
-  const int i = (gid >> 6) * SW_WG_REL + el;
-  bool live = i < batch.total_out;
-  int ii = live ? i : batch.total_out - 1;
-  int p = 0;
-#pragma unroll 1
-  while (p + 1 < batch.np && ii >= batch.out0s[p + 1]) ++p;
-  const WgProblem& P = batch.p[p];
-  const int e = ii - P.out0;
-  const int Kc = P.K + P.K2 + P.ones;
-  const size_t stride = (size_t)P.N * Kc;
-  const float* src = ws + P.ws_off + e;
-  const int n = e / Kc, k = e - n * Kc;
-  float* dst = k < P.K ? P.dW + (size_t)n * P.ldw + k : k < P.K + P.K2 ? P.dW2 + (size_t)n * P.ldw2 + (k - P.K) : P.db + n;
-  float* dst2 = (k >= P.K + P.K2 && P.db2) ? P.db2 + n : nullptr;
-  WgAdamPre a1 = {}, a2 = {};
-  float old1 = 0.f, old2 = 0.f;
-  if (ad.w) {
-    a1 = wg_adam_pre(ad, dst);
-    if (dst2) a2 = wg_adam_pre(ad, dst2);
-  }
-  if (P.accumulate) {
-    old1 = *dst;
-    if (dst2) old2 = *dst2;
-  }
-  float s = 0.f;
-  float s1 = 0.f, s2 = 0.f, s3 = 0.f;
-  int q = sub;
-  for (; q + 3 * SW_WG_RSUB < P.nsplit; q += 4 * SW_WG_RSUB) {
-    s += src[(size_t)q * stride];
-    s1 += src[(size_t)(q + SW_WG_RSUB) * stride];
-    s2 += src[(size_t)(q + 2 * SW_WG_RSUB) * stride];
-    s3 += src[(size_t)(q + 3 * SW_WG_RSUB) * stride];
-  }
-  for (; q < P.nsplit; q += SW_WG_RSUB) s += src[(size_t)q * stride];
-  s = (s + s1) + (s2 + s3);
-#pragma unroll
-  for (int o = SW_WG_REL; o < 64; o <<= 1) s += __shfl_xor(s, o);
-  float bc1 = 1.f, bc2s = 1.f;
-  if (ad.w) wg_adam_bc(ad, bc1, bc2s);
-  if (!live || sub != 0) return;
-  const float g = P.accumulate ? old1 + s : s;
-  *dst = g;
-  if (ad.w) wg_adam_fin(ad, a1, bc1, bc2s, g);
-  if (dst2) {
-    const float g2 = P.accumulate ? old2 + s : s;
-    *dst2 = g2;
-    if (ad.w) wg_adam_fin(ad, a2, bc1, bc2s, g2);
-  }
+  wg_reduce_thread<false>(batch, ws, ad, blockIdx.x * 256 + threadIdx.x, WgFold());
 }
 
 bool wg_shape_ok(int N, int K) {
@@ -290,28 +239,37 @@
   return SW_OK;
 }
 int wg_reduce_launch(WgBatch& b, float* ws, hipStream_t stream) { return wg_reduce_launch_adam(b, ws, WgAdam(), stream); }
+int wg_partial_launch(WgBatch& b, float* ws, WgAdam& ad, const float* cp_src, float* cp_dst, int cp_n, hipStream_t stream) {
+  ad.bc = nullptr;
+  if (b.total_jobs <= 0) return cp_n > 0 ? SW_ESHAPE : SW_OK;
+  float* bc = ad.w ? wg_bc_slot() : nullptr;
+#ifdef SW_WG_STAMP
+  static int stamp_launch = 0;
+  SW_LAUNCH(wgrad_partial_kernel, dim3(wg_grid_jobs(b.total_jobs) + (bc || cp_n > 0 ? 1 : 0)), dim3(SW_THREADS), 0, stream, b, ws,
+                     ad.step, ad.beta1, ad.beta2, bc, cp_src, cp_dst, cp_n, stamp_launch++ % 3);
+#else
+  SW_LAUNCH(wgrad_partial_kernel, dim3(wg_grid_jobs(b.total_jobs) + (bc || cp_n > 0 ? 1 : 0)), dim3(SW_THREADS), 0, stream, b, ws,
+                     ad.step, ad.beta1, ad.beta2, bc, cp_src, cp_dst, cp_n);
+#endif
+  SW_CHECK_LAUNCH("wgrad_partial_kernel");
+  ad.bc = bc;
+  return SW_OK;
+}
 int wg_launch_adam(WgBatch& b, float* ws, WgAdam& ad, hipStream_t stream) {
   if (b.np == 0) return SW_OK;
   size_t need = wg_finalize(b);
   if (need > SW_WG_WS_FLOATS) return SW_ESHAPE;
   if (b.total_out == 0) return SW_OK;
   ad.bc = nullptr;
-  if (b.total_jobs > 0) {
-    float* bc = ad.w ? wg_bc_slot() : nullptr;
-    SW_LAUNCH(wgrad_partial_kernel, dim3(wg_grid_jobs(b.total_jobs) + (bc ? 1 : 0)), dim3(SW_THREADS), 0, stream, b, ws, ad.step,
-                       ad.beta1, ad.beta2, bc);
-    SW_CHECK_LAUNCH("wgrad_partial_kernel");
-    ad.bc = bc;
-  }
+  if (b.total_jobs > 0)
+    if (int rc = wg_partial_launch(b, ws, ad, nullptr, nullptr, 0, stream)) return rc;
   return wg_reduce_launch_adam(b, ws, ad, stream);
 }
 
 int wg_launch_finalized(WgBatch& b, float* ws, hipStream_t stream) {
   if (b.total_out == 0) return SW_OK;
-  if (b.total_jobs > 0) {
-    SW_LAUNCH(wgrad_partial_kernel, dim3(wg_grid_jobs(b.total_jobs)), dim3(SW_THREADS), 0, stream, b, ws, (const float*)nullptr,
-                       0.0, 0.0, (float*)nullptr);
-    SW_CHECK_LAUNCH("wgrad_partial_kernel");
-  }
+  WgAdam none;
+  if (b.total_jobs > 0)
+    if (int rc = wg_partial_launch(b, ws, none, nullptr, nullptr, 0, stream)) return rc;
   return wg_reduce_launch(b, ws, stream);
 }
diff --git a/socialways_amd/csrc/sw_wgrad_dev.h b/socialways_amd/csrc/sw_wgrad_dev.h
--- a/socialways_amd/csrc/sw_wgrad_dev.h
+++ b/socialways_amd/csrc/sw_wgrad_dev.h
@@ -12,7 +12,20 @@
 #define SW_WG_DEPTH_TAIL SW_WG_DEPTH
 #endif
 
-#define SW_WG_RLD 69
+#define SW_WG_STAMP_N 8
+#ifdef SW_WG_STAMP
+#define WG_STAMP(k) do { if (st) st[k] = wall_clock64(); } while (0)
+#define WG_STAMP_ARG , unsigned long long* st
+#define WG_STAMP_PASS , st
+#else
+#define WG_STAMP(k) do { } while (0)
+#define WG_STAMP_ARG
+#define WG_STAMP_PASS
+#endif
+
+#define SW_WG_XLD 5
+#define SW_WG_RED_MAIN (4 * 16 * 64 * 4)
+#define SW_WG_RED_FLOATS (SW_WG_RED_MAIN + 4 * 64 * SW_WG_XLD)
 
 typedef __amdgpu_buffer_rsrc_t wg_rsrc;
 __device__ __forceinline__ wg_rsrc wg_make_rsrc(const float* base, unsigned bytes) {
@@ -37,6 +50,22 @@
   for (int i = 0; i < NV; ++i) v[i] = __uint_as_float(u[i]);
 }
 
+template <int NV>
+__device__ __forceinline__ void wg_stv(float* p, const float (&v)[NV]) {
+  if constexpr (NV == 4) {
+    typedef float v4u __attribute__((ext_vector_type(4), aligned(4)));
+    *reinterpret_cast<v4u*>(p) = v4u{v[0], v[1], v[2], v[3]};
+  } else if constexpr (NV == 3) {
+    typedef float v3u __attribute__((ext_vector_type(3), aligned(4)));
+    *reinterpret_cast<v3u*>(p) = v3u{v[0], v[1], v[2]};
+  } else if constexpr (NV == 2) {
+    typedef float v2u __attribute__((ext_vector_type(2), aligned(4)));
+    *reinterpret_cast<v2u*>(p) = v2u{v[0], v[1]};
+  } else {
+    *p = v[0];
+  }
+}
+
 __host__ __device__ inline int wg_tiles(int n, bool allow3) {
   if (n <= 16) return 1;
   for (int t = (n + 15) >> 4; t <= 4; ++t)
@@ -47,8 +76,8 @@
 template <int NA, int KR, int K2, int ONES, int DSCALE = 1>
 __device__ __forceinline__ void wg_run(const float* __restrict__ dbase, const float* __restrict__ abase, int ldd, int lda,
                                        int rbeg, int rend, int acol, int bcol, int lg, int ln,
-                                       float* __restrict__ mine,
-                                       const float* __restrict__ abase2, int lda2, int row0, int xoff) {
+                                       float* __restrict__ red, int wave, float* __restrict__ out, int Kc, int Nb,
+                                       const float* __restrict__ abase2, int lda2, int row0, int xoff WG_STAMP_ARG) {
   constexpr int KT = KR, XC = K2 + ONES;
   f32x4 acc[NA][KT];
 #pragma unroll
@@ -86,6 +115,10 @@
   };
 #pragma unroll
   for (int q = 0; q < DEPTH - 1; ++q) load(a[q], b[q], xq[q]);
+#ifdef SW_WG_STAMP
+  asm volatile("s_waitcnt vmcnt(0)" ::: "memory");
+  WG_STAMP(2);
+#endif
   for (int r = rbeg; r < rend; r += 4 * DEPTH) {
 #pragma unroll
     for (int q = 0; q < DEPTH; ++q) {
@@ -113,17 +146,15 @@
       }
     }
   }
+  WG_STAMP(3);
+  const int lane = 16 * lg + ln;
+  f32x4* const mine = reinterpret_cast<f32x4*>(red) + (wave * 16) * 64 + lane;
 #pragma unroll
   for (int i = 0; i < NA; ++i) {
 #pragma unroll
-    for (int kt = 0; kt < KT; ++kt) {
-#pragma unroll
-      for (int r = 0; r < 4; ++r) {
-        const int orow = NA * (4 * lg + r) + i;
-        if (KR * ln + kt < xoff) mine[orow * SW_WG_RLD + KR * ln + kt] = acc[i][kt][r];
-      }
-    }
-  }
+    for (int kt = 0; kt < KT; ++kt) mine[(i * KT + kt) * 64] = acc[i][kt];
+  }
+  float* const xred = red + SW_WG_RED_MAIN;
   if constexpr (XC > 0) {
 #pragma unroll
     for (int i = 0; i < NA; ++i) {
@@ -132,15 +163,45 @@
         float v = xacc[i][c];
         v += __shfl_xor(v, 16);
         v += __shfl_xor(v, 32);
-        if (lg == 0) mine[(NA * ln + i) * SW_WG_RLD + xoff + c] = v;
-      }
-    }
-  }
-}
-
-#define SW_WG_RED_FLOATS (4 * 64 * SW_WG_RLD)
+        if (lg == 0) xred[(wave * 64 + NA * ln + i) * SW_WG_XLD + c] = v;
+      }
+    }
+  }
+  sw_barrier();
+  WG_STAMP(4);
+  if (wave < NA) {
+    const f32x4* const all = reinterpret_cast<const f32x4*>(red) + (wave * KT) * 64 + lane;
+    f32x4 sum[KT];
+#pragma unroll
+    for (int kt = 0; kt < KT; ++kt) {
+      const f32x4 r0 = all[kt * 64], r1 = all[(16 + kt) * 64], r2 = all[(32 + kt) * 64], r3 = all[(48 + kt) * 64];
+      sum[kt] = (r0 + r1) + (r2 + r3);
+    }
+    if (KR * ln < xoff) {
+#pragma unroll
+      for (int r = 0; r < 4; ++r) {
+        const int orow = NA * (4 * lg + r) + wave;
+        if (orow < Nb) {
+          float v[KT];
+#pragma unroll
+          for (int kt = 0; kt < KT; ++kt) v[kt] = sum[kt][r];
+          wg_stv<KT>(out + (size_t)orow * Kc + KR * ln, v);
+        }
+      }
+    }
+  }
+  if constexpr (XC > 0) {
+    for (int e = threadIdx.x; e < Nb * XC; e += SW_THREADS) {
+      const int rr = e / XC, c = e - rr * XC;
+      const float* x = xred + rr * SW_WG_XLD + c;
+      out[(size_t)rr * Kc + xoff + c] = (x[0] + x[64 * SW_WG_XLD]) + (x[2 * 64 * SW_WG_XLD] + x[3 * 64 * SW_WG_XLD]);
+    }
+  }
+  WG_STAMP(5);
+}
+
 template <int DSCALE = 1>
-__device__ __forceinline__ void wg_job(const WgBatch& batch, float* __restrict__ ws, int job, float* red) {
+__device__ __forceinline__ void wg_job(const WgBatch& batch, float* __restrict__ ws, int job, float* red WG_STAMP_ARG) {
   const int lane = sw_lane(), wave = sw_wave(), ln = lane & 15, lg = lane >> 4;
   int p = 0;
 #pragma unroll 1
@@ -161,11 +222,16 @@
   const int rend = __builtin_amdgcn_readfirstlane(min(P.R, rbeg + rows_per));
   const int acol = n0 + max(0, min(NA * ln, Nb - NA));
   const int bcol = max(0, min(KR * ln, K - KR));
-  float* mine = red + wave * 64 * SW_WG_RLD;
+  float* out = ws + P.ws_off + ((size_t)sg * N + n0) * Kc;
+#ifdef SW_WG_STAMP
+  if (st) st[7] = p;
+#endif
+  WG_STAMP(1);
 #define WG_CASE(na, kr, k2, on)                                                                                     \
   case ((na * 8 + kr) * 2 + (k2 ? 1 : 0)) * 2 + on:                                                                 \
     wg_run<na, kr, k2, on, DSCALE>(P.delta, P.act, P.ldd, P.lda, rbeg, rend, acol, bcol, lg, ln,                      \
-                                   mine, P.act2 ? P.act2 : P.delta, P.act2 ? P.lda2 : P.ldd, P.row0, K);            \
+                                   red, wave, out, Kc, Nb, P.act2 ? P.act2 : P.delta, P.act2 ? P.lda2 : P.ldd, P.row0,  \
+                                   K WG_STAMP_PASS);                                                                \
     break;
 #define WG_CASES(na)                                                                                                \
   WG_CASE(na, 1, 0, 0) WG_CASE(na, 2, 0, 0) WG_CASE(na, 3, 0, 0) WG_CASE(na, 4, 0, 0)                               \
@@ -176,21 +242,112 @@
   }
 #undef WG_CASES
 #undef WG_CASE
-  sw_barrier();
-  float* out = ws + P.ws_off + (size_t)sg * N * Kc;
-  const int rows = min(64, N - n0), cols = min(SW_WG_RLD, Kc);
-  const int dq = SW_THREADS / cols, dr = SW_THREADS - dq * cols;
-  int rr = threadIdx.x / cols, cc = threadIdx.x - rr * cols;
-  const float* r0 = red, *r1 = red + 64 * SW_WG_RLD, *r2 = red + 2 * 64 * SW_WG_RLD, *r3 = red + 3 * 64 * SW_WG_RLD;
-  for (int e = threadIdx.x; e < rows * cols; e += SW_THREADS) {
-    const int o = rr * SW_WG_RLD + cc;
-    const float v = (r0[o] + r1[o]) + (r2[o] + r3[o]);
-    out[(size_t)(n0 + rr) * Kc + cc] = v;
-    cc += dr;
-    rr += dq;
-    if (cc >= cols) {
-      cc -= cols;
-      ++rr;
-    }
-  }
-}
+}
+
+#ifndef SW_WG_RSUB
+#define SW_WG_RSUB 4
+#endif
+#define SW_WG_REL (64 / SW_WG_RSUB)
+template <int NE, class Load>
+__device__ __forceinline__ void wg_slice_sums(Load ld, int nsplit, int sub, float (&out)[NE]) {
+  float s[NE], s1[NE], s2[NE], s3[NE];
+#pragma unroll
+  for (int j = 0; j < NE; ++j) s[j] = s1[j] = s2[j] = s3[j] = 0.f;
+  int k = 0;
+  for (; sub + k + 3 * SW_WG_RSUB < nsplit; k += 4 * SW_WG_RSUB) {
+    float v[NE][4];
+#pragma unroll
+    for (int j = 0; j < NE; ++j) {
+#pragma unroll
+      for (int a = 0; a < 4; ++a) v[j][a] = ld(j, k + a * SW_WG_RSUB);
+    }
+    if constexpr (NE > 1) {
+      asm volatile("" ::: "memory");
+#pragma unroll
+      for (int j = 0; j < NE; ++j) {
+#pragma unroll
+        for (int a = 0; a < 4; ++a) asm volatile("" : "+v"(v[j][a]));
+      }
+    }
+#pragma unroll
+    for (int j = 0; j < NE; ++j) {
+      s[j] += v[j][0];
+      s1[j] += v[j][1];
+      s2[j] += v[j][2];
+      s3[j] += v[j][3];
+    }
+  }
+  for (; sub + k < nsplit; k += SW_WG_RSUB) {
+    float v[NE];
+#pragma unroll
+    for (int j = 0; j < NE; ++j) v[j] = ld(j, k);
+    if constexpr (NE > 1) {
+      asm volatile("" ::: "memory");
+#pragma unroll
+      for (int j = 0; j < NE; ++j) asm volatile("" : "+v"(v[j]));
+    }
+#pragma unroll
+    for (int j = 0; j < NE; ++j) s[j] += v[j];
+  }
+#pragma unroll
+  for (int j = 0; j < NE; ++j) {
+    float t = (s[j] + s1[j]) + (s2[j] + s3[j]);
+#pragma unroll
+    for (int x = SW_WG_REL; x < 64; x <<= 1) t += __shfl_xor(t, x);
+    out[j] = t;
+  }
+}
+__device__ __forceinline__ float wg_slice_sum1(const float* __restrict__ src, size_t stride, int nsplit, int sub) {
+  float out[1];
+  wg_slice_sums<1>([&](int, int k) { return src[(size_t)(sub + k) * stride]; }, nsplit, sub, out);
+  return out[0];
+}
+
+struct WgFold {
+  int p_lstm = -1;
+  int p_m0 = -1, p_m1 = -1;
+};
+template <bool FOLD>
+__device__ __forceinline__ void wg_reduce_thread(const WgBatch& batch, const float* __restrict__ ws, const WgAdam& ad,
+                                                 const int gid, const WgFold& fold) {
+  const int lane = gid & 63, el = lane % SW_WG_REL, sub = lane / SW_WG_REL;
+  const int i = (gid >> 6) * SW_WG_REL + el;
+  bool live = i < batch.total_out;
+  int ii = live ? i : batch.total_out - 1;
+  int p = 0;
+#pragma unroll 1
+  while (p + 1 < batch.np && ii >= batch.out0s[p + 1]) ++p;
+  const WgProblem& P = batch.p[p];
+  const int e = ii - P.out0;
+  const int Kc = P.K + P.K2 + P.ones;
+  const int n = e / Kc, k = e - n * Kc;
+  int nsplit = P.nsplit;
+  if (FOLD && (p == fold.p_lstm ? k >= P.K : (p == fold.p_m0 || p == fold.p_m1))) {
+    live = false;
+    nsplit = 0;
+  }
+  float* dst = k < P.K ? P.dW + (size_t)n * P.ldw + k : k < P.K + P.K2 ? P.dW2 + (size_t)n * P.ldw2 + (k - P.K) : P.db + n;
+  float* dst2 = (k >= P.K + P.K2 && P.db2) ? P.db2 + n : nullptr;
+  WgAdamPre a1 = {}, a2 = {};
+  float old1 = 0.f, old2 = 0.f;
+  if (ad.w) {
+    a1 = wg_adam_pre(ad, dst);
+    if (dst2) a2 = wg_adam_pre(ad, dst2);
+  }
+  if (P.accumulate && nsplit) {
+    old1 = *dst;
+    if (dst2) old2 = *dst2;
+  }
+  const float s = wg_slice_sum1(ws + P.ws_off + e, (size_t)P.N * Kc, nsplit, sub);
+  float bc1 = 1.f, bc2s = 1.f;
+  if (ad.w) wg_adam_bc(ad, bc1, bc2s);
+  if (!live || sub != 0) return;
+  const float g = P.accumulate ? old1 + s : s;
+  *dst = g;
+  if (ad.w) wg_adam_fin(ad, a1, bc1, bc2s, g);
+  if (dst2) {
+    const float g2 = P.accumulate ? old2 + s : s;
+    *dst2 = g2;
+    if (ad.w) wg_adam_fin(ad, a2, bc1, bc2s, g2);
+  }
+}
diff --git a/socialways_amd/ops.py b/socialways_amd/ops.py
--- a/socialways_amd/ops.py
+++ b/socialways_amd/ops.py
@@ -152,6 +152,21 @@
 
 
 DFUSE = True
+WFOLD = True
+
+
+def gen_wgrad(enc_w, dec_w, gsave, gdelta, noise, S, B, To, Tp, d_enc, d_dec, part, wgrad, tmp, pending, adam=None):
+    head = (L.ptr(enc_w), L.ptr(dec_w), L.ptr(gsave), L.ptr(gdelta), L.ptr(noise), L.ptr(S), B, To, Tp, L.ptr(d_enc), L.ptr(d_dec))
+    opt = (None, None, None, None, 0, None, 0.0, 0.0, 0.0, 0.0)
+    if adam is not None:
+        w_all, g_all, m, v, step, lr, b1, b2, eps = adam
+        opt = (L.ptr(w_all), L.ptr(m), L.ptr(v), L.ptr(g_all), w_all.numel(), L.ptr(step), lr, b1, b2, eps)
+    if not WFOLD:
+        L.call("sw_gen_wgrad_unfolded", *head, part, L.ptr(wgrad), L.ptr(tmp), pending, *opt, L.stream())
+    elif adam is not None:
+        L.call("sw_gen_wgrad_adam", *head, L.ptr(wgrad), L.ptr(tmp), pending, *opt, L.stream())
+    else:
+        L.call("sw_gen_wgrad", *head, part, L.ptr(wgrad), L.ptr(tmp), pending, L.stream())
 
 
 def gen_backward(enc_w, emb_w, att_w, dec_w, ctx, dpred4, d_enc, d_emb, d_att, d_dec, ws=None, tag="g", aux=None, adam=None,
@@ -194,14 +209,7 @@
     L.call("sw_enc_lstm_bwd_aux", L.ptr(enc_w), L.ptr(ctx.gsave), None, L.ptr(dhT), L.ptr(dcT), None, B, To, 0,
            L.ptr(gdelta), None, None, L.ptr(aux_late[0]) if aux_late else None, L.ptr(aux_late[1]) if aux_late else None,
            L.ptr(aux_late[2]) if aux_late else None, aux_late[1].numel() if aux_late else 0, L.stream())
-    if adam is not None:
-        w_all, g_all, m, v, step, lr, b1, b2, eps = adam
-        L.call("sw_gen_wgrad_adam", L.ptr(enc_w), L.ptr(dec_w), L.ptr(ctx.gsave), L.ptr(gdelta), L.ptr(ctx.noise), L.ptr(ctx.S),
-               B, To, Tp, L.ptr(d_enc), L.ptr(d_dec), L.ptr(wgrad), L.ptr(tmp), pending, L.ptr(w_all), L.ptr(m), L.ptr(v),
-               L.ptr(g_all), w_all.numel(), L.ptr(step), lr, b1, b2, eps, L.stream())
-        return
-    L.call("sw_gen_wgrad", L.ptr(enc_w), L.ptr(dec_w), L.ptr(ctx.gsave), L.ptr(gdelta), L.ptr(ctx.noise), L.ptr(ctx.S), B, To, Tp,
-           L.ptr(d_enc), L.ptr(d_dec), 0, L.ptr(wgrad), L.ptr(tmp), pending, L.stream())
+    gen_wgrad(enc_w, dec_w, ctx.gsave, gdelta, ctx.noise, ctx.S, B, To, Tp, d_enc, d_dec, 0, wgrad, tmp, pending, adam)
 
 
 class GenCtxK:
@@ -264,8 +272,7 @@
            L.ptr(gdelta_k), L.ptr(dh_k), L.ptr(dc_k), L.ptr(dS_k), L.ptr(aux[0]) if aux else None,
            L.ptr(aux[1]) if aux else None, L.ptr(aux[2]) if aux else None, aux[1].numel() if aux else 0, L.stream())
     dhT, dcT, dS = (t.view(K, B, 64).sum(0) for t in (dh_k, dc_k, dS_k))
-    L.call("sw_gen_wgrad", L.ptr(enc_w), L.ptr(dec_w), L.ptr(ctx.gsave_k), L.ptr(gdelta_k), L.ptr(ctx.noise_k), L.ptr(ctx.S_k),
-           KB, To, Tp, L.ptr(d_enc), L.ptr(d_dec), 1, L.ptr(wgrad), L.ptr(tmp), None, L.stream())
+    gen_wgrad(enc_w, dec_w, ctx.gsave_k, gdelta_k, ctx.noise_k, ctx.S_k, KB, To, Tp, d_enc, d_dec, 1, wgrad, tmp, None)
     pending = None
     if one.use_social and (one.scenes.P > 0 or one.scenes.NB > 0):
         sc = one.scenes
@@ -281,8 +288,7 @@
         d_att.zero_()
     L.call("sw_enc_lstm_bwd", L.ptr(enc_w), L.ptr(one.gsave), None, L.ptr(dhT), L.ptr(dcT), None, B, To, 0,
            L.ptr(gdelta_1), None, None, L.stream())
-    L.call("sw_gen_wgrad", L.ptr(enc_w), L.ptr(dec_w), L.ptr(one.gsave), L.ptr(gdelta_1), L.ptr(one.noise), L.ptr(one.S), B, To, Tp,
-           L.ptr(d_enc), L.ptr(d_dec), 2, L.ptr(wgrad), L.ptr(tmp), pending, L.stream())
+    gen_wgrad(enc_w, dec_w, one.gsave, gdelta_1, one.noise, one.S, B, To, Tp, d_enc, d_dec, 2, wgrad, tmp, pending)
 
 
 def obs_len_arg(obs_len, B, To, lo, device):
```
